# youmi-zym/GO-SLAM

Measured on AMD Instinct MI355X. Metric: BA keyframes/s (6 x FactorGraph.update: reproject + corr lookup + GRU + 2 GN BA iters) on synthetic 640x480 RGB-D, higher is better.
Workload: dtype f32 (BA/geometry; fp64 solve), f16 (corr volume, GRU convs); 1 GPU; configs[1]-shaped frontend window: 60x80 maps (480x640 RGB-D), P=25 keyframes, E=75 edges, 6 updates/keyframe, iters=2, RGB-D depth prior, upsample on; parallelism=replicas x1 (tracking does not shard)

## Files before the change

go_slam_amd/_lib.py:

```python
import ctypes
import os
import subprocess

_HERE = os.path.dirname(os.path.abspath(__file__))
CSRC = os.path.join(_HERE, "csrc")
LIB_PATH = os.environ.get("GOSLAM_HIP_LIB") or os.path.join(CSRC, "libgoslam_hip.so")

_lib = None

c_int, c_float, c_void_p, c_size_t = ctypes.c_int, ctypes.c_float, ctypes.c_void_p, ctypes.c_size_t

_P = c_void_p
SIGNATURES = {
    "gs_version": (ctypes.c_char_p, []),
    "gs_last_error": (ctypes.c_char_p, []),
    "gs_enc_conv_wpack_elems": (c_size_t, [c_int, c_int, c_int]),
    "gs_enc_conv_stat_chunks": (c_int, [c_int, c_int, c_int]),
    "gs_enc_conv": (c_int, [_P, c_int, c_int, _P, _P, _P, c_int, c_int, c_int, c_int, c_int, c_int, c_int, _P, _P, _P]),
    "gs_norm_act_workspace_bytes_chunks": (c_size_t, [c_int, c_int, c_int]),
    "gs_timing_begin": (c_int, [_P]),
    "gs_timing_end": (c_int, []),
    "gs_timing_read": (c_int, [ctypes.c_char_p, ctypes.POINTER(ctypes.c_double), ctypes.POINTER(c_int)]),
    "gs_timing_names": (c_int, [ctypes.c_char_p, c_int]),
    "gs_corr_index_forward": (c_int, [_P, _P, _P] + [c_int] * 7 + [_P]),
    "gs_corr_index_backward": (c_int, [_P, _P, _P] + [c_int] * 7 + [_P]),
    "gs_corr_lookup_pyramid": (c_int, [_P] * 6 + [c_int] * 9 + [_P]),
    "gs_corr_lookup_enc": (c_int, [_P] * 8 + [c_int] * 7 + [_P]),
    "gs_corr_lookup_enc_slots": (c_int, [_P] * 9 + [c_int] * 7 + [_P]),
    "gs_corr_lookup_pyramid_slots": (c_int, [_P] * 7 + [c_int] * 9 + [_P]),
    "gs_corr_volume_pyramid_slots": (c_int, [_P] * 7 + [c_int] * 5 + [_P, c_size_t, _P]),
    "gs_corr_volume_workspace_bytes": (c_size_t, [c_int] * 4),
    "gs_corr_volume_pyramid": (c_int, [_P] * 6 + [c_int] * 5 + [_P, c_size_t, _P]),
    "gs_corr_level_elems": (c_size_t, [c_int] * 4),
    "gs_altcorr_backward": (c_int, [_P] * 6 + [c_int] * 8 + [_P]),
    "gs_altcorr_forward": (c_int, [_P] * 4 + [c_int] * 9 + [_P]),
    "gs_altcorr_pyramid": (c_int, [_P] * 8 + [c_int] * 5 + [_P]),
    "gs_reproject": (c_int, [_P] * 7 + [c_int] * 3 + [_P]),
    "gs_projmap": (c_int, [_P] * 7 + [c_int] * 3 + [_P]),
    "gs_frame_distance": (c_int, [_P] * 6 + [c_int] * 3 + [c_float, _P]),
    "gs_iproj": (c_int, [_P] * 4 + [c_int] * 3 + [_P]),
    "gs_depth_filter": (c_int, [_P] * 6 + [c_int] * 4 + [_P]),
    "gs_pointcloud_workspace_bytes": (c_size_t, [c_int] * 3),
    "gs_pointcloud_count": (c_int, [_P] * 5 + [c_float, c_float] + [c_int] * 4 + [_P, c_size_t, _P]),
    "gs_pointcloud_mask": (c_int, [_P, _P] + [c_int] * 4 + [_P, c_size_t, _P]),
    "gs_pointcloud_scan": (c_int, [c_int] * 3 + [_P, c_size_t, _P, _P]),
    "gs_pointcloud_emit": (c_int, [_P] * 5 + [c_int] * 4 + [_P, c_size_t, ctypes.c_longlong, _P, _P, _P]),
    "gs_frame_prep_color": (c_int, [_P, c_int, c_int, c_int, c_int, c_int, _P]),
    "gs_frame_prep_depth": (c_int, [_P, c_int, c_float, c_int, c_int, c_int, c_int, _P]),
    "gs_cvx_upsample":(c_int, [_P] * 4 + [c_int] * 4 + [_P]),
    "gs_upmask_upsample": (c_int, [_P, c_int, _P, _P, _P, _P, _P, c_int, c_int, c_int, _P]),
    "gs_bias_act": (c_int, [_P, _P, _P, c_int, c_int, c_int, c_int, c_int, _P]),
    "gs_motion_features": (c_int, [_P, _P, _P, c_int, c_int, c_int, _P]),
    "gs_ba_inputs": (c_int, [_P] * 6 + [c_int, c_int, c_int, _P]),
    "gs_lowmem_gather": (c_int, [_P] * 7 + [c_int, c_int, c_int, _P]),
    "gs_lowmem_scatter": (c_int, [_P] * 8 + [c_int, c_int, c_int, _P]),
    "gs_damping_rows": (c_int, [_P] * 5 + [c_int, c_int, c_float, c_float, _P]),
    "gs_conv1x1": (c_int, [_P, c_int, c_int, _P, _P, c_int, _P, c_int, c_int, ctypes.c_longlong, _P]),
    "gs_conv7x7_c4": (c_int, [_P, _P, _P, _P, c_int, c_int, c_int, c_int, c_int, c_int, _P]),
    "gs_conv3x3_wpack_elems": (c_size_t, [c_int, c_int]),
    "gs_conv3x3_pp": (c_int, [_P, c_int, c_int, _P, c_int, _P, c_int, c_int, c_int, c_int, c_int, c_int, _P]),
    "gs_conv3x3_bias_relu": (c_int, [_P, c_int, c_int, _P, _P, _P, c_int, c_int, c_int, c_int, c_int, _P]),
    "gs_conv3x3_gru_zr": (c_int, [_P, c_int, c_int, _P, _P, _P, _P, _P, _P, c_int, c_int, c_int, _P]),
    "gs_conv3x3_gru_zr2": (c_int, [_P, _P, c_int, c_int, _P, _P, _P, _P, _P, _P, c_int, c_int, c_int, _P]),
    "gs_conv3x3_gru_q": (c_int, [_P, _P, c_int, c_int, _P, _P, _P, _P, _P, _P, _P, c_int, c_int, c_int, _P]),
    "gs_conv3x3_head": (c_int, [_P, c_int, _P, c_int, _P, _P, c_int, c_int, c_float, _P, c_int, c_int, c_int, _P]),
    "gs_segment_mean": (c_int, [_P, c_int, _P, c_int, _P, _P, _P, c_int, c_int, c_int, _P]),
    "gs_norm_act_workspace_bytes": (c_size_t, [c_int, c_int, c_int]),
    "gs_norm_act": (c_int, [_P, _P, _P, _P] + [c_int] * 6 + [c_float, _P, c_size_t, c_int, _P]),
    "gs_gru_glo_workspace_bytes": (c_size_t, [c_int]),
    "gs_gru_glo": (c_int, [_P] * 11 + [c_int, c_int, _P, c_size_t, _P]),
    "gs_gru_glo_fused_workspace_bytes": (c_size_t, [c_int, c_int]),
    "gs_gru_glo_fused": (c_int, [_P, c_int] + [_P] * 10 + [c_int, c_int, _P, c_size_t, _P]),
    "gs_gru_gate_zr": (c_int, [_P] * 6 + [c_int] * 3 + [_P]),
    "gs_gru_gate_q": (c_int, [_P] * 7 + [c_int] * 2 + [_P]),
    "gs_edge_prep": (c_int, [_P] * 4 + [c_int, _P, _P] + [c_int] * 6 + [c_float, c_int, c_int, _P]),
    "gs_edge_greedy": (c_int, [_P] * 5 + [c_int] * 5 + [c_float, c_int, c_int, _P]),
    "gs_ba_workspace_bytes": (c_size_t, [c_int] * 5),
    "gs_ba": (c_int, [_P] * 9 + [c_int] * 3 + [c_float, c_float] + [c_int] * 6 + [_P, _P, _P, _P, c_size_t, _P]),
    "gs_ba_ex": (c_int, [_P] * 9 + [c_int] * 3 + [c_float, c_float] + [c_int] * 6 + [_P, _P, _P, _P, c_size_t, c_int, _P]),
    "gs_chol_solve": (c_int, [_P, _P, c_int, c_float, c_float, c_int, _P, _P, _P]),
    "gs_traj_eval_workspace_bytes": (c_size_t, [c_int]),
    "gs_traj_world": (c_int, [_P, _P, c_int, _P, _P, _P]),
    "gs_ape_moments": (c_int, [_P, _P, _P, c_int, _P, _P, c_size_t, _P]),
    "gs_ape_stats": (c_int, [_P, _P, _P, _P, c_int, _P, _P, _P, c_size_t, _P]),
    "gs_grid_meta_default": (c_int, [_P]),
    "gs_neus_level_major_min_points": (c_int, [c_int]),
    "gs_render_sample": (c_int, [_P] * 7 + [c_float, _P, _P, _P] + [c_int] * 3 + [_P]),
    "gs_grid_encode": (c_int, [_P] * 4 + [c_int, _P]),
    "gs_grid_backward": (c_int, [_P, _P, _P, c_int, c_float, _P, _P, c_int, c_float, _P, _P, c_int, _P]),
    "gs_mlp_workspace_bytes": (c_size_t, [c_int, c_int]),
    "gs_mlp_forward": (c_int, [_P] * 3 + [c_int] * 3 + [_P, c_size_t, _P]),
    "gs_neus_forward_workspace_bytes": (c_size_t, [c_int, c_int]),
    "gs_neus_forward": (c_int, [_P] * 9 + [c_float] + [_P] * 18 + [c_float, _P, c_float, c_int, c_int, _P, c_size_t, _P]),
    "gs_neus_forward_pieces": (c_int, [c_int] * 3),
    "gs_neus_forward_segmented": (c_int, [_P] * 9 + [c_float] + [_P] * 18 + [c_float, c_int, _P, _P, c_float]
                                  + [c_int] * 4 + [_P, c_size_t, _P]),
    "gs_render_img_sample": (c_int, [_P, c_int, c_int] + [c_float] * 4 + [_P] * 5 + [c_int] + [_P] * 5
                             + [c_int, c_int, _P]),
    "gs_render_img_metrics_workspace_bytes": (c_size_t, []),
    "gs_render_img_metrics": (c_int, [_P] * 7 + [c_int, c_int] + [_P] * 5 + [c_size_t, _P]),
    "gs_neus_backward_rays": (c_int, [_P] * 13 + [c_int, c_int, _P]),
    "gs_mapping_loss": (c_int, [_P] * 8 + [c_float] * 4 + [c_int] + [_P] * 4 + [c_int, c_int, _P]),
    "gs_map_grad_sqnorm": (c_int, [_P, c_size_t, c_float, _P, c_size_t, _P, _P]),
    "gs_map_adamw": (c_int, [_P, _P, _P, _P, _P, c_size_t, c_float, _P, c_size_t] + [c_float] * 6 + [c_int, _P, c_float, _P]),
    "gs_map_gram_blocks": (c_int, [c_int]),
    "gs_map_gram": (c_int, [_P, c_int, _P, _P]),
    "gs_map_step_prep": (c_int, [_P, c_int, _P, c_float, c_float, c_int] + [_P] * 13),
    "gs_map_step_post": (c_int, [_P, c_int, c_float, _P, c_int, _P, _P, _P, c_float, _P, _P, c_int, c_float, c_int, _P, _P, _P]),
    "gs_map_adamw_seg": (c_int, [_P, _P, _P, _P, _P, c_size_t, c_float, _P, _P, _P, _P, _P, c_size_t] + [c_float] * 6
                         + [c_int, _P, _P, c_float, _P]),
    "gs_mlp_backward_blocks": (c_int, [c_int]),
    "gs_mlp_backward": (c_int, [_P, _P, _P, _P, c_float, _P, _P, c_int, _P]),
    "gs_neus_backward_points": (c_int, [_P] * 7 + [c_float] + [_P] * 9 + [c_int, c_float, _P, _P, c_int, c_float] + [_P] * 5 + [c_int, c_float, c_int, _P, c_int, c_int, _P, _P]),
    "gs_neus_backward_points_binned": (c_int, [_P] * 7 + [c_float] + [_P] * 9 + [c_int, c_float, _P, _P, c_float] + [_P] * 5
                                       + [c_int, c_float, c_int, _P, c_int, c_int, _P, c_size_t, _P, _P, _P]),
    "gs_neus_bin_workspace_bytes": (c_size_t, [c_int]),
    "gs_neus_backward_raygrad": (c_int, [_P] * 7 + [c_float] + [_P] * 9 + [c_int, c_float] + [_P] * 3
                                 + [c_int, c_int, _P]),
    "gs_pose_grad_reduce": (c_int, [_P, _P, _P, c_int, _P, _P]),
    "gs_ray_draw": (c_int, [_P] * 7 + [c_int] * 4 + [c_float] * 4 + [_P] * 5),
    "gs_sdf_lattice": (c_int, [_P] * 3 + [c_int] * 3 + [_P] * 6 + [_P]),
    "gs_mcubes_workspace_bytes": (c_size_t, [c_int] * 3),
    "gs_mcubes_count": (c_int, [_P, c_int, c_int, c_int, c_float, _P, c_size_t, _P]),
    "gs_mcubes_scan": (c_int, [c_int, c_int, c_int, _P, c_size_t, _P, _P]),
    "gs_mcubes_emit": (c_int, [_P, c_int, c_int, c_int, c_float, _P, c_size_t, ctypes.c_longlong, ctypes.c_longlong,
                               _P, _P, _P]),
    "gs_mesh_depth_workspace_bytes": (c_size_t, []),
    "gs_mesh_depth": (c_int, [_P, c_int, _P, c_int, _P, c_int] + [c_float] * 4 + [c_int, c_int, c_float, c_float, _P, _P,
                                                                                   c_size_t, _P]),
    "gs_mesh_visibility": (c_int, [_P, c_int, _P, _P, c_int] + [c_float] * 4 + [c_int, c_int, c_float, _P, _P, _P]),
    "gs_face_components_workspace_bytes": (c_size_t, [c_int]),
    "gs_face_components": (c_int, [_P, c_int, _P, _P, c_size_t, _P]),
    "gs_face_component_areas": (c_int, [_P, _P, c_int, _P, _P, _P, _P, _P, c_size_t, _P]),
    "gs_hull_extremes_workspace_bytes": (c_size_t, [c_int]),
    "gs_hull_extremes": (c_int, [_P, c_int, _P, _P, c_size_t, _P]),
    "gs_hull_prefilter": (c_int, [_P, c_int, _P, c_int, ctypes.c_double, _P, _P]),
    "gs_mesh_visbuf_workspace_bytes": (c_size_t, []),
    "gs_mesh_visbuf": (c_int, [_P, c_int, _P, c_int, _P, c_int] + [c_float] * 4 + [c_int, c_int, c_float, c_float, _P, _P,
                                                                                    c_size_t, _P]),
    "gs_line_visbuf": (c_int, [_P, c_int, ctypes.c_uint, _P, c_int] + [c_float] * 4 + [c_int, c_int, c_float, c_float, _P,
                                                                                        _P]),
    "gs_vertex_normals": (c_int, [_P, c_int, _P, c_int, ctypes.c_double, _P, _P, _P]),
    "gs_visbuf_resolve": (c_int, [_P, c_int, c_int, c_int, _P, c_int, _P, c_int, _P] + [c_float] * 4
                          + [_P, _P, c_int, _P, c_int, c_float, c_float, ctypes.c_uint, _P, _P]),
    "gs_nn_cell_keys":(c_int, [_P, c_int, _P, _P, _P, _P]),
    "gs_nn_grid_build": (c_int, [_P, c_int, _P, _P, _P, _P, _P, _P, _P]),
    "gs_nn_query_workspace_bytes": (c_size_t, [c_int]),
    "gs_nn_query": (c_int, [_P, _P, _P, _P, c_int, _P, _P, _P, c_int, _P, ctypes.c_double, _P, _P, _P, c_size_t, _P]),
    "gs_icp_moments_workspace_bytes": (c_size_t, [c_int]),
    "gs_icp_moments": (c_int, [_P, c_int, _P, _P, _P, _P, _P, _P, c_size_t, _P]),
}


class ColorView(ctypes.Structure):
    _fields_ = [("src", c_void_p), ("map_x", c_void_p), ("map_y", c_void_p), ("tmp", c_void_p), ("dst", c_void_p),
                ("h", c_int), ("w", c_int), ("c", c_int), ("mh", c_int), ("mw", c_int)]


class DepthView(ctypes.Structure):
    _fields_ = [("src", c_void_p), ("dst", c_void_p), ("h", c_int), ("w", c_int)]


FRAME_PREP_MAX_VIEWS = 32


class GridMeta(ctypes.Structure):
    _fields_ = [("scale", c_float * 16), ("resolution", ctypes.c_uint32 * 16), ("size", ctypes.c_uint32 * 16),
                ("offset", ctypes.c_uint32 * 16), ("hashed", ctypes.c_uint32 * 16), ("total", ctypes.c_uint32)]


def grid_meta():
    m = GridMeta()
    check(lib().gs_grid_meta_default(ctypes.byref(m)), "gs_grid_meta_default")
    return m


def build(verbose=False):
    cmd = ["make", "-C", CSRC, "-j8"]
    res = subprocess.run(cmd, stdout=subprocess.PIPE, stderr=subprocess.STDOUT, text=True)
    if verbose or res.returncode != 0:
        print(res.stdout)
    if res.returncode != 0:
        raise RuntimeError("building libgoslam_hip.so failed:\n" + res.stdout[-4000:])
    return LIB_PATH


def lib():
    global _lib
    if _lib is None:
        if not os.path.exists(LIB_PATH):
            raise RuntimeError(
                f"{LIB_PATH} not found: build it with `python -c 'import __graft_entry__ as g; g.build()'` "
                "(go_slam_amd has no CPU fallback)")
        handle = ctypes.CDLL(LIB_PATH)
        for name, (res, args) in SIGNATURES.items():
            fn = getattr(handle, name)
            fn.restype = res
            fn.argtypes = args
        _lib = handle
    return _lib


def check(rc, what):
    if rc != 0:
        msg = lib().gs_last_error().decode("utf-8", "replace")
        raise RuntimeError(f"{what} failed (status {rc}): {msg}")


class kernel_timer:

    def __init__(self, device=None):
        self.device = device

    def __enter__(self):
        check(lib().gs_timing_begin(stream_ptr(self.device)), "gs_timing_begin")
        return self

    def __exit__(self, *exc):
        lib().gs_timing_end()
        return False

    def read(self):
        L = lib()
        buf = ctypes.create_string_buffer(1 << 16)
        check(L.gs_timing_names(buf, len(buf)), "gs_timing_names")
        out = {}
        for name in [n for n in buf.value.decode().split(",") if n]:
            ms, cnt = ctypes.c_double(0.0), c_int(0)
            check(L.gs_timing_read(name.encode(), ctypes.byref(ms), ctypes.byref(cnt)), "gs_timing_read")
            out[name] = (ms.value, cnt.value)
        return out


def stream_ptr(device=None):
    import torch
    return ctypes.c_void_p(torch.cuda.current_stream(device).cuda_stream)


_EMPTY_SENTINEL = {}


def ptr(t):
    if t is None:
        return ctypes.c_void_p(0)
    p = t.data_ptr()
    if p == 0 and t.numel() == 0 and t.is_cuda:
        s = _EMPTY_SENTINEL.get(t.device)
        if s is None:
            import torch
            s = _EMPTY_SENTINEL[t.device] = torch.zeros(64, dtype=torch.uint8, device=t.device)
        p = s.data_ptr()
    return ctypes.c_void_p(p)
```

go_slam_amd/csrc/ba.hip:

```cpp
#include "common.h"

int gs_chol_solve_launch(double* H, double* b, int n, float lm, float ep, float* dx_out, int32_t* fail_flag,
                         int32_t* fail_count, hipStream_t st);

namespace {

constexpr float kMinDepth = 0.25f;
constexpr float kAlpha = 0.05f;
constexpr int kPrepThreads = 1024;
constexpr int kAccSplit = 4;
constexpr int kMaxBuf = 4096;

struct BaWs {
  int32_t* hdr;
  int32_t* kinv;
  int32_t* kx;
  int32_t* edge_m;
  int32_t* row_ptr;
  int32_t* csr_edge;
  int32_t* ent_ptr;
  int32_t* ent_src;
  int32_t* ent_pose;
  int32_t* pair_ptr;
  float* Q;
// ... 312 lines not shown
          if (j_in) gs_atomic_add_f64(&w.b[6 * pj_ + (tid - 84)], s);
        }
      }
      __syncthreads();
    }
  }

  if (!motion_only && active) {
    if (nsplit > 1) {
      float* po = w.part + (((size_t)split * gridDim.y + m) * 8) * hw + p;
      po[0] = Csum;
      po[(size_t)hw] = wsum;
#pragma unroll
      for (int n = 0; n < 6; ++n) po[(size_t)(2 + n) * hw] = Ei[n];
      return;
    }
    const size_t o = (size_t)m * hw + p;
    const float sens = disps_sens[(size_t)k * hw + p];
    const float mk = (sens > 0.0f) ? 1.0f : 0.0f;
    const float C = Csum + mk * kAlpha + (1.0f - mk) * eta[o];
    const float ww = wsum - mk * kAlpha * (disp - sens);
    w.Q[o] = 1.0f / C;
    w.W[o] = ww;
    if (i_in) {
      float* eo = w.Ei + ((size_t)m * 6) * hw + p;
#pragma unroll
      for (int n = 0; n < 6; ++n) eo[(size_t)n * hw] = Ei[n];
    }
  }
}

__global__ __launch_bounds__(256) void ba_accum_finish_kernel(const float* __restrict__ disps,
                                                              const float* __restrict__ disps_sens,
                                                              const float* __restrict__ eta, int t0, int t1, int hw, int nsp,
                                                              BaWs w) {
  const int m = blockIdx.y;
  if (m >= w.hdr[0]) return;
  const int nsplit = min(nsp, max(w.row_ptr[m + 1] - w.row_ptr[m], 1));
  if (nsplit <= 1) return;
  const int p = blockIdx.x * 256 + threadIdx.x;
  if (p >= hw) return;
  float acc[8];
#pragma unroll
  for (int n = 0; n < 8; ++n) acc[n] = 0.0f;
  for (int s2 = 0; s2 < nsplit; ++s2) {
    const float* pi_ = w.part + (((size_t)s2 * gridDim.y + m) * 8) * hw + p;
#pragma unroll
    for (int n = 0; n < 8; ++n) acc[n] += pi_[(size_t)n * hw];
  }
  const int k = w.kx[m];
  const size_t o = (size_t)m * hw + p;
  const float disp = disps[(size_t)k * hw + p];
  const float sens = disps_sens[(size_t)k * hw + p];
  const float mk = (sens > 0.0f) ? 1.0f : 0.0f;
  const float C = acc[0] + mk * kAlpha + (1.0f - mk) * eta[o];
  const float ww = acc[1] - mk * kAlpha * (disp - sens);
  w.Q[o] = 1.0f / C;
  w.W[o] = ww;
  const int pi = k - t0;
  if (pi >= 0 && pi < t1 - t0) {
    float* eo = w.Ei + ((size_t)m * 6) * hw + p;
#pragma unroll
    for (int n = 0; n < 6; ++n) eo[(size_t)n * hw] = acc[2 + n];
  }
}

__global__ __launch_bounds__(256) void ba_schur_kernel(int M, int hw, int P, BaWs w) {
  __shared__ float red[4][44];
  const int tid = threadIdx.x;
  const int wave = tid >> 6, lane = tid & 63;
  typedef const __attribute__((address_space(4))) int* cip;
  cip pair_ptr = (cip)w.pair_ptr, ent_ptr = (cip)w.ent_ptr, ent_pose = (cip)w.ent_pose, ent_src = (cip)w.ent_src;
  const int n_pairs = pair_ptr[M];
  const int n6 = 6 * P;
  for (int pidx = blockIdx.x; pidx < n_pairs; pidx += gridDim.x) {
    int lo = 0, hi = M;
    while (hi - lo > 1) {
      const int mid = (lo + hi) >> 1;
      if (pair_ptr[mid] <= pidx) lo = mid; else hi = mid;
    }
    const int m = lo;
    const int eb = ent_ptr[m];
    const int nm = ent_ptr[m + 1] - eb;
    const int r = pidx - pair_ptr[m];
    const int a = r / nm, b = r - a * nm;
    const int pa = ent_pose[eb + a], pb = ent_pose[eb + b];
    if (pa < pb) continue;
    const int sa = ent_src[eb + a], sb = ent_src[eb + b];
    const float* Ea = (sa < M) ? w.Ei + (size_t)sa * 6 * hw : w.Eij + (size_t)(sa - M) * 6 * hw;
    const float* Eb = (sb < M) ? w.Ei + (size_t)sb * 6 * hw : w.Eij + (size_t)(sb - M) * 6 * hw;
    const float* Qm = w.Q + (size_t)m * hw;
    const float* Wm = w.W + (size_t)m * hw;
    const bool diag = (a == b);
    float S[36];
#pragma unroll
    for (int i = 0; i < 36; ++i) S[i] = 0.f;
    float vv[6] = {0.f, 0.f, 0.f, 0.f, 0.f, 0.f};
    constexpr int UP = 4;
    for (int p0 = tid; p0 < hw; p0 += UP * 256) {
      float q[UP], ea[UP][6], eb_[UP][6], ww[UP];
#pragma unroll
      for (int u = 0; u < UP; ++u) {
        const int p = p0 + 256 * u;
        const bool ok = p < hw;
        const int pc = ok ? p : tid;
        q[u] = Qm[pc];
#pragma unroll
        for (int n = 0; n < 6; ++n) {
          ea[u][n] = Ea[(size_t)n * hw + pc];
          eb_[u][n] = Eb[(size_t)n * hw + pc];
        }
        ww[u] = diag ? Wm[pc] : 0.0f;
      }
#pragma unroll
      for (int u = 0; u < UP; ++u) {
        if (p0 + 256 * u < hw) {
#pragma unroll
          for (int n = 0; n < 6; ++n) ea[u][n] = ea[u][n] * q[u];
#pragma unroll
          for (int n = 0; n < 6; ++n)
#pragma unroll
            for (int c = 0; c < 6; ++c) S[n * 6 + c] = fmaf(ea[u][n], eb_[u][c], S[n * 6 + c]);
          if (diag) {
#pragma unroll
            for (int n = 0; n < 6; ++n) vv[n] = fmaf(ea[u][n], ww[u], vv[n]);
          }
        }
      }
    }
    {
      float rs[42];
#pragma unroll
      for (int i = 0; i < 36; ++i) rs[i] = S[i];
#pragma unroll
      for (int n = 0; n < 6; ++n) rs[36 + n] = vv[n];
      gs_wave_reduce_scatter<42>(rs, lane);
      const int ix = gs_bitrev6(lane);
      if (ix < 42) red[wave][ix] = rs[0];
    }
    __syncthreads();
    if (tid < 36) {
      const int rr = tid / 6, cc = tid - rr * 6;
      const double s = (double)((red[0][tid] + red[1][tid]) + (red[2][tid] + red[3][tid]));
      if (pa > pb || rr >= cc)
        gs_atomic_add_f64(&w.H[(size_t)(6 * pa + rr) * n6 + (6 * pb + cc)], -s);
    } else if (diag && tid < 42) {
      const double s = (double)((red[0][tid] + red[1][tid]) + (red[2][tid] + red[3][tid]));
      gs_atomic_add_f64(&w.b[6 * pa + (tid - 36)], -s);
    }
    __syncthreads();
  }
}

__global__ __launch_bounds__(256) void ba_update_kernel(
    float* __restrict__ poses, float* __restrict__ disps, const float* __restrict__ dx,
    float* __restrict__ dz, int M, int t0, int t1, int hw, BaWs w) {
  const int tid = threadIdx.x;
  const int P = t1 - t0;
  if ((int)blockIdx.y == M) {
    if (blockIdx.x != 0) return;
    for (int kk = t0 + tid; kk < t1; kk += 256) {
      float* pp = poses + (size_t)kk * 7;
      float t[3] = {pp[0], pp[1], pp[2]};
      float q[4] = {pp[3], pp[4], pp[5], pp[6]};
      float xi[6], tn[3], qn[4];
#pragma unroll
      for (int n = 0; n < 6; ++n) xi[n] = dx[(size_t)(kk - t0) * 6 + n];
      gs_retr_se3(xi, t, q, tn, qn);
      pp[0] = tn[0]; pp[1] = tn[1]; pp[2] = tn[2];
      pp[3] = qn[0]; pp[4] = qn[1]; pp[5] = qn[2]; pp[6] = qn[3];
    }
    return;
  }
  const int m = blockIdx.y;
  const int p = blockIdx.x * 256 + tid;
  if (p >= hw) return;
  if (m >= w.hdr[0]) {
    dz[(size_t)m * hw + p] = 0.0f;
    return;
  }
  const int eb = w.ent_ptr[m], ee = w.ent_ptr[m + 1];
  float dw = 0.f;
  for (int idx = eb; idx < ee; ++idx) {
    const int pn = w.ent_pose[idx];
    if (pn <= 0 || pn >= P) continue;
    const int s = w.ent_src[idx];
    const float* En = (s < M) ? w.Ei + (size_t)s * 6 * hw : w.Eij + (size_t)(s - M) * 6 * hw;
    float acc = 0.f;
#pragma unroll
    for (int n = 0; n < 6; ++n) acc += En[(size_t)n * hw + p] * dx[(size_t)pn * 6 + n];
    dw += acc;
  }
  const size_t o = (size_t)m * hw + p;
  const float z = w.Q[o] * (w.W[o] - dw);
  dz[o] = z;
  const size_t dk = (size_t)w.kx[m] * hw + p;
  disps[dk] = disps[dk] + z;
}

__global__ void ba_status_kernel(int32_t* status_out, BaWs w) {
  if (threadIdx.x < 4) status_out[threadIdx.x] = (threadIdx.x == 2) ? w.hdr[3] : (threadIdx.x == 3 ? w.hdr[4] : w.hdr[threadIdx.x]);
}

}

extern "C" size_t gs_ba_workspace_bytes(int n_edges, int n_poses, int n_depth, int nbuf, int hw) {
  if (n_edges < 0 || n_poses < 0 || n_depth < 0 || nbuf < 0 || hw < 0) return 0;
  return carve(nullptr, n_edges, n_poses, n_depth, nbuf, hw).total + 256;
}

extern "C" int gs_ba_ex(float* poses, float* disps, const float* intrinsics, const float* disps_sens,
                        const float* targets, const float* weights, const float* eta, const int64_t* ii,
                        const int64_t* jj, int t0, int t1, int iterations, float lm, float ep, int motion_only,
                        int n_edges, int n_depth, int nbuf, int h, int w, float* dx, float* dz,
                        int32_t* status_out, void* workspace, size_t workspace_bytes, int flags, gs_stream_t stream) {
  GS_REQUIRE(poses && disps && intrinsics && disps_sens && targets && weights && ii && jj && dx && workspace,
             "ba: null pointer");
  GS_REQUIRE(motion_only || (eta && dz), "ba: eta/dz required unless motion_only");
  GS_REQUIRE(h > 0 && w > 0 && n_edges >= 0 && iterations >= 0, "ba: bad shape");
  GS_REQUIRE(t0 >= 0 && t1 > t0 && t1 <= nbuf, "ba: window [%d,%d) outside buffer of %d frames", t0, t1, nbuf);
  GS_REQUIRE(nbuf <= kMaxBuf, "ba: buffer of %d frames exceeds the supported %d", nbuf, kMaxBuf);
  GS_REQUIRE(n_depth > 0 && n_depth <= nbuf && n_depth <= 65534, "ba: n_depth=%d out of range", n_depth);
  const int hw = h * w, P = t1 - t0, M = n_depth;
  const size_t need = gs_ba_workspace_bytes(n_edges, P, M, nbuf, hw);
  if (workspace_bytes < need) {
    gs_set_error("ba: workspace too small (%zu < %zu bytes)", workspace_bytes, need);
    return GS_ERR_WORKSPACE;
  }
  void* base = (void*)gs_align((size_t)workspace);
  BaWs ws = carve(base, n_edges, P, M, nbuf, hw);
  hipStream_t st = (hipStream_t)stream;
  const int n6 = 6 * P;

  const bool reuse = (flags & 1) != 0;
  if (!reuse) {
    ba_prep_kernel<<<1, kPrepThreads, 0, st>>>(ii, jj, n_edges, nbuf, t0, t1, M, ws);
    GS_CHECK_LAUNCH("ba_prep");
  }
  const int chunks = gs_cdiv(hw, 256);
  for (int it = 0; it < iterations; ++it) {
    if (hipMemsetAsync(ws.H, 0, ((size_t)n6 * n6 + n6) * sizeof(double), st) != hipSuccess) {
      gs_set_error("ba: memset failed");
      return GS_ERR_LAUNCH;
    }
    const int nsp = (!motion_only && n_edges >= 6 * M) ? kAccSplit : 1;
    ba_accum_kernel<<<dim3(chunks, M, nsp), 256, 0, st>>>(poses, disps, intrinsics, disps_sens, targets, weights,
                                                          eta, jj, t0, t1, hw, w, motion_only,
                                                          (reuse && it == 0) ? 1 : 0, ws);
    GS_CHECK_LAUNCH("ba_accum");
    if (!motion_only) {
      if (nsp > 1) {
        ba_accum_finish_kernel<<<dim3(chunks, M), 256, 0, st>>>(disps, disps_sens, eta, t0, t1, hw, nsp, ws);
        GS_CHECK_LAUNCH("ba_accum_finish");
      }
      ba_schur_kernel<<<2048, 256, 0, st>>>(M, hw, P, ws);
      GS_CHECK_LAUNCH("ba_schur");
    }
    int rc = gs_chol_solve_launch(ws.H, ws.b, n6, lm, ep, dx, &ws.hdr[2], &ws.hdr[3], st);
    if (rc != GS_OK) return rc;
    if (motion_only)
      ba_update_kernel<<<dim3(1, 1), 256, 0, st>>>(poses, disps, dx, dz, 0, t0, t1, hw, ws);
    else
      ba_update_kernel<<<dim3(chunks, M + 1), 256, 0, st>>>(poses, disps, dx, dz, M, t0, t1, hw, ws);
    GS_CHECK_LAUNCH("ba_update");
  }
  if (status_out) {
    ba_status_kernel<<<1, 64, 0, st>>>(status_out, ws);
    GS_CHECK_LAUNCH("ba_status");
  }
  return GS_OK;
}

extern "C" int gs_ba(float* poses, float* disps, const float* intrinsics, const float* disps_sens,
                     const float* targets, const float* weights, const float* eta, const int64_t* ii,
                     const int64_t* jj, int t0, int t1, int iterations, float lm, float ep, int motion_only,
                     int n_edges, int n_depth, int nbuf, int h, int w, float* dx, float* dz,
                     int32_t* status_out, void* workspace, size_t workspace_bytes, gs_stream_t stream) {
  return gs_ba_ex(poses, disps, intrinsics, disps_sens, targets, weights, eta, ii, jj, t0, t1, iterations, lm, ep,
                  motion_only, n_edges, n_depth, nbuf, h, w, dx, dz, status_out, workspace, workspace_bytes, 0, stream);
}
```

go_slam_amd/csrc/conv3x3_pp.hip:

```cpp
#include "common.h"
#include "conv3x3_common.h"

namespace {

constexpr int PP_KG = 4;
constexpr int PP_PSTR = 5;
constexpr int pp_zpad(int tw) { return (((2 * (tw + 2) + 2) * PP_PSTR + 3 + 15) / 16) * 16; }
constexpr int pp_patch_slots(int tw) {
  return (((512 / tw + 2) * (tw + 2) * PP_PSTR + 511) / 512) * 512 + pp_zpad(tw);
}

__device__ __attribute__((aligned(16))) const uint32_t pp_zero_page[4] = {0u, 0u, 0u, 0u};

__device__ __forceinline__ void pp_glds16(const void* src, void* lds_wave_base) {
  __builtin_amdgcn_global_load_lds((const __attribute__((address_space(1))) void*)src,
                                   (__attribute__((address_space(3))) void*)lds_wave_base, 16, 0, 0);
}

#define PP_BAR()                              \
  do {                                        \
    asm volatile("" ::: "memory");            \
    __builtin_amdgcn_s_barrier();             \
    asm volatile("" ::: "memory");            \
    __builtin_amdgcn_sched_barrier(0);        \
  } while (0)

#define PP_LGKM0()                                        \
  do {                                                    \
    asm volatile("s_waitcnt lgkmcnt(0)" ::: "memory");    \
    __builtin_amdgcn_sched_barrier(0);                    \
  } while (0)

struct PpEpi {
  const float* bias;
  const float* glo;
  const _Float16* inp_pre;
  const _Float16* aux0;
  const _Float16* aux1;
  _Float16* out0;
  _Float16* out1;
  const _Float16* xb;
  int xsb, split;
  long long* dbg;
  int variant;
};

template <bool PROBE>
__device__ __forceinline__ void pp_stamp(long long* dbg, int slot) {
  if constexpr (PROBE) {
    if (dbg && threadIdx.x == 0) dbg[(size_t)blockIdx.x * 4 + slot] = (long long)__builtin_amdgcn_s_memtime();
  }
}

__device__ __forceinline__ float pp_sigm(float v) { return gs_sigmoid(v); }

template <int TW, int EPI, int BN = 128, bool PROBE = false>
__global__ __launch_bounds__(512, 1) void conv3x3_pp_kernel(const _Float16* __restrict__ x, int xs, int C,
                                                            const half8* __restrict__ wpack, _Float16* __restrict__ y,
                                                            int ys, int H, int W, int rows, int tiles_x, int NB,
                                                            int xcd, PpEpi ep) {
  static_assert(BN == 128 || (BN == 64 && (EPI == 0 || EPI == 3)), "64-channel workgroups: plain / bias + ReLU only");
  constexpr int PP_BN = BN;
  constexpr int PP_WTAP = PP_KG * PP_BN;
  constexpr int NJ = BN / 64;
  constexpr int PP_TS = NJ == 2 ? 72 : 40;
  constexpr int TH_ = 512 / TW, PW_ = TW + 2, NPX = (TH_ + 2) * PW_;
  constexpr int PSTR = PP_PSTR;
  constexpr int ZPAD = pp_zpad(TW);
  constexpr int NROUND = (NPX * PSTR + 511) / 512;
  constexpr int PSLOTS = NROUND * 512 + ZPAD;
  constexpr int ZSLOT = NROUND * 512;
  static_assert(PSLOTS == pp_patch_slots(TW), "launch_pp sizes the LDS with the same formula");
  static_assert(NROUND <= 9, "one DMA round per tap");
  extern __shared__ half8 smem[];
  half8* const pbuf = smem;
  half8* const wbuf = smem + 2 * PSLOTS;
  half8* const wjunk = wbuf + 4 * PP_WTAP;
  const int tid = threadIdx.x, lane = tid & 63;
  const int wv = __builtin_amdgcn_readfirstlane(tid >> 6);
  const int grp2 = wv >> 2;
  const int wm = (wv & 1) + 2 * grp2;
  const int wn = (wv >> 1) & 1;
  const int r = lane & 31, kgl = lane >> 5;
  int tix, nb;
  decode_block(blockIdx.x, gridDim.x / NB, NB, xcd, tix, nb);
  const int tx0 = (tix % tiles_x) * TW;
  const int g0 = (tix / tiles_x) * TH_;
  const int nchunk = C / 32;
  const int T = nchunk * 9;
  const half8* wsrc = wpack + (size_t)nb * T * PP_WTAP;

  int pb[4];
  bool top[4], bot[4];
#pragma unroll
  for (int i = 0; i < 4; ++i) {
    int ty, tx;
    tile_pixel<TW, true>(wm, i, r, ty, tx);
    pb[i] = ty * PW_ + tx;
    const int yy = (g0 + ty) % H;
    top[i] = yy == 0;
    bot[i] = yy == H - 1;
  }
  int poff[NROUND];
#pragma unroll
  for (int q = 0; q < NROUND; ++q) {
    const int s = q * 512 + tid, p = s / PSTR, kg = s - PSTR * p;
    int off = -1;
    if (p < NPX && kg < 4) {
      const int pr = p / PW_, pc = p - pr * PW_;
      const int gv = g0 + pr - 1, gx = tx0 + pc - 1;
      if (gv >= 0 && gv < rows && gx >= 0 && gx < W) off = (gv * W + gx) * 4 + kg;
    }
    poff[q] = off;
  }

  int vb[4], vt[4], vo[4];
#pragma unroll
  for (int i = 0; i < 4; ++i) {
    vb[i] = pb[i] * PSTR + kgl;
    vt[i] = top[i] ? ZSLOT : vb[i];
    vo[i] = bot[i] ? ZSLOT : vb[i];
  }
  {
    const half8 z8 = {0, 0, 0, 0, 0, 0, 0, 0};
    if (tid < ZPAD) pbuf[ZSLOT + tid] = z8;
    else if (tid < 2 * ZPAD) pbuf[PSLOTS + ZSLOT + tid - ZPAD] = z8;
    static_assert(2 * ZPAD <= 512, "one store per thread");
  }

  float16v acc[NJ][4];
#pragma unroll
  for (int j = 0; j < NJ; ++j)
#pragma unroll
    for (int i = 0; i < 4; ++i)
#pragma unroll
      for (int e = 0; e < 16; ++e) acc[j][i][e] = 0.0f;
  half8 a[2][NJ], b[2][4];

  auto issue_patch = [&](int src_chunk, int buf, int q, int off) {
    const void* src = (const void*)pp_zero_page;
    if (off >= 0) {
      const size_t pix = (size_t)(off >> 2);
      const int c0 = src_chunk * 32 + (off & 3) * 8;
      if constexpr (EPI == 1 || EPI == 2)
        src = c0 < ep.split ? (const void*)(x + pix * xs + c0) : (const void*)(ep.xb + pix * ep.xsb + (c0 - ep.split));
      else
        src = (const void*)(x + pix * xs + c0);
    }
    pp_glds16(src, pbuf + buf * PSLOTS + q * 512 + wv * 64);
  };
  auto issue_w = [&](int src_tap, int buf) {
    if constexpr (BN == 128) {
      pp_glds16(wsrc + (size_t)src_tap * PP_WTAP + tid, wbuf + buf * PP_WTAP + wv * 64);
    } else {
      if (wv < 4) pp_glds16(wsrc + (size_t)src_tap * PP_WTAP + tid, wbuf + buf * PP_WTAP + wv * 64);
      else pp_glds16((const void*)pp_zero_page, wjunk + (wv - 4) * 64);
    }
  };
  auto read_frags = [&](int pbuf_ix, int wbuf_ix, int tap) {
    const half8* wb = wbuf + wbuf_ix * PP_WTAP;
    const half8* pp = pbuf + pbuf_ix * PSLOTS;
    const int dy = tap / 3, toff = dy * PW_ + (tap % 3);
#pragma unroll
    for (int s = 0; s < 2; ++s) {
      const int kg = 2 * s + kgl;
#pragma unroll
      for (int j = 0; j < NJ; ++j) a[s][j] = wb[kg * PP_BN + wn * (PP_BN / 2) + 32 * j + r];
    }
#pragma unroll
    for (int i = 0; i < 4; ++i) {
      int base = dy == 0 ? vt[i] : dy == 2 ? vo[i] : vb[i];
      if constexpr (PROBE) {
        if (ep.variant & 2) base = vb[i];
      }
      asm volatile("" : "+v"(base));
      const half8* q = pp + base;
      b[0][i] = q[toff * PSTR];
      b[1][i] = q[toff * PSTR + 2];
    }
  };
  bool prio = true;
  if constexpr (PROBE) prio = !(ep.variant & 1);
  auto math = [&](auto&& between) {
    if (prio) __builtin_amdgcn_s_setprio(1);
#pragma unroll
    for (int i = 0; i < 2; ++i)
#pragma unroll
      for (int j = 0; j < NJ; ++j)
        acc[j][i] = __builtin_amdgcn_mfma_f32_32x32x16_f16(a[0][j], b[0][i], acc[j][i], 0, 0, 0);
    __builtin_amdgcn_sched_barrier(0);
    between();
    __builtin_amdgcn_sched_barrier(0);
#pragma unroll
    for (int i = 2; i < 4; ++i)
#pragma unroll
      for (int j = 0; j < NJ; ++j)
        acc[j][i] = __builtin_amdgcn_mfma_f32_32x32x16_f16(a[0][j], b[0][i], acc[j][i], 0, 0, 0);
#pragma unroll
    for (int i = 0; i < 4; ++i)
#pragma unroll
      for (int j = 0; j < NJ; ++j)
        acc[j][i] = __builtin_amdgcn_mfma_f32_32x32x16_f16(a[1][j], b[1][i], acc[j][i], 0, 0, 0);
    if (prio) __builtin_amdgcn_s_setprio(0);
  };

  pp_stamp<PROBE>(ep.dbg, 0);
#pragma unroll
  for (int q = 0; q < NROUND; ++q) issue_patch(0, 0, q, poff[q]);
  issue_w(0, 0);
  issue_w(1, 1);
  issue_w(2, 2);
  asm volatile("s_waitcnt vmcnt(0) lgkmcnt(0)" ::: "memory");
  PP_BAR();
  pp_stamp<PROBE>(ep.dbg, 1);
  if (grp2 == 1) PP_BAR();
  read_frags(0, 0, 0);
  PP_LGKM0();
  PP_BAR();

  for (int ck = 0; ck < nchunk; ++ck) {
#pragma unroll
    for (int tap = 0; tap < 9; ++tap) {
      const int tg = ck * 9 + tap;
      __builtin_amdgcn_sched_barrier(0);
      math([&]() {
        if constexpr (PROBE) {
          if (ep.variant & 4) return;
        }
        const int tw = tg + 3 < T ? tg + 3 : T - 1;
        issue_w(tw, (tg + 3) & 3);
        if (tap < NROUND) issue_patch(ck + 1 < nchunk ? ck + 1 : nchunk - 1, (ck + 1) & 1, tap, poff[tap]);
      });
      __builtin_amdgcn_sched_barrier(0);
      if (tap < NROUND) asm volatile("s_waitcnt vmcnt(2)" ::: "memory");
      else asm volatile("s_waitcnt vmcnt(1)" ::: "memory");
      PP_BAR();
      bool reads = true;
      if constexpr (PROBE) reads = !(ep.variant & 8);
      if (reads) {
        if (tap < 8) read_frags(ck & 1, (tg + 1) & 3, tap + 1);
        else if (ck + 1 < nchunk) read_frags((ck + 1) & 1, (tg + 1) & 3, 0);
      }
      PP_LGKM0();
      PP_BAR();
    }
  }
  pp_stamp<PROBE>(ep.dbg, 2);
  if (grp2 == 0) PP_BAR();
  asm volatile("s_waitcnt vmcnt(0)" ::: "memory");
  PP_BAR();

  _Float16* tile = reinterpret_cast<_Float16*>(smem) + wv * 32 * PP_TS;
  _Float16* yb = y + nb * PP_BN + wn * (PP_BN / 2);
  constexpr int PIECES = NJ * 4;
  constexpr int PXIT = 64 / PIECES;
  constexpr int NIT = 32 / PXIT;
#pragma unroll
  for (int i = 0; i < 4; ++i) {
    size_t pix4[NIT];
    bool ok4[NIT];
    half8 pi4[NIT], u4[NIT], v4[NIT];
    const int piece = lane & (PIECES - 1);
    const int c8 = wn * (PP_BN / 2) + piece * 8;
#pragma unroll
    for (int it = 0; it < NIT; ++it) {
      const int pxr = it * PXIT + lane / PIECES;
      int ty, tx;
      tile_pixel<TW, true>(wm, i, pxr, ty, tx);
      const int gv = g0 + ty, gx = tx0 + tx;
      ok4[it] = gv < rows && gx < W;
      pix4[it] = (size_t)gv * W + gx;
      if constexpr (EPI == 1 || EPI == 2) {
        const half8 z8 = {0, 0, 0, 0, 0, 0, 0, 0};
        pi4[it] = z8; u4[it] = z8; v4[it] = z8;
        if (ok4[it]) {
          if constexpr (EPI == 1) {
            if (ep.inp_pre) pi4[it] = *reinterpret_cast<const half8*>(ep.inp_pre + pix4[it] * 384 + nb * 128 + c8);
            if (nb == 1) u4[it] = *reinterpret_cast<const half8*>(x + pix4[it] * xs + c8);
          } else {
            if (ep.inp_pre) pi4[it] = *reinterpret_cast<const half8*>(ep.inp_pre + pix4[it] * 384 + 256 + c8);
            u4[it] = *reinterpret_cast<const half8*>(ep.aux0 + pix4[it] * 128 + c8);
            v4[it] = *reinterpret_cast<const half8*>(ep.aux1 + pix4[it] * 128 + c8);
          }
        }
      }
    }
#pragma unroll
    for (int j = 0; j < NJ; ++j)
#pragma unroll
      for (int g = 0; g < 4; ++g) {
        half4 o;
#pragma unroll
        for (int e = 0; e < 4; ++e) o[e] = (_Float16)acc[j][i][4 * g + e];
        *reinterpret_cast<half4*>(tile + r * PP_TS + j * 32 + 8 * g + 4 * kgl) = o;
      }
    __builtin_amdgcn_fence(__ATOMIC_RELEASE, "wavefront");
    __builtin_amdgcn_wave_barrier();
    __builtin_amdgcn_fence(__ATOMIC_ACQUIRE, "wavefront");
#pragma unroll
    for (int it = 0; it < NIT; ++it) {
      const int pxr = it * PXIT + lane / PIECES;
      if (ok4[it]) {
        const half8 v = *reinterpret_cast<const half8*>(tile + pxr * PP_TS + piece * 8);
        const size_t pix = pix4[it];
        if constexpr (EPI == 0) {
          *reinterpret_cast<half8*>(yb + pix * ys + piece * 8) = v;
        } else if constexpr (EPI == 3) {
          const float* bb = ep.bias + nb * PP_BN + c8;
          half8 o;
#pragma unroll
          for (int k = 0; k < 8; ++k) o[k] = (_Float16)fmaxf((float)v[k] + bb[k], 0.0f);
          *reinterpret_cast<half8*>(yb + pix * ys + piece * 8) = o;
        } else if constexpr (EPI == 1) {
          const int img = (int)(pix / ((size_t)H * W));
          const half8 pi = pi4[it];
          const float* bb = ep.bias + nb * 128 + c8;
          const float* gg = ep.glo + (size_t)img * 256 + nb * 128 + c8;
          half8 o;
          if (nb == 0) {
#pragma unroll
            for (int k = 0; k < 8; ++k) o[k] = (_Float16)pp_sigm((float)v[k] + (float)pi[k] + bb[k] + gg[k]);
            *reinterpret_cast<half8*>(ep.out0 + pix * 128 + c8) = o;
          } else {
            const half8 net = u4[it];
#pragma unroll
            for (int k = 0; k < 8; ++k)
              o[k] = (_Float16)(pp_sigm((float)v[k] + (float)pi[k] + bb[k] + gg[k]) * (float)net[k]);
            *reinterpret_cast<half8*>(ep.out1 + pix * 128 + c8) = o;
          }
        } else {
          const int img = (int)(pix / ((size_t)H * W));
          const half8 pi = pi4[it], zz = u4[it], nn = v4[it];
          const float* bb = ep.bias + c8;
          const float* gg = ep.glo + (size_t)img * 128 + c8;
          half8 o;
#pragma unroll
          for (int k = 0; k < 8; ++k) {
            const float a_ = (float)v[k] + (float)pi[k] + bb[k] + gg[k];
            const float q = gs_tanh(a_);
            const float zf = (float)zz[k];
            o[k] = (_Float16)((1.0f - zf) * (float)nn[k] + zf * q);
          }
          *reinterpret_cast<half8*>(ep.out0 + pix * 128 + c8) = o;
        }
      }
    }
    __builtin_amdgcn_fence(__ATOMIC_RELEASE, "wavefront");
    __builtin_amdgcn_wave_barrier();
  }
  pp_stamp<PROBE>(ep.dbg, 3);
}

template <int TW, int EPI, int BN = 128, bool PROBE = false>
int launch_pp(const void* x, int x_stride, int c_in, const void* wpack, void* y, int y_stride, int n_out, int n, int h,
              int w, int xcd, hipStream_t st, PpEpi ep = PpEpi()) {
  constexpr int PP_BN = BN, PP_WTAP = PP_KG * BN;
  constexpr size_t lds = (size_t)(2 * pp_patch_slots(TW) + 4 * PP_WTAP + (BN == 64 ? 256 : 0)) * sizeof(half8);
  static_assert(lds <= 160 * 1024, "conv3x3_pp: more LDS than a CU has");
  static GsLdsLimit limit;
  if (int rc = limit.raise((const void*)conv3x3_pp_kernel<TW, EPI, BN, PROBE>, lds, "conv3x3_pp")) return rc;
  const long long rows = (long long)n * h;
  GS_REQUIRE(rows * w < (1ll << 29), "conv3x3_pp: too many pixels");
  const int tiles_x = gs_cdiv(w, TW), tiles_y = gs_cdiv((int)rows, 512 / TW);
  const int NB = n_out / PP_BN;
  const long long blocks = (long long)tiles_x * tiles_y * NB;
  GS_REQUIRE(blocks < (1ll << 31), "conv3x3_pp: too many workgroups");
  conv3x3_pp_kernel<TW, EPI, BN, PROBE><<<dim3((unsigned)blocks), 512, lds, st>>>(
      (const _Float16*)x, x_stride, c_in, (const half8*)wpack, (_Float16*)y, y_stride, h, w, (int)rows, tiles_x, NB, xcd,
      ep);
  GS_CHECK_LAUNCH("conv3x3_pp");
  return GS_OK;
}

template <int EPI, int BN = 128>
int dispatch_pp(const void* x, int x_stride, int c_in, const void* wpack, int tw, void* y, int y_stride, int n_out, int n,
                int h, int w, int xcd, hipStream_t st, PpEpi ep = PpEpi()) {
  if (tw == 8) return launch_pp<8, EPI, BN>(x, x_stride, c_in, wpack, y, y_stride, n_out, n, h, w, xcd, st, ep);
  return launch_pp<16, EPI, BN>(x, x_stride, c_in, wpack, y, y_stride, n_out, n, h, w, xcd, st, ep);
}

int pp_block_channels(int n_out) { return n_out % 128 == 0 ? 128 : 64; }

int pp_tile_width(int w) { return gs_cdiv(w, 8) * 8 < gs_cdiv(w, 16) * 16 ? 8 : 16; }

}

extern "C" int gs_conv3x3_pp(const void* x, int x_stride, int c_in, const void* wpack, int tw, void* y, int y_stride,
                             int n_out, int n, int h, int w, int xcd_order, gs_stream_t stream) {
  GS_REQUIRE(x && wpack && y, "conv3x3_pp: null pointer");
  GS_REQUIRE(tw == 8 || tw == 16, "conv3x3_pp: tile width must be 8 or 16");
  GS_REQUIRE(c_in > 0 && c_in % 32 == 0, "conv3x3_pp: c_in must be a multiple of 32 (weights packed with kc = 32)");
  GS_REQUIRE(n_out > 0 && n_out % 64 == 0, "conv3x3_pp: n_out must be a multiple of 64");
  GS_REQUIRE(x_stride >= c_in && x_stride % 8 == 0, "conv3x3_pp: x_stride must be >= c_in and a multiple of 8");
  GS_REQUIRE(y_stride >= n_out && y_stride % 8 == 0, "conv3x3_pp: y_stride must be >= n_out and a multiple of 8");
  GS_REQUIRE(n >= 0 && h > 0 && w > 0, "conv3x3_pp: bad shape");
  if (n == 0) return GS_OK;
  if (pp_block_channels(n_out) == 64)
    return dispatch_pp<0, 64>(x, x_stride, c_in, wpack, tw, y, y_stride, n_out, n, h, w, xcd_order ? 1 : 0,
                              (hipStream_t)stream);
  return dispatch_pp<0>(x, x_stride, c_in, wpack, tw, y, y_stride, n_out, n, h, w, xcd_order ? 1 : 0,
                        (hipStream_t)stream);
}

extern "C" int gs_conv3x3_gru_zr(const void* hx, int hx_stride, int c_in, const void* wpack, const float* bias_zr,
                                 const float* glo_zr, const void* inp_pre, void* z_out, void* rnet_out, int n, int h,
                                 int w, gs_stream_t stream) {
  GS_REQUIRE(hx && wpack && bias_zr && glo_zr && z_out && rnet_out, "conv3x3_gru_zr: null pointer");
  GS_REQUIRE(c_in >= 128 && c_in % 32 == 0, "conv3x3_gru_zr: c_in must be >= 128 and a multiple of 32");
  GS_REQUIRE(hx_stride >= c_in && hx_stride % 8 == 0, "conv3x3_gru_zr: bad hx_stride");
  GS_REQUIRE(n >= 0 && h > 0 && w > 0, "conv3x3_gru_zr: bad shape");
  if (n == 0) return GS_OK;
  PpEpi ep = PpEpi();
  ep.bias = bias_zr;
  ep.glo = glo_zr;
  ep.inp_pre = (const _Float16*)inp_pre;
  ep.out0 = (_Float16*)z_out;
  ep.out1 = (_Float16*)rnet_out;
  ep.xb = (const _Float16*)hx;
  ep.xsb = hx_stride;
  ep.split = 1 << 30;
  return dispatch_pp<1>(hx, hx_stride, c_in, wpack, pp_tile_width(w), nullptr, 0, 256, n, h, w, 1, (hipStream_t)stream, ep);
}

extern "C" int gs_conv3x3_gru_zr2(const void* net, const void* x_rest, int x_rest_stride, int c_rest, const void* wpack,
                                  const float* bias_zr, const float* glo_zr, const void* inp_pre, void* z_out,
                                  void* rnet_out, int n, int h, int w, gs_stream_t stream) {
  GS_REQUIRE(net && x_rest && wpack && bias_zr && glo_zr && z_out && rnet_out, "conv3x3_gru_zr2: null pointer");
  GS_REQUIRE(c_rest > 0 && c_rest % 32 == 0, "conv3x3_gru_zr2: c_rest must be a multiple of 32");
  GS_REQUIRE(x_rest_stride >= c_rest && x_rest_stride % 8 == 0, "conv3x3_gru_zr2: bad x_rest_stride");
  GS_REQUIRE(n >= 0 && h > 0 && w > 0, "conv3x3_gru_zr2: bad shape");
  if (n == 0) return GS_OK;
  PpEpi ep = PpEpi();
  ep.bias = bias_zr;
  ep.glo = glo_zr;
  ep.inp_pre = (const _Float16*)inp_pre;
  ep.out0 = (_Float16*)z_out;
  ep.out1 = (_Float16*)rnet_out;
  ep.xb = (const _Float16*)x_rest;
  ep.xsb = x_rest_stride;
  ep.split = 128;
  return dispatch_pp<1>(net, 128, 128 + c_rest, wpack, pp_tile_width(w), nullptr, 0, 256, n, h, w, 1,
                        (hipStream_t)stream, ep);
}

extern "C" int gs_conv3x3_gru_q(const void* rnet, const void* x_rest, int x_rest_stride, int c_rest, const void* wpack,
                                const float* bias_q, const float* glo_q, const void* inp_pre, const void* z,
                                const void* net, void* net_out, int n, int h, int w, gs_stream_t stream) {
  GS_REQUIRE(rnet && x_rest && wpack && bias_q && glo_q && z && net && net_out, "conv3x3_gru_q: null pointer");
  GS_REQUIRE(c_rest > 0 && c_rest % 32 == 0, "conv3x3_gru_q: c_rest must be a multiple of 32");
  GS_REQUIRE(x_rest_stride >= c_rest && x_rest_stride % 8 == 0, "conv3x3_gru_q: bad x_rest_stride");
  GS_REQUIRE(n >= 0 && h > 0 && w > 0, "conv3x3_gru_q: bad shape");
  if (n == 0) return GS_OK;
  PpEpi ep = PpEpi();
  ep.bias = bias_q;
  ep.glo = glo_q;
  ep.inp_pre = (const _Float16*)inp_pre;
  ep.aux0 = (const _Float16*)z;
  ep.aux1 = (const _Float16*)net;
  ep.out0 = (_Float16*)net_out;
  ep.xb = (const _Float16*)x_rest;
  ep.xsb = x_rest_stride;
  ep.split = 128;
  return dispatch_pp<2>(rnet, 128, 128 + c_rest, wpack, pp_tile_width(w), nullptr, 0, 128, n, h, w, 1,
                        (hipStream_t)stream, ep);
}

extern "C" int gs_conv3x3_bias_relu(const void* x, int x_stride, int c_in, const void* wpack, const float* bias, void* y,
                                    int y_stride, int n_out, int n, int h, int w, gs_stream_t stream) {
  GS_REQUIRE(x && wpack && bias && y, "conv3x3_bias_relu: null pointer");
  GS_REQUIRE(c_in > 0 && c_in % 32 == 0, "conv3x3_bias_relu: c_in must be a multiple of 32");
  GS_REQUIRE(n_out > 0 && n_out % 64 == 0, "conv3x3_bias_relu: n_out must be a multiple of 64");
  GS_REQUIRE(x_stride >= c_in && x_stride % 8 == 0, "conv3x3_bias_relu: bad x_stride");
  GS_REQUIRE(y_stride >= n_out && y_stride % 8 == 0, "conv3x3_bias_relu: bad y_stride");
  GS_REQUIRE(n >= 0 && h > 0 && w > 0, "conv3x3_bias_relu: bad shape");
  if (n == 0) return GS_OK;
  PpEpi ep = PpEpi();
  ep.bias = bias;
  if (pp_block_channels(n_out) == 64)
    return dispatch_pp<3, 64>(x, x_stride, c_in, wpack, pp_tile_width(w), y, y_stride, n_out, n, h, w, 1,
                              (hipStream_t)stream, ep);
  return dispatch_pp<3>(x, x_stride, c_in, wpack, pp_tile_width(w), y, y_stride, n_out, n, h, w, 1, (hipStream_t)stream,
                        ep);
}

extern "C" size_t gs_conv3x3_wpack_elems(int c_in, int n_out) { return (size_t)9 * c_in * n_out; }

#ifdef GS_BUILD_PROBES
extern "C" int gs_conv3x3_pp_probe(const void* x, int x_stride, int c_in, const void* wpack, int tw, void* y, int y_stride,
                                   int n_out, int n, int h, int w, int variant, long long* dbg, gs_stream_t stream) {
  GS_REQUIRE(x && wpack && y, "conv3x3_pp_probe: null pointer");
  GS_REQUIRE(tw == 16 && c_in > 0 && c_in % 32 == 0 && n_out > 0 && n_out % 128 == 0 && n > 0,
             "conv3x3_pp_probe: bad arguments (tw must be 16)");
  PpEpi ep = PpEpi();
  ep.dbg = dbg;
  ep.variant = variant;
  return launch_pp<16, 0, 128, true>(x, x_stride, c_in, wpack, y, y_stride, n_out, n, h, w, 1, (hipStream_t)stream, ep);
}
#endif
```

go_slam_amd/csrc/geom.hip:

```cpp
#include "geom_common.h"

namespace {

constexpr float kMinDepthKernel = 0.25f;
constexpr float kMinDepthPy = 0.2f;

__global__ __launch_bounds__(256) void reproject_kernel(
    const float* __restrict__ poses, const float* __restrict__ disps, const float* __restrict__ intr,
    const int64_t* __restrict__ ii, const int64_t* __restrict__ jj, float* __restrict__ coords,
    float* __restrict__ valid, int hw, int wd) {
  const int p = blockIdx.x * 256 + threadIdx.x;
  const int e = blockIdx.y;
  if (p >= hw) return;
  const int ix = (int)ii[e], jx = (int)jj[e];
  float tij[3], qij[4];
  if (ix == jx) {
    tij[0] = -0.1f; tij[1] = 0.f; tij[2] = 0.f;
    qij[0] = 0.f; qij[1] = 0.f; qij[2] = 0.f; qij[3] = 1.f;
  } else {
    float ti[3], qi[4], tj[3], qj[4];
    gs_load_pose(poses, ix, ti, qi);
    gs_load_pose(poses, jx, tj, qj);
    float qinv[4] = {-qi[0], -qi[1], -qi[2], qi[3]};
    float r[3], tinv[3];
    gs_act_so3(qinv, ti, r);
    tinv[0] = -r[0]; tinv[1] = -r[1]; tinv[2] = -r[2];
    gs_act_so3(qj, tinv, r);
    tij[0] = tj[0] + r[0]; tij[1] = tj[1] + r[1]; tij[2] = tj[2] + r[2];
    gs_quat_mul(qj, qinv, qij);
  }
  const float fxi = intr[ix * 4 + 0], fyi = intr[ix * 4 + 1], cxi = intr[ix * 4 + 2], cyi = intr[ix * 4 + 3];
  const float fxj = intr[jx * 4 + 0], fyj = intr[jx * 4 + 1], cxj = intr[jx * 4 + 2], cyj = intr[jx * 4 + 3];
  const float u = (float)(p % wd), v = (float)(p / wd);
  float X0[4] = {(u - cxi) / fxi, (v - cyi) / fyi, 1.0f, disps[(size_t)ix * hw + p]};
  float X1[4];
  gs_act_se3(tij, qij, X0, X1);
  const float Z = (X1[2] < 0.5f * kMinDepthPy) ? 1.0f : X1[2];
  const size_t o = (size_t)e * hw + p;
  reinterpret_cast<float2*>(coords)[o] = make_float2(fxj * (X1[0] / Z) + cxj, fyj * (X1[1] / Z) + cyj);
  valid[o] = ((X1[2] > kMinDepthPy) && (X0[2] > kMinDepthPy)) ? 1.0f : 0.0f;
}

__global__ __launch_bounds__(256) void projmap_kernel(
    const float* __restrict__ poses, const float* __restrict__ disps, const float* __restrict__ intr,
    const int64_t* __restrict__ ii, const int64_t* __restrict__ jj, float* __restrict__ coords,
    float* __restrict__ valid, int hw, int wd) {
  const int p = blockIdx.x * 256 + threadIdx.x;
  const int e = blockIdx.y;
  if (p >= hw) return;
  const int ix = (int)ii[e], jx = (int)jj[e];
  float ti[3], qi[4], tj[3], qj[4], tij[3], qij[4];
  gs_load_pose(poses, ix, ti, qi);
  gs_load_pose(poses, jx, tj, qj);
  gs_rel_se3(ti, qi, tj, qj, tij, qij);
  const float fx = intr[0], fy = intr[1], cx = intr[2], cy = intr[3];
  const float u = (float)(p % wd), v = (float)(p / wd);
  float Xi[4] = {(u - cx) / fx, (v - cy) / fy, 1.0f, disps[(size_t)ix * hw + p]};
  float Xj[4];
  gs_act_se3(tij, qij, Xi, Xj);
  float cu = u, cv = v;
  if (Xj[2] > 0.01f) {
    cu = fx * (Xj[0] / Xj[2]) + cx;
    cv = fy * (Xj[1] / Xj[2]) + cy;
  }
  const size_t o = (size_t)e * hw + p;
  coords[o * 3 + 0] = cu;
  coords[o * 3 + 1] = cv;
  coords[o * 3 + 2] = 0.0f;
  valid[o] = (Xj[2] > kMinDepthKernel) ? 1.0f : 0.0f;
}

__global__ __launch_bounds__(256) void frame_distance_kernel(
    const float* __restrict__ poses, const float* __restrict__ disps, const float* __restrict__ intr,
    const int64_t* __restrict__ ii, const int64_t* __restrict__ jj, float* __restrict__ dist,
    int hw, int wd, float beta) {
  const int e = blockIdx.x;
  const int ix = (int)ii[e], jx = (int)jj[e];
  float ti[3], qi[4], tj[3], qj[4], tij[3], qij[4];
  gs_load_pose(poses, ix, ti, qi);
  gs_load_pose(poses, jx, tj, qj);
  gs_rel_se3(ti, qi, tj, qj, tij, qij);
  const float fx = intr[0], fy = intr[1], cx = intr[2], cy = intr[3];
  float accum = 0.f, valid = 0.f;
  const float* dsp = disps + (size_t)ix * hw;
  for (int p = threadIdx.x; p < hw; p += 256) {
    const float u = (float)(p % wd), v = (float)(p / wd);
    float Xi[4] = {(u - cx) / fx, (v - cy) / fy, 1.0f, dsp[p]};
    float Xj[4];
    gs_act_se3(tij, qij, Xi, Xj);
    float du = fx * (Xj[0] / Xj[2]) + cx - u;
    float dv = fy * (Xj[1] / Xj[2]) + cy - v;
    float d = sqrtf(du * du + dv * dv);
    if (Xj[2] > kMinDepthKernel) { accum += beta * d; valid += beta; }
    float Yx = Xi[0] + Xi[3] * tij[0];
    float Yy = Xi[1] + Xi[3] * tij[1];
    float Yz = Xi[2] + Xi[3] * tij[2];
    du = fx * (Yx / Yz) + cx - u;
    dv = fy * (Yy / Yz) + cy - v;
    d = sqrtf(du * du + dv * dv);
    if (Yz > kMinDepthKernel) { accum += (1.0f - beta) * d; valid += (1.0f - beta); }
  }
  __shared__ float red[2][4];
  accum = gs_wave_sum(accum);
  valid = gs_wave_sum(valid);
  const int wave = threadIdx.x >> 6;
  if ((threadIdx.x & 63) == 0) { red[0][wave] = accum; red[1][wave] = valid; }
  __syncthreads();
  if (threadIdx.x == 0) {
    const float a = (red[0][0] + red[0][1]) + (red[0][2] + red[0][3]);
    const float vl = (red[1][0] + red[1][1]) + (red[1][2] + red[1][3]);
    const float total = (float)hw * (beta + (1.0f - beta));
    dist[e] = (vl / (total + 1e-8f) < 0.75f) ? 1000.0f : a / vl;
  }
}

__global__ __launch_bounds__(256) void iproj_kernel(
    const float* __restrict__ poses, const float* __restrict__ disps, const float* __restrict__ intr,
    float* __restrict__ points, int hw, int wd) {
  const int p = blockIdx.x * 256 + threadIdx.x;
  const int n = blockIdx.y;
  if (p >= hw) return;
  float t[3], q[4];
  gs_load_pose(poses, n, t, q);
  const float u = (float)(p % wd), v = (float)(p / wd);
  gs_iproj_point(t, q, intr[0], intr[1], intr[2], intr[3], u, v, disps[(size_t)n * hw + p],
                 points + ((size_t)n * hw + p) * 3);
}

__global__ __launch_bounds__(256) void depth_filter_kernel(
    const float* __restrict__ poses, const float* __restrict__ disps, const float* __restrict__ intr,
    const int64_t* __restrict__ inds, const float* __restrict__ thresh, float* __restrict__ counter,
    int num, int hw, int ht, int wd) {
  const int p = blockIdx.x * 256 + threadIdx.x;
  const int b = blockIdx.y;
  if (p >= hw) return;
  counter[(size_t)b * hw + p] = gs_depth_filter_count(poses, disps, (int)inds[b], p, intr[0], intr[1], intr[2],
                                                      intr[3], thresh[b], num, hw, ht, wd);
}

}

#define GS_GEOM_COMMON(name)                                                              \
  GS_REQUIRE(n >= 0 && h > 0 && w > 0, name ": bad shape");                               \
  if (n == 0) return GS_OK;                                                               \
  hipStream_t st = (hipStream_t)stream;                                                   \
  const int hw = h * w;

extern "C" int gs_reproject(const float* poses, const float* disps, const float* intrinsics,
                            const int64_t* ii, const int64_t* jj, float* coords, float* valid, int n, int h,
                            int w, gs_stream_t stream) {
  GS_REQUIRE(poses && disps && intrinsics && ii && jj && coords && valid, "reproject: null pointer");
  GS_GEOM_COMMON("reproject");
  GS_REQUIRE(n <= 65535, "reproject: n=%d exceeds grid.y limit", n);
  reproject_kernel<<<dim3(gs_cdiv(hw, 256), n), 256, 0, st>>>(poses, disps, intrinsics, ii, jj, coords, valid, hw, w);
  GS_CHECK_LAUNCH("reproject");
  return GS_OK;
}

extern "C" int gs_projmap(const float* poses, const float* disps, const float* intrinsics, const int64_t* ii,
                          const int64_t* jj, float* coords, float* valid, int n, int h, int w,
                          gs_stream_t stream) {
  GS_REQUIRE(poses && disps && intrinsics && ii && jj && coords && valid, "projmap: null pointer");
  GS_GEOM_COMMON("projmap");
  GS_REQUIRE(n <= 65535, "projmap: n=%d exceeds grid.y limit", n);
  projmap_kernel<<<dim3(gs_cdiv(hw, 256), n), 256, 0, st>>>(poses, disps, intrinsics, ii, jj, coords, valid, hw, w);
  GS_CHECK_LAUNCH("projmap");
  return GS_OK;
}

extern "C" int gs_frame_distance(const float* poses, const float* disps, const float* intrinsics,
                                 const int64_t* ii, const int64_t* jj, float* dist, int n, int h, int w,
                                 float beta, gs_stream_t stream) {
  GS_REQUIRE(poses && disps && intrinsics && ii && jj && dist, "frame_distance: null pointer");
  GS_GEOM_COMMON("frame_distance");
  frame_distance_kernel<<<n, 256, 0, st>>>(poses, disps, intrinsics, ii, jj, dist, hw, w, beta);
  GS_CHECK_LAUNCH("frame_distance");
  return GS_OK;
}

extern "C" int gs_iproj(const float* poses, const float* disps, const float* intrinsics, float* points, int n,
                        int h, int w, gs_stream_t stream) {
  GS_REQUIRE(poses && disps && intrinsics && points, "iproj: null pointer");
  GS_GEOM_COMMON("iproj");
  GS_REQUIRE(n <= 65535, "iproj: n=%d exceeds grid.y limit", n);
  iproj_kernel<<<dim3(gs_cdiv(hw, 256), n), 256, 0, st>>>(poses, disps, intrinsics, points, hw, w);
  GS_CHECK_LAUNCH("iproj");
  return GS_OK;
}

extern "C" int gs_depth_filter(const float* poses, const float* disps, const float* intrinsics,
                               const int64_t* ix, const float* thresh, float* counter, int n, int num, int h,
                               int w, gs_stream_t stream) {
  GS_REQUIRE(poses && disps && intrinsics && ix && thresh && counter, "depth_filter: null pointer");
  GS_GEOM_COMMON("depth_filter");
  GS_REQUIRE(n <= 65535 && num > 0, "depth_filter: bad n/num");
  depth_filter_kernel<<<dim3(gs_cdiv(hw, 256), n), 256, 0, st>>>(poses, disps, intrinsics, ix, thresh, counter, num, hw, h, w);
  GS_CHECK_LAUNCH("depth_filter");
  return GS_OK;
}
```

go_slam_amd/csrc/gru_gates.hip:

```cpp
#include "common.h"

namespace {

typedef _Float16 half8 __attribute__((ext_vector_type(8)));

__device__ __forceinline__ float sigm(float x) { return gs_sigmoid(x); }

__global__ __launch_bounds__(256) void gru_gate_zr_kernel(const _Float16* __restrict__ zr_pre,
                                                          const float* __restrict__ bias,
                                                          const float* __restrict__ glo,
                                                          const _Float16* __restrict__ inp_pre,
                                                          _Float16* __restrict__ hx,
                                                          _Float16* __restrict__ z_out, int hw, int ldx,
                                                          size_t total ) {
  const size_t t = (size_t)blockIdx.x * 256 + threadIdx.x;
  if (t >= total) return;
  const int c8 = (int)(t & 15);
  const size_t pix = t >> 4;
  const int n = (int)(pix / hw);
  const half8 zp = *reinterpret_cast<const half8*>(zr_pre + pix * 256 + c8 * 8);
  const half8 rp = *reinterpret_cast<const half8*>(zr_pre + pix * 256 + 128 + c8 * 8);
  half8* hp = reinterpret_cast<half8*>(hx + pix * ldx + c8 * 8);
  const half8 net = *hp;
  half8 zi = {0, 0, 0, 0, 0, 0, 0, 0}, ri = zi;
// ... 254 lines not shown
      __builtin_amdgcn_fence(__ATOMIC_RELEASE, "wavefront");
      __builtin_amdgcn_wave_barrier();
    }
  }
}

__global__ __launch_bounds__(384) void glo_heads_kernel(const float* __restrict__ partial, int nchunk, float inv_hw,
                                                        const _Float16* __restrict__ wz, const _Float16* __restrict__ wr,
                                                        const _Float16* __restrict__ wq, const float* __restrict__ bz,
                                                        const float* __restrict__ br, const float* __restrict__ bq,
                                                        float* __restrict__ gzr, float* __restrict__ gq) {
  const int n = blockIdx.x, t = threadIdx.x;
  __shared__ float g[128];
  __shared__ float part3[3][128];
  {
    const int third = t >> 7, ch = t & 127;
    float s = 0.0f;
    for (int c0 = third; c0 < nchunk; c0 += 30) {
      float v[10];
#pragma unroll
      for (int u = 0; u < 10; ++u) {
        const int c = c0 + 3 * u;
        v[u] = c < nchunk ? partial[((size_t)n * nchunk + c) * 128 + ch] : 0.0f;
      }
#pragma unroll
      for (int u = 0; u < 10; ++u)
        if (c0 + 3 * u < nchunk) s += v[u];
    }
    part3[third][ch] = s;
  }
  __syncthreads();
  if (t < 128) g[t] = (float)(_Float16)(((part3[0][t] + part3[1][t]) + part3[2][t]) * inv_hw);
  __syncthreads();
  const int head = t >> 7, o = t & 127;
  const _Float16* w = (head == 0 ? wz : head == 1 ? wr : wq) + (size_t)o * 128;
  float s = (head == 0 ? bz : head == 1 ? br : bq)[o];
#pragma unroll 4
  for (int k8 = 0; k8 < 16; ++k8) {
    const half8 v = *reinterpret_cast<const half8*>(w + k8 * 8);
#pragma unroll
    for (int k = 0; k < 8; ++k) s = fmaf((float)v[k], g[k8 * 8 + k], s);
  }
  s = (float)(_Float16)s;
  if (head < 2) gzr[(size_t)n * 256 + head * 128 + o] = s;
  else gq[(size_t)n * 128 + o] = s;
}
}

extern "C" int gs_bias_act(const void* x, const float* bias, void* y, int rows, int channels, int x_stride,
                           int y_stride, int act, gs_stream_t stream) {
  GS_REQUIRE(x && y, "bias_act: null pointer");
  GS_REQUIRE(rows >= 0 && channels > 0 && channels % 8 == 0, "bias_act: channels must be a multiple of 8");
  GS_REQUIRE(x_stride >= channels && x_stride % 8 == 0, "bias_act: x_stride must be >= channels and a multiple of 8");
  GS_REQUIRE(y_stride >= channels && y_stride % 8 == 0, "bias_act: y_stride must be >= channels and a multiple of 8");
  GS_REQUIRE(act >= 0 && act <= 2, "bias_act: act in {0 none, 1 relu, 2 sigmoid}");
  if (rows == 0) return GS_OK;
  const size_t total = (size_t)rows * (channels / 8);
  const unsigned grid = (unsigned)((total + 255) / 256);
  hipStream_t st = (hipStream_t)stream;
  const _Float16* xi = (const _Float16*)x;
  _Float16* yo = (_Float16*)y;
  const int c8n = channels / 8;
#define GS_BA(A, B) bias_act_kernel<A, B><<<grid, 256, 0, st>>>(xi, bias, yo, c8n, x_stride, y_stride, total)
  if (bias) { if (act == 0) GS_BA(0, true); else if (act == 1) GS_BA(1, true); else GS_BA(2, true); }
  else      { if (act == 0) GS_BA(0, false); else if (act == 1) GS_BA(1, false); else GS_BA(2, false); }
#undef GS_BA
  GS_CHECK_LAUNCH("bias_act");
  return GS_OK;
}

extern "C" int gs_segment_mean(const void* x, int x_stride, const float* in_bias, int in_relu, const int* seg_offsets,
                               const int* seg_edges, void* out, int n_seg, int hw, int channels, gs_stream_t stream) {
  GS_REQUIRE(x && seg_offsets && seg_edges && out, "segment_mean: null pointer");
  GS_REQUIRE(n_seg >= 0 && hw > 0 && channels > 0 && channels % 8 == 0, "segment_mean: channels must be a multiple of 8");
  GS_REQUIRE(x_stride >= channels && x_stride % 8 == 0, "segment_mean: x_stride must be >= channels, multiple of 8");
  if (n_seg == 0) return GS_OK;
  const size_t total = (size_t)n_seg * hw * (channels / 8);
  segment_mean_kernel<<<(unsigned)((total + 255) / 256), 256, 0, (hipStream_t)stream>>>(
      (const _Float16*)x, x_stride, in_bias, in_relu, seg_offsets, seg_edges, (_Float16*)out, hw, channels / 8, total);
  GS_CHECK_LAUNCH("segment_mean");
  return GS_OK;
}

constexpr int GLO_CHUNKS = 32;
extern "C" size_t gs_gru_glo_workspace_bytes(int n) { return (size_t)(n > 0 ? n : 0) * GLO_CHUNKS * 128 * sizeof(float); }

extern "C" int gs_gru_glo(const void* w_pre, const float* w_bias, const void* net, const void* wz, const void* wr,
                          const void* wq, const float* bz, const float* br, const float* bq, float* gzr, float* gq,
                          int n, int hw, void* workspace, size_t workspace_bytes, gs_stream_t stream) {
  GS_REQUIRE(w_pre && w_bias && net && wz && wr && wq && bz && br && bq && gzr && gq, "gru_glo: null pointer");
  GS_REQUIRE(n >= 0 && hw > 0, "gru_glo: bad shape");
  if (n == 0) return GS_OK;
  GS_REQUIRE(workspace && workspace_bytes >= gs_gru_glo_workspace_bytes(n), "gru_glo: workspace too small");
  hipStream_t st = (hipStream_t)stream;
  const int nchunk = GLO_CHUNKS;
  glo_pool_kernel<<<dim3(nchunk, n), 256, 0, st>>>((const _Float16*)w_pre, w_bias, (const _Float16*)net,
                                                   (float*)workspace, hw, nchunk);
  GS_CHECK_LAUNCH("gru_glo pool");
  glo_heads_kernel<<<n, 384, 0, st>>>((const float*)workspace, nchunk, 1.0f / (float)hw, (const _Float16*)wz,
                                      (const _Float16*)wr, (const _Float16*)wq, bz, br, bq, gzr, gq);
  GS_CHECK_LAUNCH("gru_glo heads");
  return GS_OK;
}

extern "C" size_t gs_gru_glo_fused_workspace_bytes(int n, int hw) {
  if (n <= 0 || hw <= 0) return 0;
  return (size_t)n * ((hw + 31) / 32) * 128 * sizeof(float);
}

extern "C" int gs_gru_glo_fused(const void* net, int net_stride, const void* w_pack, const float* w_bias, const void* wz,
                                const void* wr, const void* wq, const float* bz, const float* br, const float* bq,
                                float* gzr, float* gq, int n, int hw, void* workspace, size_t workspace_bytes,
                                gs_stream_t stream) {
  GS_REQUIRE(net && w_pack && w_bias && wz && wr && wq && bz && br && bq && gzr && gq, "gru_glo_fused: null pointer");
  GS_REQUIRE(n >= 0 && hw > 0 && net_stride >= 128 && net_stride % 8 == 0, "gru_glo_fused: bad shape");
  GS_REQUIRE((((size_t)net | (size_t)w_pack) & 15) == 0, "gru_glo_fused: net / w_pack must be 16-byte aligned");
  if (n == 0) return GS_OK;
  GS_REQUIRE(workspace && workspace_bytes >= gs_gru_glo_fused_workspace_bytes(n, hw), "gru_glo_fused: workspace too small");
  hipStream_t st = (hipStream_t)stream;
  const int bpi = (hw + 31) / 32;
  const size_t nblk = (size_t)n * bpi;
  const size_t lds = (size_t)(4 * 8 * 512 + 4 * 32 * 72) * sizeof(_Float16) + 128 * sizeof(float);
  static GsLdsLimit limit;
  if (int rc = limit.raise((const void*)glo_conv_pool_kernel, lds, "gru_glo_fused")) return rc;
  size_t grid = 256 * 3;
  if (grid > (nblk + 3) / 4) grid = (nblk + 3) / 4;
  glo_conv_pool_kernel<<<(unsigned)grid, 256, lds, st>>>((const _Float16*)net, net_stride, (const _Float16*)w_pack, w_bias,
                                                         (float*)workspace, hw, bpi, nblk);
  GS_CHECK_LAUNCH("gru_glo_fused pool");
  glo_heads_kernel<<<n, 384, 0, st>>>((const float*)workspace, bpi, 1.0f / (float)hw, (const _Float16*)wz,
                                      (const _Float16*)wr, (const _Float16*)wq, bz, br, bq, gzr, gq);
  GS_CHECK_LAUNCH("gru_glo_fused heads");
  return GS_OK;
}

namespace {
__global__ __launch_bounds__(256) void motion_features_kernel(const float2* __restrict__ coords1,
                                                              const float2* __restrict__ target,
                                                              _Float16* __restrict__ out, int hw, int w, size_t total) {
  const size_t t = (size_t)blockIdx.x * 256 + threadIdx.x;
  if (t >= total) return;
  const int p = (int)(t % hw);
  const float gx = (float)(p % w), gy = (float)(p / w);
  const float2 c = coords1[t], tg = target[t];
  typedef _Float16 half4m __attribute__((ext_vector_type(4)));
  half4m o;
  o[0] = (_Float16)fminf(fmaxf(c.x - gx, -64.0f), 64.0f);
  o[1] = (_Float16)fminf(fmaxf(c.y - gy, -64.0f), 64.0f);
  o[2] = (_Float16)fminf(fmaxf(tg.x - c.x, -64.0f), 64.0f);
  o[3] = (_Float16)fminf(fmaxf(tg.y - c.y, -64.0f), 64.0f);
  reinterpret_cast<half4m*>(out)[t] = o;
}

__global__ __launch_bounds__(256) void damping_rows_kernel(const float* __restrict__ eta, const int* __restrict__ inv,
                                                           const int64_t* __restrict__ index,
                                                           float* __restrict__ damping_buf, float* __restrict__ out,
                                                           int hw, float scale, float eps, size_t total) {
  const size_t t = (size_t)blockIdx.x * 256 + threadIdx.x;
  if (t >= total) return;
  const int k = (int)(t / hw), p = (int)(t - (size_t)k * hw);
  const int m = inv[k];
  float* slot = damping_buf + (size_t)index[k] * hw + p;
  float v;
  if (m >= 0) { v = eta[(size_t)m * hw + p]; *slot = v; }
  else v = *slot;
  out[t] = scale * v + eps;
}

__global__ __launch_bounds__(256) void ba_inputs_kernel(const float2* __restrict__ coords1, const float2* __restrict__ delta,
                                                        const float2* __restrict__ weight, float2* __restrict__ target,
                                                        float* __restrict__ ba_target, float* __restrict__ ba_weight,
                                                        int hw, size_t total) {
  const size_t t = (size_t)blockIdx.x * 256 + threadIdx.x;
  if (t >= total) return;
  const size_t e = t / hw;
  const int p = (int)(t - e * hw);
  const float2 c = coords1[t], d = delta[t], wt = weight[t];
  const float2 tg = make_float2(c.x + d.x, c.y + d.y);
  target[t] = tg;
  float* bt = ba_target + e * 2 * hw + p;
  bt[0] = tg.x; bt[hw] = tg.y;
  float* bw = ba_weight + e * 2 * hw + p;
  bw[0] = wt.x; bw[hw] = wt.y;
}
}

extern "C" int gs_motion_features(const float* coords1, const float* target, void* out, int n, int h, int w,
                                  gs_stream_t stream) {
  GS_REQUIRE(coords1 && target && out, "motion_features: null pointer");
  GS_REQUIRE(n >= 0 && h > 0 && w > 0, "motion_features: bad shape");
  if (n == 0) return GS_OK;
  const size_t total = (size_t)n * h * w;
  motion_features_kernel<<<(unsigned)((total + 255) / 256), 256, 0, (hipStream_t)stream>>>(
      (const float2*)coords1, (const float2*)target, (_Float16*)out, h * w, w, total);
  GS_CHECK_LAUNCH("motion_features");
  return GS_OK;
}

extern "C" int gs_ba_inputs(const float* coords1, const float* delta, const float* weight, float* target,
                            float* ba_target, float* ba_weight, int n, int h, int w, gs_stream_t stream) {
  GS_REQUIRE(coords1 && delta && weight && target && ba_target && ba_weight, "ba_inputs: null pointer");
  GS_REQUIRE(n >= 0 && h > 0 && w > 0, "ba_inputs: bad shape");
  if (n == 0) return GS_OK;
  const size_t total = (size_t)n * h * w;
  ba_inputs_kernel<<<(unsigned)((total + 255) / 256), 256, 0, (hipStream_t)stream>>>(
      (const float2*)coords1, (const float2*)delta, (const float2*)weight, (float2*)target, ba_target, ba_weight,
      h * w, total);
  GS_CHECK_LAUNCH("ba_inputs");
  return GS_OK;
}

extern "C" int gs_damping_rows(const float* eta, const int* inv, const int64_t* index, float* damping_buf, float* out,
                               int n_rows, int hw, float scale, float eps, gs_stream_t stream) {
  GS_REQUIRE(inv && index && damping_buf && out, "damping_rows: null pointer");
  GS_REQUIRE(n_rows >= 0 && hw > 0, "damping_rows: bad shape");
  if (n_rows == 0) return GS_OK;
  const size_t total = (size_t)n_rows * hw;
  damping_rows_kernel<<<(unsigned)((total + 255) / 256), 256, 0, (hipStream_t)stream>>>(eta, inv, index, damping_buf, out,
                                                                                       hw, scale, eps, total);
  GS_CHECK_LAUNCH("damping_rows");
  return GS_OK;
}
```

go_slam_amd/depth_video.py:

```python
import torch
import torch.multiprocessing as _mp

from . import droid_backends
from .droid_net import cvx_upsample


class DepthVideo:
    def __init__(self, cfg_or_ht, args_or_wd, buffer=512, device="cuda:0", stereo=False, full_res=False):
        if isinstance(cfg_or_ht, int):
            self.cfg, self.args = None, None
            mh, mw = int(cfg_or_ht), int(args_or_wd)
            shared = False
        else:
            cfg, args = cfg_or_ht, args_or_wd
            self.cfg, self.args = cfg, args
            mh, mw = cfg["cam"]["H_out"] // 8, cfg["cam"]["W_out"] // 8
            buffer, device = cfg["tracking"]["buffer"], args.device
            stereo = (cfg["mode"] == "stereo")
            full_res, shared = True, True
        self.device = torch.device(device)
        self.scale_factor = 8
        self.map_ht, self.map_wd = mh, mw
        self.ht, self.wd = (cfg["cam"]["H_out"], cfg["cam"]["W_out"]) if self.cfg is not None else (8 * mh, 8 * mw)
        self.stereo = stereo
# ... 56 lines not shown
    def _count(self):
        return int(self._counter.value)

    def _set_count(self, n):
        self._counter.value = int(n)

    def __setitem__(self, index, item):
        n = self._count()
        if isinstance(index, int) and index >= n:
            self._set_count(index + 1)
        elif torch.is_tensor(index) and int(index.max()) > n:
            self._set_count(int(index.max()) + 1)
        self.timestamp[index] = item[0]
        if hasattr(self, "images"):
            self.images[index] = item[1]
        pose, disp, depth = item[2], item[3], item[4]
        if pose is not None:
            self.poses[index] = pose
        if disp is not None:
            self.disps[index] = disp
        if depth is not None:
            if hasattr(self, "depths_gt"):
                self.depths_gt[index] = depth
            sub = depth[..., 3::8, 3::8].to(self.device)
            self.disps_sens[index] = torch.where(sub > 0, 1.0 / sub, sub)
            self.disps[index] = self.disps_sens[index].clone()
        for slot, name in ((5, "intrinsics"), (6, "fmaps"), (7, "nets"), (8, "inps")):
            if len(item) > slot and (slot > 5 or item[slot] is not None):
                getattr(self, name)[index] = item[slot]
        if len(item) > 6:
            self._run_write_hooks(index)
        if len(item) > 9 and item[9] is not None and hasattr(self, "poses_gt"):
            self.poses_gt[index] = item[9].to(self.poses_gt.device)

    def add_write_hook(self, fn):
        import weakref
        hooks = self.__dict__.setdefault("_write_hooks", [])
        hooks.append(weakref.WeakMethod(fn) if hasattr(fn, "__self__") else (lambda f=fn: f))

    def __getstate__(self):
        state = dict(self.__dict__)
        state.pop("_write_hooks", None)
        return state

    def _run_write_hooks(self, index):
        hooks = self.__dict__.get("_write_hooks")
        if hooks:
            live = []
            for h in hooks:
                fn = h()
                if fn is not None:
                    fn(index)
                    live.append(h)
            self._write_hooks = live

    def __getitem__(self, index):
        if isinstance(index, int) and index > 0:
            index = self._count() + index
        return (self.poses[index], self.disps[index], self.intrinsics[index], self.fmaps[index], self.nets[index],
                self.inps[index])

    def append(self, *item):
        self[self._count()] = item

    def get_bound(self):
        with self.mapping.get_lock():
            return self.bound[0]

    def get_mapping_item(self, index, device="cuda:0", decay=0.1):
        from .lietorch_shim import SE3
        with self.mapping.get_lock():
            image = self.images[index].permute(1, 2, 0).contiguous().to(device)
            mask = self.mask_filtered[index].clone().to(device)
            depth = 1.0 / (self.disps_filtered[index].to(device) + 1e-7)
            w2c = SE3(self.poses_filtered[index].clone()).to(device)
            c2w = (SE3(self.pose_compensate[0].clone()).to(device) * w2c.inv()).matrix()
            gt_c2w = self.poses_gt[index].clone().to(device)
            self.update_priority[index] *= decay
            self._finish_locked_section()
        return image, depth, c2w, gt_c2w, mask

    def get_mapping_items(self, indices, device="cuda:0", decay=0.1):
        from .lietorch_shim import SE3
        order = list(indices)
        uniq = list(dict.fromkeys(order))
        if not uniq:
            return {}
        t = torch.as_tensor(uniq, dtype=torch.long, device=self.images.device)
        count = {}
        for i in order:
            count[i] = count.get(i, 0) + 1
        with self.mapping.get_lock():
            images = self.images[t].permute(0, 2, 3, 1).contiguous().to(device)
            masks = self.mask_filtered[t].clone().to(device)
            depths = 1.0 / (self.disps_filtered[t].to(device) + 1e-7)
            w2c = SE3(self.poses_filtered[t].clone()).to(device)
            c2w = (SE3(self.pose_compensate[0:1].clone()).to(device) * w2c.inv()).matrix()
            gt = self.poses_gt[t].clone().to(device)
            for k in range(max(count.values())):
                sel = [i for i in uniq if count[i] > k]
                self.update_priority[torch.as_tensor(sel, dtype=torch.long, device=self.update_priority.device)] *= decay
            self._finish_locked_section()
        return {i: (images[j], depths[j], c2w[j], gt[j], masks[j]) for j, i in enumerate(uniq)}

    def normalize(self):
        with self.get_lock():
            n = self._count()
            s = self.disps[:n].mean()
            self.disps[:n] /= s
            self.poses[:n, :3] *= s
            self.dirty[:n] = True
            self._finish_locked_section()

    def _finish_locked_section(self):
        if self._shared and self.device.type == "cuda":
            torch.cuda.current_stream(self.device).synchronize()

    @staticmethod
    def format_indices(ii, jj, device="cuda"):
        if not isinstance(ii, torch.Tensor):
            ii = torch.as_tensor(ii)
        if not isinstance(jj, torch.Tensor):
            jj = torch.as_tensor(jj)
        return (ii.to(device=device, dtype=torch.long).reshape(-1).contiguous(),
                jj.to(device=device, dtype=torch.long).reshape(-1).contiguous())

    def upsample(self, ix, mask):
        if hasattr(mask, "upsample_into"):
            ix = ix.to(device=self.device, dtype=torch.long).contiguous()
            if self.disps.is_cuda and self.disps.is_contiguous() and self.disps_up.is_contiguous():
                mask.upsample_into(self.disps, ix, self.disps_up)
                return
            mask = mask.materialize()
        m = mask.reshape(-1, 576, self.map_ht, self.map_wd)
        if m.dtype == torch.float16 and m.is_cuda:
            cl = m.is_contiguous(memory_format=torch.channels_last)
            if not cl:
                m = m.contiguous()
            ix = ix.to(device=self.device, dtype=torch.long).contiguous()
            from . import _lib
            with torch.cuda.device(self.device):
                rc = _lib.lib().gs_cvx_upsample(_lib.ptr(self.disps), _lib.ptr(m), _lib.ptr(ix),
                                                _lib.ptr(self.disps_up), ix.numel(), self.map_ht, self.map_wd, int(cl),
                                                _lib.stream_ptr(self.device))
            _lib.check(rc, "DepthVideo.upsample")
            return
        up = cvx_upsample(self.disps[ix].unsqueeze(-1), mask)
        self.disps_up[ix] = up.squeeze(-1).float()

    def reproject(self, ii, jj):
        ii, jj = DepthVideo.format_indices(ii, jj, self.device)
        return droid_backends.reproject(self.poses, self.disps, self.intrinsics, ii, jj)

    def distance(self, ii=None, jj=None, beta=0.3, bidirectional=True):
        return_matrix = False
        N = self._count()
        if ii is None:
            return_matrix = True
            ii, jj = torch.meshgrid(torch.arange(N), torch.arange(N), indexing="ij")
        ii, jj = DepthVideo.format_indices(ii, jj, self.device)
        intr = self.intrinsics[0].contiguous()
        if bidirectional:
            poses = self.poses[:N].clone()
            d1 = droid_backends.frame_distance(poses, self.disps, intr, ii, jj, beta)
            d2 = droid_backends.frame_distance(poses, self.disps, intr, jj, ii, beta)
            d = 0.5 * (d1 + d2)
        else:
            d = droid_backends.frame_distance(self.poses, self.disps, intr, ii, jj, beta)
        return d.reshape(N, N) if return_matrix else d

    ba_accepts_tables = True

    def ba(self, target, weight, eta, ii, jj, t0=1, t1=None, iters=2, lm=1e-4, ep=0.1,
           motion_only=False, ba_type=None, tables=None):
        lock = self.get_lock() if ba_type is None else self.get_ba_lock(ba_type)
        with lock:
            if t1 is None:
                t1 = max(int(ii.max()), int(jj.max())) + 1
            out = droid_backends.ba(self.poses, self.disps, self.intrinsics[0].contiguous(), self.disps_sens,
                                    target, weight, eta, ii, jj, t0, t1, iters, lm, ep, motion_only, tables=tables)
            self.disps.clamp_(min=0.001)
            self._finish_locked_section()
        return out
```

go_slam_amd/droid_backends.py:

```python
import os

import torch

from . import _lib

_DT = {torch.float16: 0, torch.float32: 1, torch.float64: 2}

_ws_cache = {}
_ba_status = {}
BA_CHECK = os.environ.get("GOSLAM_BA_CHECK", "0") == "1"


def _chk(name, t, dtype=None):
    if not isinstance(t, torch.Tensor):
        raise RuntimeError(f"{name} must be a tensor")
    if not t.is_cuda:
        raise RuntimeError(f"{name} must be a GPU tensor (go_slam_amd has no CPU path)")
    if not t.is_contiguous():
        raise RuntimeError(f"{name} must be contiguous")
    if dtype is not None and t.dtype != dtype:
        raise RuntimeError(f"{name} must have dtype {dtype}, got {t.dtype}")
    return t


def _workspace(device, nbytes):
    key = (device.index, torch.cuda.current_stream(device).cuda_stream)
    buf = _ws_cache.get(key)
    if buf is None or buf.numel() < nbytes:
        buf = torch.empty(int(nbytes * 1.25) + 1024, dtype=torch.uint8, device=device)
        _ws_cache[key] = buf
    return buf


def ba(poses, disps, intrinsics, disps_sens, targets, weights, eta, ii, jj,
       t0, t1, iterations, lm, ep, motion_only, tables=None):
    _chk("targets", targets, torch.float32)
    _chk("weights", weights, torch.float32)
    _chk("poses", poses, torch.float32)
    _chk("disps", disps, torch.float32)
    _chk("intrinsics", intrinsics, torch.float32)
    _chk("disps_sens", disps_sens, torch.float32)
    _chk("ii", ii, torch.int64)
    _chk("jj", jj, torch.int64)
    if not eta.is_contiguous():
        eta = eta.contiguous()
    dev = poses.device
    nbuf, ht, wd = disps.shape
    E = ii.shape[0]
    P = int(t1) - int(t0)
    hw = ht * wd
    M = eta.reshape(-1, hw).shape[0]
    L = _lib.lib()
    need = L.gs_ba_workspace_bytes(E, P, M, nbuf, hw)
    flags = 0
    new_key = None
    if tables is None:
        ws = _workspace(dev, need + 256)
    else:
        key = (ii.data_ptr(), ii._version, jj.data_ptr(), jj._version, E, int(t0), int(t1), M, nbuf, ht, wd, dev)
        ws = tables.get("workspace")
        if ws is not None and tables.get("key") == key and ws.numel() >= need + 256:
            flags = 1
        else:
            ws = tables["workspace"] = torch.empty(need + 256, dtype=torch.uint8, device=dev)
            tables.pop("key", None)
            new_key = key
    dx = torch.empty(P, 6, dtype=torch.float32, device=dev)
    dz = None if motion_only else (torch.empty if int(iterations) > 0 else torch.zeros)(M, hw, dtype=torch.float32,
                                                                                      device=dev)
    status = _ba_status.get(dev.index)
    if status is None:
        status = _ba_status[dev.index] = torch.zeros(4, dtype=torch.int32, device=dev)
    with torch.cuda.device(dev):
        rc = L.gs_ba_ex(_lib.ptr(poses), _lib.ptr(disps), _lib.ptr(intrinsics), _lib.ptr(disps_sens),
                        _lib.ptr(targets), _lib.ptr(weights), _lib.ptr(eta), _lib.ptr(ii), _lib.ptr(jj),
                        int(t0), int(t1), int(iterations), float(lm), float(ep), int(bool(motion_only)),
                        E, M, nbuf, ht, wd, _lib.ptr(dx), _lib.ptr(dz), _lib.ptr(status),
                        _lib.ptr(ws), ws.numel(), flags, _lib.stream_ptr(dev))
    _lib.check(rc, "droid_backends.ba")
    if new_key is not None:
        tables["key"] = new_key
        tables["ii"], tables["jj"] = ii, jj
    if BA_CHECK:
        st = ba_status(dev)
        if st["depth_rows_mismatch"]:
            raise RuntimeError(f"droid_backends.ba: eta has {M} rows but the graph has {st['depth_keyframes']} depth "
                               "keyframes (unique(arange(t0, t1) U ii))")
    return [dx, dz]


def ba_status(device=None):
    dev = torch.device("cuda", torch.cuda.current_device()) if device is None else torch.device(device)
    status = _ba_status.get(dev.index if dev.index is not None else torch.cuda.current_device())
    if status is None:
        return None
    s = status.tolist()
    return {"depth_keyframes": s[0], "depth_rows_mismatch": bool(s[1]), "cholesky_failures": s[2]}


def frame_distance(poses, disps, intrinsics, ii, jj, beta):
    _chk("poses", poses, torch.float32)
    _chk("disps", disps, torch.float32)
    _chk("intrinsics", intrinsics, torch.float32)
    _chk("ii", ii, torch.int64)
    _chk("jj", jj, torch.int64)
    n = ii.shape[0]
    _, ht, wd = disps.shape
    dist = torch.empty(n, dtype=torch.float32, device=poses.device)
    with torch.cuda.device(poses.device):
        rc = _lib.lib().gs_frame_distance(_lib.ptr(poses), _lib.ptr(disps), _lib.ptr(intrinsics), _lib.ptr(ii),
                                          _lib.ptr(jj), _lib.ptr(dist), n, ht, wd, float(beta),
                                          _lib.stream_ptr(poses.device))
    _lib.check(rc, "droid_backends.frame_distance")
    return dist


def projmap(poses, disps, intrinsics, ii, jj):
    _chk("poses", poses, torch.float32)
    _chk("disps", disps, torch.float32)
    _chk("intrinsics", intrinsics, torch.float32)
    _chk("ii", ii, torch.int64)
    _chk("jj", jj, torch.int64)
    n = ii.shape[0]
    _, ht, wd = disps.shape
    coords = torch.empty(n, ht, wd, 3, dtype=torch.float32, device=poses.device)
    valid = torch.empty(n, ht, wd, 1, dtype=torch.float32, device=poses.device)
    with torch.cuda.device(poses.device):
        rc = _lib.lib().gs_projmap(_lib.ptr(poses), _lib.ptr(disps), _lib.ptr(intrinsics), _lib.ptr(ii),
                                   _lib.ptr(jj), _lib.ptr(coords), _lib.ptr(valid), n, ht, wd,
                                   _lib.stream_ptr(poses.device))
    _lib.check(rc, "droid_backends.projmap")
    return [coords, valid]


def depth_filter(poses, disps, intrinsics, ix, thresh):
    _chk("poses", poses, torch.float32)
    _chk("disps", disps, torch.float32)
    _chk("intrinsics", intrinsics, torch.float32)
    _chk("ix", ix, torch.int64)
    _chk("thresh", thresh, torch.float32)
    num, ht, wd = disps.shape
    n = ix.shape[0]
    counter = torch.empty(n, ht, wd, dtype=torch.float32, device=disps.device)
    with torch.cuda.device(disps.device):
        rc = _lib.lib().gs_depth_filter(_lib.ptr(poses), _lib.ptr(disps), _lib.ptr(intrinsics), _lib.ptr(ix),
                                        _lib.ptr(thresh), _lib.ptr(counter), n, num, ht, wd,
                                        _lib.stream_ptr(disps.device))
    _lib.check(rc, "droid_backends.depth_filter")
    return counter


def iproj(poses, disps, intrinsics):
    _chk("poses", poses, torch.float32)
    _chk("disps", disps, torch.float32)
    _chk("intrinsics", intrinsics, torch.float32)
    n, ht, wd = disps.shape
    points = torch.empty(n, ht, wd, 3, dtype=torch.float32, device=disps.device)
    with torch.cuda.device(disps.device):
        rc = _lib.lib().gs_iproj(_lib.ptr(poses), _lib.ptr(disps), _lib.ptr(intrinsics), _lib.ptr(points),
                                 n, ht, wd, _lib.stream_ptr(disps.device))
    _lib.check(rc, "droid_backends.iproj")
    return points


def corr_index_forward(volume, coords, radius):
    _chk("volume", volume)
    _chk("coords", coords, torch.float32)
    if volume.dtype not in _DT:
        raise RuntimeError(f"corr_index_forward: unsupported dtype {volume.dtype}")
    n, h1, w1, h2, w2 = volume.shape
    rd = 2 * radius + 1
    corr = torch.empty(n, rd, rd, h1, w1, dtype=volume.dtype, device=volume.device)
    with torch.cuda.device(volume.device):
        rc = _lib.lib().gs_corr_index_forward(_lib.ptr(volume), _lib.ptr(coords), _lib.ptr(corr), n, h1, w1, h2,
                                              w2, int(radius), _DT[volume.dtype],
                                              _lib.stream_ptr(volume.device))
    _lib.check(rc, "droid_backends.corr_index_forward")
    return [corr]


def corr_index_backward(volume, coords, corr_grad, radius):
    _chk("volume", volume)
    _chk("coords", coords, torch.float32)
    _chk("corr_grad", corr_grad, volume.dtype)
    n, h1, w1, h2, w2 = volume.shape
    grad = torch.zeros_like(volume)
    with torch.cuda.device(volume.device):
        rc = _lib.lib().gs_corr_index_backward(_lib.ptr(coords), _lib.ptr(corr_grad), _lib.ptr(grad), n, h1, w1,
                                               h2, w2, int(radius), _DT[volume.dtype],
                                               _lib.stream_ptr(volume.device))
    _lib.check(rc, "droid_backends.corr_index_backward")
    return [grad]


CORR_ROWMAJOR, CORR_TILE8 = 0, 1


def corr_lookup_pyramid(pyramid, coords, radius=3, channels_last=False, layout=CORR_ROWMAJOR, map_size=None):
    assert len(pyramid) == 4
    for i, v in enumerate(pyramid):
        _chk(f"pyramid[{i}]", v, pyramid[0].dtype)
    _chk("coords", coords, torch.float32)
    if layout == CORR_TILE8:
        n, h1, w1 = pyramid[0].shape[:3]
        h2, w2 = map_size
        for l in range(4):
            want = (n, h1, w1, _lib.lib().gs_corr_level_elems(h2, w2, l, layout)) if l < 2 else (n, h1, w1, h2 >> l, w2 >> l)
            if tuple(pyramid[l].shape) != want:
                raise RuntimeError(f"tile8 pyramid level {l} has shape {tuple(pyramid[l].shape)}, expected {want}")
    else:
        n, h1, w1, h2, w2 = pyramid[0].shape
        for l in range(4):
            if tuple(pyramid[l].shape) != (n, h1, w1, h2 >> l, w2 >> l):
                raise RuntimeError(f"pyramid level {l} has shape {tuple(pyramid[l].shape)}")
    rd = 2 * radius + 1
    corr = torch.empty((n, 4 * rd * rd, h1, w1), dtype=pyramid[0].dtype, device=coords.device,
                       memory_format=torch.channels_last if channels_last else torch.contiguous_format)
    with torch.cuda.device(coords.device):
        rc = _lib.lib().gs_corr_lookup_pyramid(_lib.ptr(pyramid[0]), _lib.ptr(pyramid[1]), _lib.ptr(pyramid[2]),
                                               _lib.ptr(pyramid[3]), _lib.ptr(coords), _lib.ptr(corr), n, h1, w1,
                                               h2, w2, int(radius), _DT[pyramid[0].dtype], int(bool(channels_last)),
                                               int(layout), _lib.stream_ptr(coords.device))
    _lib.check(rc, "corr_lookup_pyramid")
    return corr


def reproject(poses, disps, intrinsics, ii, jj):
    _chk("poses", poses, torch.float32)
    _chk("disps", disps, torch.float32)
    _chk("intrinsics", intrinsics, torch.float32)
    _chk("ii", ii, torch.int64)
    _chk("jj", jj, torch.int64)
    n = ii.shape[0]
    _, ht, wd = disps.shape
    coords = torch.empty(1, n, ht, wd, 2, dtype=torch.float32, device=poses.device)
    valid = torch.empty(1, n, ht, wd, 1, dtype=torch.float32, device=poses.device)
    with torch.cuda.device(poses.device):
        rc = _lib.lib().gs_reproject(_lib.ptr(poses), _lib.ptr(disps), _lib.ptr(intrinsics), _lib.ptr(ii),
                                     _lib.ptr(jj), _lib.ptr(coords), _lib.ptr(valid), n, ht, wd,
                                     _lib.stream_ptr(poses.device))
    _lib.check(rc, "reproject")
    return coords, valid


def altcorr_forward(fmap1, fmap2, coords, radius):
    _chk("fmap1", fmap1)
    _chk("fmap2", fmap2, fmap1.dtype)
    _chk("coords", coords, torch.float32)
    if fmap1.dtype not in (torch.float16, torch.float32):
        raise RuntimeError(f"altcorr_forward: unsupported dtype {fmap1.dtype}")
    B, H1, W1, C = fmap1.shape
    _, H2, W2, _ = fmap2.shape
    S = coords.shape[1]
    rd = 2 * radius + 1
    corr = torch.empty(B, S, rd * rd, H1, W1, dtype=fmap1.dtype, device=fmap1.device)
    with torch.cuda.device(fmap1.device):
        rc = _lib.lib().gs_altcorr_forward(_lib.ptr(fmap1), _lib.ptr(fmap2), _lib.ptr(coords), _lib.ptr(corr), B, S,
                                           H1, W1, H2, W2, C, int(radius), _DT[fmap1.dtype],
                                           _lib.stream_ptr(fmap1.device))
    _lib.check(rc, "droid_backends.altcorr_forward")
    return [corr]


def altcorr_backward(fmap1, fmap2, coords, corr_grad, radius):
    for name, t in (("fmap1", fmap1), ("fmap2", fmap2), ("coords", coords), ("corr_grad", corr_grad)):
        _chk(name, t, torch.float32)
    B, H1, W1, C = fmap1.shape
    _, H2, W2, _ = fmap2.shape
    S = coords.shape[1]
    g1 = torch.empty_like(fmap1)
    g2 = torch.zeros_like(fmap2)
    gc = torch.zeros_like(coords)
    with torch.cuda.device(fmap1.device):
        rc = _lib.lib().gs_altcorr_backward(_lib.ptr(fmap1), _lib.ptr(fmap2), _lib.ptr(coords), _lib.ptr(corr_grad),
                                            _lib.ptr(g1), _lib.ptr(g2), B, S, H1, W1, H2, W2, C, int(radius),
                                            _lib.stream_ptr(fmap1.device))
    _lib.check(rc, "droid_backends.altcorr_backward")
    return [g1, g2, gc]


CORR_VOLUME_MAX_W = 96


def corr_volume_supported(fmap1):
    n, dim, h, w = fmap1.shape
    return fmap1.dtype == torch.float16 and dim == 128 and h >= 8 and w % 4 == 0 and 8 <= w <= CORR_VOLUME_MAX_W


def corr_tile8_supported(fmap):
    return corr_volume_supported(fmap) and fmap.shape[-1] % 16 == 0


def corr_untile8(vol, hl, wl):
    n, h, w, plane = vol.shape
    nty, ntx = (hl + 7) // 8, (wl + 7) // 8
    t = vol.view(n, h, w, nty, ntx, 8, 8).permute(0, 1, 2, 3, 5, 4, 6).reshape(n, h, w, nty * 8, ntx * 8)
    return t[..., :hl, :wl].contiguous()


def corr_volume_pyramid(fmap1, fmap2, layout=CORR_ROWMAJOR):
    _chk("fmap1", fmap1, torch.float16)
    _chk("fmap2", fmap2, torch.float16)
    if fmap1.shape != fmap2.shape or not corr_volume_supported(fmap1):
        raise RuntimeError(f"corr_volume_pyramid: unsupported shape {tuple(fmap1.shape)} / {tuple(fmap2.shape)}")
    n, dim, h, w = fmap1.shape
    dev = fmap1.device
    L = _lib.lib()
    if layout == CORR_TILE8:
        if not corr_tile8_supported(fmap1):
            raise RuntimeError(f"corr_volume_pyramid: tile8 layout needs w % 16 == 0, got {tuple(fmap1.shape)}")
        vols = [torch.empty(n, h, w, L.gs_corr_level_elems(h, w, l, layout), dtype=torch.float16, device=dev)
                for l in range(2)]
        vols += [torch.empty(n, h, w, h >> l, w >> l, dtype=torch.float16, device=dev) for l in (2, 3)]
    else:
        vols = [torch.empty(n, h, w, h >> l, w >> l, dtype=torch.float16, device=dev) for l in range(4)]
    need = L.gs_corr_volume_workspace_bytes(n, dim, h, w)
    ws = _workspace(dev, need + 256)
    with torch.cuda.device(dev):
        rc = L.gs_corr_volume_pyramid(_lib.ptr(fmap1), _lib.ptr(fmap2), *[_lib.ptr(v) for v in vols], n, dim, h, w,
                                      int(layout), _lib.ptr(ws), ws.numel(), _lib.stream_ptr(dev))
    _lib.check(rc, "corr_volume_pyramid")
    return vols
```

go_slam_amd/droid_net.py:

```python
import os

import torch
import torch.nn as nn
import torch.nn.functional as F

from .weight_packs import WeightPacks, conv_pack, tensors_key


class GradientClip(nn.Module):

    def forward(self, x):
        return x


def segment_mean(x, index, num_segments):
    n = x.shape[0]
    onehot = torch.zeros(num_segments, n, dtype=x.dtype, device=x.device)
    onehot[index, torch.arange(n, device=x.device)] = 1
    cnt = onehot.sum(dim=1, keepdim=True).clamp(min=1)
    avg = (onehot / cnt)
    if x.is_contiguous(memory_format=torch.channels_last):
        flat = x.permute(0, 2, 3, 1).reshape(n, -1)
        out = (avg @ flat).view(num_segments, x.shape[2], x.shape[3], x.shape[1])
        return out.permute(0, 3, 1, 2)
# ... 183 lines not shown
        return conv3x3_hip(x, w)
    with torch.autocast("cuda", enabled=False):
        y = F.conv2d(x, w, None, stride=stride, padding=padding)
    if not y.is_contiguous(memory_format=torch.channels_last):
        y = y.contiguous(memory_format=torch.channels_last)
    return y


def conv_bias_act(cache, conv, x, act, out=None, out_channel=0):
    w, b = conv_pack(cache, conv, "nhwc", lambda t: t.detach().half().contiguous(memory_format=torch.channels_last))
    if GRU_FUSED_EPILOGUE and act == "relu" and _use_own_conv3x3(x, w, conv.stride, conv.padding):
        from . import _lib
        n, c, h, wd = x.shape
        O = w.shape[0]
        if out is None:
            out, out_channel = torch.empty((n, O, h, wd), dtype=torch.float16, device=x.device,
                                           memory_format=torch.channels_last), 0
        with torch.cuda.device(x.device):
            rc = _lib.lib().gs_conv3x3_bias_relu(_lib.ptr(x), c, c, _lib.ptr(conv3x3_weight_image(w, 32)), _lib.ptr(b),
                                                 out.data_ptr() + 2 * out_channel, out.shape[1], O, n, h, wd,
                                                 _lib.stream_ptr(x.device))
        _lib.check(rc, "conv3x3_bias_relu")
        return out
    y = conv_nobias(x, w, conv.stride, conv.padding)
    return bias_act(y, b, act, out, out_channel)


def copy_channels(x, out, out_channel):
    bias_act(x, None, "none", out, out_channel)


class LazyUpmask:

    def __init__(self, module, x, shape):
        self.module, self.x, self.shape_ = module, x, shape
        self._value = None

    def __getitem__(self, index):
        if index == 0 and self.shape_[0] == 1:
            return self
        return self.materialize()[index]

    def materialize(self):
        if self._value is None:
            m = self.module
            self._value = conv1x1_bias_act(m._packs, m.agg.upmask[0], self.x, "none").view(*self.shape_)
        return self._value

    def upsample_into(self, disps, ix, disps_up):
        from . import _lib
        wplain, bias = conv_pack(self.module._packs, self.module.agg.upmask[0], "plain",
                                 lambda w: w.detach().reshape(576, 128).half().contiguous())
        x = self.x
        m, c, h, w = x.shape
        assert c == 128 and x.is_contiguous(memory_format=torch.channels_last) and ix.numel() == m
        with torch.cuda.device(x.device):
            rc = _lib.lib().gs_upmask_upsample(_lib.ptr(x), 128, _lib.ptr(wplain), _lib.ptr(bias), _lib.ptr(disps),
                                               _lib.ptr(ix), _lib.ptr(disps_up), m, h, w, _lib.stream_ptr(x.device))
        _lib.check(rc, "upmask_upsample")

    def __getattr__(self, name):
        return getattr(self.materialize(), name)


class ConvGRU(nn.Module):

    def __init__(self, h_planes=128, i_planes=128):
        super().__init__()
        self.do_checkpoint = False
        self.fuse_gates = True
        c = h_planes + i_planes
        self.convz = nn.Conv2d(c, h_planes, 3, padding=1)
        self.convr = nn.Conv2d(c, h_planes, 3, padding=1)
        self.convq = nn.Conv2d(c, h_planes, 3, padding=1)
        self.w = nn.Conv2d(h_planes, h_planes, 1)
        self.convz_glo = nn.Conv2d(h_planes, h_planes, 1)
        self.convr_glo = nn.Conv2d(h_planes, h_planes, 1)
        self.convq_glo = nn.Conv2d(h_planes, h_planes, 1)
        self._packs = WeightPacks()

    def _fusable(self, net, inputs):
        cl = torch.channels_last
        return (net.is_cuda and not torch.is_grad_enabled() and net.dtype == torch.float16 and net.shape[1] == 128
                and net.is_contiguous(memory_format=cl) and all(t.dtype == torch.float16 for t in inputs))

    def _weight_tensors(self):
        mods = (self.convz, self.convr, self.convq, self.w, self.convz_glo, self.convr_glo, self.convq_glo)
        return [m.weight for m in mods] + [m.bias for m in mods]

    def _weights_key(self):
        return tensors_key(self._weight_tensors())

    def _all_packs(self):
        def build():
            cl = torch.channels_last
            wzr = torch.cat([self.convz.weight, self.convr.weight], 0).detach().half().contiguous(memory_format=cl)
            wq = self.convq.weight.detach().half().contiguous(memory_format=cl)
            bzr = torch.cat([self.convz.bias, self.convr.bias]).detach().float().contiguous()
            bq = self.convq.bias.detach().float().contiguous()
            ww = self.w.weight.detach().half().contiguous(memory_format=cl)
            bw = self.w.bias.detach().float().contiguous()
            glo = [m.weight.detach().half().reshape(128, 128).contiguous()
                   for m in (self.convz_glo, self.convr_glo, self.convq_glo)]
            glo += [m.bias.detach().float().contiguous() for m in (self.convz_glo, self.convr_glo, self.convq_glo)]
            keep = list(range(0, 128)) + list(range(256, self.convz.weight.shape[1]))
            w_all = torch.cat([self.convz.weight, self.convr.weight, self.convq.weight], 0).detach()
            hoist = (w_all[:, 128:256].half().contiguous(memory_format=cl),
                     w_all[:256][:, keep].half().contiguous(memory_format=cl),
                     w_all[256:][:, keep].half().contiguous(memory_format=cl))
            return (wzr, wq, bzr, bq, ww, bw, glo), hoist, pack_1x1_weight(self.w.weight)
        return self._packs.get("gru", self._weight_tensors(), build)

    def _half_weights(self):
        return self._all_packs()[0]

    _hw_hoist = property(lambda self: self._all_packs()[1])
    _ww_pack = property(lambda self: self._all_packs()[2])

    def _forward_fused(self, net, inputs):
        hx = torch.cat([net, *inputs], dim=1)
        if not hx.is_contiguous(memory_format=torch.channels_last):
            hx = hx.contiguous(memory_format=torch.channels_last)
        return self.forward_hx(net, hx)

    def inp_gates(self, inp):
        return conv_nobias(inp, self._hw_hoist[0], padding=1)

    def global_context(self, net):
        from . import _lib
        b, c, h, w = net.shape
        hw = h * w
        (wzr, wq, bzr, bq, ww, bw, gw), _, ww_pack = self._all_packs()
        L = _lib.lib()
        st = _lib.stream_ptr(net.device)
        dev = net.device
        gzr = torch.empty(b, 256, dtype=torch.float32, device=dev)
        gq = torch.empty(b, 128, dtype=torch.float32, device=dev)
        if GRU_GLO_FUSED:
            ws = torch.empty(L.gs_gru_glo_fused_workspace_bytes(b, hw), dtype=torch.uint8, device=dev)
            _lib.check(L.gs_gru_glo_fused(_lib.ptr(net), 128, _lib.ptr(ww_pack), _lib.ptr(bw), _lib.ptr(gw[0]),
                                          _lib.ptr(gw[1]), _lib.ptr(gw[2]), _lib.ptr(gw[3]), _lib.ptr(gw[4]),
                                          _lib.ptr(gw[5]), _lib.ptr(gzr), _lib.ptr(gq), b, hw, _lib.ptr(ws),
                                          ws.numel(), st), "gru_glo_fused")
        else:
            w_pre = torch.empty_like(net)
            _lib.check(L.gs_conv1x1(_lib.ptr(net), 128, 128, _lib.ptr(ww_pack), None, 0, _lib.ptr(w_pre), 128,
                                    128, b * hw, st), "conv1x1(gru.w)")
            ws = torch.empty(L.gs_gru_glo_workspace_bytes(b), dtype=torch.uint8, device=dev)
            _lib.check(L.gs_gru_glo(_lib.ptr(w_pre), _lib.ptr(bw), _lib.ptr(net), _lib.ptr(gw[0]), _lib.ptr(gw[1]),
                                    _lib.ptr(gw[2]), _lib.ptr(gw[3]), _lib.ptr(gw[4]), _lib.ptr(gw[5]),
                                    _lib.ptr(gzr), _lib.ptr(gq), b, hw, _lib.ptr(ws), ws.numel(), st), "gru_glo")
        return gzr, gq

    def forward_hx(self, net, hx, inp_pre=None, glo=None):
        from . import _lib
        b, c, h, w = net.shape
        hw = h * w
        (wzr, wq, bzr, bq, ww, bw, gw), hoist, _ = self._all_packs()
        if inp_pre is not None:
            wzr, wq = hoist[1], hoist[2]
        L = _lib.lib()
        st = _lib.stream_ptr(net.device)
        dev = net.device
        with torch.autocast("cuda", enabled=False):
            gzr, gq = glo if glo is not None else self.global_context(net)
            cin = hx.shape[1]
            if GRU_FUSED_EPILOGUE and _use_own_conv3x3(hx, wzr, 1, 1) and h * w > 0:
                z = torch.empty_like(net)
                rnet = torch.empty_like(net)
                out = torch.empty_like(net)
                _lib.check(L.gs_conv3x3_gru_zr2(_lib.ptr(net), hx.data_ptr() + 2 * 128, cin, cin - 128,
                                                _lib.ptr(conv3x3_weight_image(wzr, 32)), _lib.ptr(bzr), _lib.ptr(gzr),
                                                _lib.ptr(inp_pre), _lib.ptr(z), _lib.ptr(rnet), b, h, w, st),
                           "conv3x3_gru_zr2")
                _lib.check(L.gs_conv3x3_gru_q(_lib.ptr(rnet), hx.data_ptr() + 2 * 128, cin, cin - 128,
                                              _lib.ptr(conv3x3_weight_image(wq, 32)), _lib.ptr(bq), _lib.ptr(gq),
                                              _lib.ptr(inp_pre), _lib.ptr(z), _lib.ptr(net), _lib.ptr(out), b, h, w,
                                              st), "conv3x3_gru_q")
                return out
            copy_channels(net, hx, 0)
            zr_pre = conv_nobias(hx, wzr, padding=1)
            z = torch.empty_like(net)
            _lib.check(L.gs_gru_gate_zr(_lib.ptr(zr_pre), _lib.ptr(bzr), _lib.ptr(gzr), _lib.ptr(inp_pre), _lib.ptr(hx),
                                        _lib.ptr(z), b, hw, hx.shape[1], st), "gru_gate_zr")
            q_pre = conv_nobias(hx, wq, padding=1)
            out = torch.empty_like(net)
            _lib.check(L.gs_gru_gate_q(_lib.ptr(q_pre), _lib.ptr(bq), _lib.ptr(gq), _lib.ptr(inp_pre), _lib.ptr(z),
                                       _lib.ptr(net), _lib.ptr(out), b, hw, st), "gru_gate_q")
        return out

    def forward(self, net, *inputs):
        if self.fuse_gates and self._fusable(net, inputs):
            return self._forward_fused(net, inputs)
        inp = torch.cat(inputs, dim=1)
        hx = torch.cat([net, inp], dim=1)
        b, c, h, w = net.shape
        glo = (torch.sigmoid(self.w(net)) * net).view(b, c, h * w).mean(-1).view(b, c, 1, 1)
        z = torch.sigmoid(self.convz(hx) + self.convz_glo(glo))
        r = torch.sigmoid(self.convr(hx) + self.convr_glo(glo))
        q = torch.tanh(self.convq(torch.cat([r * net, inp], dim=1)) + self.convq_glo(glo))
        return (1 - z) * net + z * q


class GraphAgg(nn.Module):

    def __init__(self):
        super().__init__()
        self.conv1 = nn.Conv2d(128, 128, 3, padding=1)
        self.conv2 = nn.Conv2d(128, 128, 3, padding=1)
        self.relu = nn.ReLU(inplace=True)
        self.eta = nn.Sequential(nn.Conv2d(128, 1, 3, padding=1), GradientClip(), nn.Softplus())
        self.upmask = nn.Sequential(nn.Conv2d(128, 8 * 8 * 9, 1, padding=0))

    def forward(self, net, ii):
        batch, num, ch, ht, wd = net.shape
        x = self.relu(self.conv1(net.view(batch * num, ch, ht, wd)))
        uniq, ix = torch.unique(ii, sorted=True, return_inverse=True)
        assert batch == 1
        x = segment_mean(x, ix, uniq.numel())
        x = self.relu(self.conv2(x))
        eta = self.eta(x).view(batch, -1, ht, wd)
        upmask = self.upmask(x).view(batch, -1, 8 * 8 * 9, ht, wd)
        return 0.01 * eta, upmask


class UpdateModule(nn.Module):

    def __init__(self):
        super().__init__()
        cor_planes = 4 * (2 * 3 + 1) ** 2
        self.corr_encoder = nn.Sequential(
            nn.Conv2d(cor_planes, 128, 1), nn.ReLU(inplace=True),
            nn.Conv2d(128, 128, 3, padding=1), nn.ReLU(inplace=True))
        self.flow_encoder = nn.Sequential(
            nn.Conv2d(4, 128, 7, padding=3), nn.ReLU(inplace=True),
            nn.Conv2d(128, 64, 3, padding=1), nn.ReLU(inplace=True))
        self.weight = nn.Sequential(
            nn.Conv2d(128, 128, 3, padding=1), nn.ReLU(inplace=True),
            nn.Conv2d(128, 2, 3, padding=1), GradientClip(), nn.Sigmoid())
        self.delta = nn.Sequential(
            nn.Conv2d(128, 128, 3, padding=1), nn.ReLU(inplace=True),
            nn.Conv2d(128, 2, 3, padding=1), GradientClip())
        self.gru = ConvGRU(128, 128 + 128 + 64)
        self.agg = GraphAgg()
        self.fuse_epilogues = True
        self._packs = WeightPacks()

    def drop_edge_caches(self):
        self._inp_pre_cache = None

    invalidate_context = drop_edge_caches

    INP_CACHE_BYTES = 16 << 30
    INP_CACHE_ENTRIES = 64
    cache_check = os.environ.get("GOSLAM_CACHE_CHECK", "0") == "1"

    @staticmethod
    def _checksum(inp):
        flat = inp.detach().reshape(-1)
        if flat.dtype in (torch.float16, torch.bfloat16):
            flat = flat.view(torch.int16)
        elif flat.dtype == torch.float32:
            flat = flat.view(torch.int32)
        w = (torch.arange(flat.numel(), device=flat.device, dtype=torch.int64) % 8191) + 1
        return int((flat.to(torch.int64) * w).sum())

    _device_caps = {}

    def _cache_cap(self, device):
        cap = self.INP_CACHE_BYTES
        if device.type == "cuda":
            idx = device.index if device.index is not None else torch.cuda.current_device()
            dev_cap = UpdateModule._device_caps.get(idx)
            if dev_cap is None:
                try:
                    dev_cap = torch.cuda.mem_get_info(device)[1] // 8
                except RuntimeError:
                    dev_cap = cap
                UpdateModule._device_caps[idx] = dev_cap
            cap = min(cap, dev_cap)
        return cap

    def _edge_state(self, inp, n, ht, wd):
        import collections
        import weakref
        hx = getattr(self, "_hx", None)
        if hx is None or hx.shape[0] != n or hx.shape[2:] != (ht, wd) or hx.device != inp.device:
            hx = torch.empty((n, 320, ht, wd), dtype=torch.float16, device=inp.device,
                             memory_format=torch.channels_last)
            self._hx = hx
        cache = getattr(self, "_inp_pre_cache", None)
        if cache is None:
            cache = self._inp_pre_cache = collections.OrderedDict()
        wkey = self.gru._weights_key()
        owner = inp._base if inp._base is not None else inp
        key = (inp.data_ptr(), tuple(inp.shape), tuple(inp.stride()), inp.dtype)
        ent = cache.get(key)
        if ent is not None and ent[0]() is owner and ent[1] == inp._version and ent[2] == wkey:
            if self.cache_check and ent[4] != self._checksum(inp):
                raise RuntimeError("UpdateModule: the context features `inp` were modified behind the version counter "
                                   "(raw-pointer write?) while their hoisted convolution was cached; call "
                                   "update.invalidate_context() after such writes")
            cache.move_to_end(key)
            return hx, ent[3]
        inp4 = inp.view(n, -1, ht, wd)
        if inp4.dtype != torch.float16 or not inp4.is_contiguous(memory_format=torch.channels_last):
            inp4 = inp4.half().contiguous(memory_format=torch.channels_last)
        try:
            inp_pre = self.gru.inp_gates(inp4)
        except torch.OutOfMemoryError:
            cache.clear()
            torch.cuda.empty_cache()
            inp_pre = self.gru.inp_gates(inp4)
        for k in [k for k, e in cache.items() if e[2] != wkey or e[0]() is None]:
            del cache[k]

        def _gone(_ref, key=key, cache_ref=weakref.ref(cache)):
            c = cache_ref()
            if c is not None:
                e = c.get(key)
                if e is not None and e[0] is _ref:
                    del c[key]
        cache[key] = (weakref.ref(owner, _gone), inp._version, wkey, inp_pre,
                      self._checksum(inp) if self.cache_check else None)
        nbytes = lambda e: sum(x.numel() * x.element_size()
                               for x in (e[3] if isinstance(e[3], (tuple, list)) else (e[3],)) if torch.is_tensor(x))
        total = sum(nbytes(e) for e in cache.values())
        cap = self._cache_cap(inp.device)
        while (total > cap or len(cache) > self.INP_CACHE_ENTRIES) and len(cache) > 1:
            _, e = cache.popitem(last=False)
            total -= nbytes(e)
        return hx, inp_pre

    def _head_weights(self):
        mods = (self.delta[0], self.weight[0], self.agg.conv1)

        def build():
            w = torch.cat([m.weight for m in mods], 0).detach().half().contiguous(memory_format=torch.channels_last)
            return w, [m.bias.detach().float().contiguous() for m in mods]
        return self._packs.get("heads", [m.weight for m in mods] + [m.bias for m in mods], build)

    def _corr_independent_part(self, net4, inp, f4, n, ht, wd):
        hx, inp_pre = self._edge_state(inp, n, ht, wd)
        if CONV7X7_OWN and conv7x7_c4_supported(self.flow_encoder[0], f4):
            f4 = conv7x7_c4_bias_act(self._packs, self.flow_encoder[0], f4, "relu")
        else:
            f4 = conv_bias_act(self._packs, self.flow_encoder[0], f4, "relu")
        conv_bias_act(self._packs, self.flow_encoder[2], f4, "relu", out=hx, out_channel=256)
        with torch.autocast("cuda", enabled=False):
            glo = self.gru.global_context(net4)
        return hx, inp_pre, glo

    def _forward_fast(self, net, inp, corr, flow, ii, jj, seg=None):
        batch, num, ch, ht, wd = net.shape
        cl = torch.channels_last
        packs = self._packs
        out_dim = (batch, num, -1, ht, wd)
        n = batch * num
        net4 = net.view(n, -1, ht, wd)
        from .corr import LazyLookup
        lazy = corr if isinstance(corr, LazyLookup) and FUSE_LOOKUP_ENCODER and corr.block.fused_encoder_supported() \
            else None
        if lazy is None:
            if isinstance(corr, LazyLookup):
                corr = corr.materialize()
            c4 = corr.view(n, -1, ht, wd).half().contiguous(memory_format=cl)
        if flow is None:
            flow = torch.zeros(batch, num, 4, ht, wd, device=net.device)
        f4 = flow.view(n, -1, ht, wd).half().contiguous(memory_format=cl)
        hx, inp_pre, glo = self._corr_independent_part(net4, inp, f4, n, ht, wd)
        if lazy is not None:
            c4 = lazy.encoded(*self._corr_enc0_padded())
        else:
            c4 = conv1x1_bias_act(packs, self.corr_encoder[0], c4, "relu")
        conv_bias_act(packs, self.corr_encoder[2], c4, "relu", out=hx, out_channel=128)
        net4 = self.gru.forward_hx(net4, hx, inp_pre, glo=glo)
        net = net4.view(*out_dim)
        hw_, hb = self._head_weights()
        heads = conv_nobias(net4, hw_ if ii is not None else hw_[:256], padding=1)
        delta = conv3x3_head(heads, self.delta[2], packs, "none", in_channel=0, in_bias=hb[0], in_relu=True)
        weight = conv3x3_head(heads, self.weight[2], packs, "sigmoid", in_channel=128, in_bias=hb[1], in_relu=True)
        delta, weight = delta.view(batch, num, ht, wd, 2), weight.view(batch, num, ht, wd, 2)
        if ii is None:
            return net, delta, weight
        agg = self.agg
        if seg is None:
            seg = build_segments(ii.to(net.device))
        x = segment_mean_hip(heads, seg, in_channel=256, channels=128, in_bias=hb[2], in_relu=True)
        x = conv_bias_act(packs, agg.conv2, x, "relu")
        eta = conv3x3_head(x, agg.eta[0], packs, "softplus", out_scale=0.01).view(batch, -1, ht, wd)
        if FUSE_UPMASK_UPSAMPLE:
            upmask = LazyUpmask(self, x, (batch, -1, 8 * 8 * 9, ht, wd))
        else:
            upmask = conv1x1_bias_act(packs, agg.upmask[0], x, "none").view(batch, -1, 8 * 8 * 9, ht, wd)
        return net, delta, weight, eta, upmask

    def _corr_enc0_padded(self):
        def pad(weight):
            w = torch.zeros(128, 208, dtype=torch.float16, device=weight.device)
            w[:, :196] = weight.detach().reshape(128, 196).half()
            return w
        return conv_pack(self._packs, self.corr_encoder[0], "pad208", pad)

    def _fast_ok(self, net, inp, corr):
        cl = torch.channels_last
        n4 = net.view(-1, *net.shape[2:])
        return (self.fuse_epilogues and net.is_cuda and not torch.is_grad_enabled() and net.dtype == torch.float16
                and net.shape[2] == 128 and n4.is_contiguous(memory_format=cl) and torch.is_autocast_enabled())

    def forward(self, net, inp, corr, flow=None, ii=None, jj=None, seg=None):
        batch, num, ch, ht, wd = net.shape
        if self._fast_ok(net, inp, corr):
            return self._forward_fast(net, inp, corr, flow, ii, jj, seg)
        if hasattr(corr, "materialize"):
            corr = corr.materialize()
        if flow is None:
            flow = torch.zeros(batch, num, 4, ht, wd, device=net.device)
        out_dim = (batch, num, -1, ht, wd)
        net = net.view(batch * num, -1, ht, wd)
        inp = inp.view(batch * num, -1, ht, wd)
        corr = self.corr_encoder(corr.view(batch * num, -1, ht, wd))
        flow = self.flow_encoder(flow.view(batch * num, -1, ht, wd))
        net = self.gru(net, inp, corr, flow)
        delta = self.delta(net).view(*out_dim).permute(0, 1, 3, 4, 2)[..., :2].contiguous()
        weight = self.weight(net).view(*out_dim).permute(0, 1, 3, 4, 2)[..., :2].contiguous()
        net = net.view(*out_dim)
        if ii is not None:
            eta, upmask = self.agg(net, ii.to(net.device))
            return net, delta, weight, eta, upmask
        return net, delta, weight


class DroidNet(nn.Module):

    def __init__(self):
        super().__init__()
        from .extractor import BasicEncoder
        self.fnet = BasicEncoder(out_dim=128, norm_fn="instance")
        self.cnet = BasicEncoder(out_dim=256, norm_fn="none")
        self.update = UpdateModule()


def load_pretrained(net, state_dict):
    sd = {k.replace("module.", ""): v for k, v in state_dict.items()}
    for head in ("weight", "delta"):
        for p in ("weight", "bias"):
            k = f"update.{head}.2.{p}"
            sd[k] = sd[k][:2]
    net.load_state_dict(sd)
    return net
```

go_slam_amd/factor_graph.py:

```python
import numpy as np
import torch

from .corr import AltCorrBlock, CorrBlock, CorrPool

def coords_grid(ht, wd, device):
    y, x = torch.meshgrid(torch.arange(ht, device=device).float(), torch.arange(wd, device=device).float(),
                          indexing="ij")
    return torch.stack([x, y], dim=-1)


def _segments_np(index):
    uniq, ix = np.unique(index, return_inverse=True)
    ix = ix.reshape(-1).astype(np.int64)
    order = np.argsort(ix, kind="stable").astype(np.int32)
    offsets = np.zeros(uniq.size + 1, dtype=np.int32)
    offsets[1:] = np.cumsum(np.bincount(ix, minlength=uniq.size))
    return {"uniq": uniq.astype(np.int64), "ix": ix, "offsets": offsets, "order": order, "n": int(uniq.size)}


def _as_tensors(d):
    return {k: (torch.from_numpy(np.ascontiguousarray(v)) if isinstance(v, np.ndarray) else v) for k, v in d.items()}


def upload_tables(host, device):
# ... 193 lines not shown
        if ii.numel() == 0 or self.ii.numel() + self.ii_inac.numel() == 0:
            return ii, jj
        if ii.is_cuda:
            have = torch.cat([self.ii, self.ii_inac]) * (1 << 20) + torch.cat([self.jj, self.jj_inac])
            keep = torch.nonzero(~torch.isin(ii * (1 << 20) + jj, have)).reshape(-1)
            if keep.numel() == ii.numel():
                return ii, jj
            return ii.index_select(0, keep), jj.index_select(0, keep)
        have = set(self._edges_on_host((self.ii, self.jj), (self.ii_inac, self.jj_inac)))
        keep = torch.tensor([e not in have for e in zip(ii.cpu().tolist(), jj.cpu().tolist())],
                            dtype=torch.bool, device=ii.device)
        return ii[keep], jj[keep]

    @torch.no_grad()
    def filter_edges(self):
        conf = self.weight.mean(dim=(0, 2, 3, 4))
        mask = ((self.ii - self.jj).abs() > 2) & (conf < 1e-3)
        self.ii_bad = torch.cat([self.ii_bad, self.ii[mask]])
        self.jj_bad = torch.cat([self.jj_bad, self.jj[mask]])
        self.rm_factors(mask, store=False)

    @torch.no_grad()
    def clear_edges(self):
        if self.ii.numel():
            if self.corr_impl == "volume" and self.corr is not None:
                self.corr = self.corr[torch.zeros(0, dtype=torch.long, device=self.ii.device)]
            self.ii, self.jj, self.age = (x.new_empty((0,)) for x in (self.ii, self.jj, self.age))
            self.target, self.weight = (x.new_empty((x.shape[0], 0) + tuple(x.shape[2:])) for x in (self.target, self.weight))
        self.net = None
        self.inp = None

    _KEYFRAME_BUFFERS = ("timestamp", "images", "dirty", "red", "poses", "poses_gt", "disps", "disps_sens",
                         "disps_up", "depths_gt", "intrinsics", "poses_filtered", "disps_filtered",
                         "mask_filtered", "update_priority", "nets", "inps", "fmaps")

    @torch.no_grad()
    def rm_keyframe(self, ix):
        v = self.video
        for name in self._KEYFRAME_BUFFERS:
            buf = getattr(v, name, None)
            if torch.is_tensor(buf):
                buf[ix] = buf[ix + 1]
        m = (self.ii_inac == ix) | (self.jj_inac == ix)
        self.ii_inac = self.ii_inac - (self.ii_inac >= ix).long()
        self.jj_inac = self.jj_inac - (self.jj_inac >= ix).long()
        if bool(m.any()):
            keep = ~m
            self.ii_inac, self.jj_inac = self.ii_inac[keep], self.jj_inac[keep]
            self.target_inac, self.weight_inac = self.target_inac[:, keep], self.weight_inac[:, keep]
        m = (self.ii == ix) | (self.jj == ix)
        self.ii = self.ii - (self.ii >= ix).long()
        self.jj = self.jj - (self.jj >= ix).long()
        self.rm_factors(m, store=False)

    def add_neighborhood_factors(self, t0, t1, r=3):
        ii, jj = torch.meshgrid(torch.arange(t0, t1), torch.arange(t0, t1), indexing="ij")
        ii, jj = ii.reshape(-1), jj.reshape(-1)
        c = 1 if getattr(self.video, "stereo", False) else 0
        keep = ((ii - jj).abs() > c) & ((ii - jj).abs() <= r)
        self.add_factors(ii[keep].to(self.device), jj[keep].to(self.device))

    @staticmethod
    def propose_proximity_edges(d, existing, t0, t1, t, rad, nms, thresh, max_factors, stereo):
        import numpy as np
        ilen, jlen = t - t0, t - t1

        def suppress(di, dj):
            d[max(0, di - nms):min(ilen, di + nms + 1), max(0, dj - nms):min(jlen, dj + nms + 1)] = np.inf

        for i, j in existing:
            if t0 <= i < t and t1 <= j < t:
                d[i - t0, j - t1] = np.inf
                suppress(i - t0, j - t1)
        es = []
        for i in range(t0, t):
            if stereo:
                es.append((i, i))
                d[i - t0, i - t1] = np.inf
            for j in range(max(i - rad, 0), i):
                es += [(i, j), (j, i)]
                d[i - t0, j - t1] = np.inf
                suppress(i - t0, j - t1)
        flat = d.reshape(-1)
        order = np.argsort(flat, kind="stable")
        order = order[flat[order] <= thresh]
        for k in order.tolist():
            di, dj = k // jlen, k % jlen
            if d[di, dj] > thresh:
                continue
            if len(es) > max_factors:
                break
            i, j = t0 + di, t1 + dj
            es += [(i, j), (j, i)]
            suppress(di, dj)
        return es

    @staticmethod
    def propose_edges_on_device(raw, existing, i0, j0, t, rad, nms, cut, thresh, max_factors, stereo, jmin, loop):
        from . import _lib
        dev = raw.device
        n_local = sum((1 if stereo else 0) + 2 * max(i - max(i - rad, jmin), 0) for i in range(i0, t))
        cap = n_local + max(int(max_factors), 0) + 16
        raw = raw.detach().float().contiguous()
        d_work = torch.empty_like(raw)
        es = torch.zeros(cap, 2, dtype=torch.long, device=dev)
        count = torch.zeros(1, dtype=torch.int32, device=dev)
        ex_i, ex_j = (None, None) if existing is None else (existing[0].long().contiguous(), existing[1].long().contiguous())
        n_ex = 0 if existing is None else int(ex_i.numel())
        L, st = _lib.lib(), _lib.stream_ptr(dev)
        with torch.cuda.device(dev):
            _lib.check(L.gs_edge_prep(_lib.ptr(raw), _lib.ptr(d_work), _lib.ptr(ex_i), _lib.ptr(ex_j), n_ex, _lib.ptr(es),
                                      _lib.ptr(count), cap, i0, j0, t, rad, nms, float(cut), int(bool(stereo)), jmin, st),
                       "edge_prep")
            vals, order = torch.sort(d_work, stable=True)
            _lib.check(L.gs_edge_greedy(_lib.ptr(raw), _lib.ptr(vals), _lib.ptr(order), _lib.ptr(es), _lib.ptr(count), cap,
                                        i0, j0, t, nms, float(thresh), int(max_factors), int(bool(loop)), st),
                       "edge_greedy")
        return es[:int(count)]

    @torch.no_grad()
    def add_proximity_factors(self, t0=0, t1=0, rad=2, nms=2, beta=0.25, thresh=16.0, remove=False, max_t=None):
        cnt = self.video.counter
        t = max_t if max_t is not None else int(getattr(cnt, "value", cnt))
        if t <= t0 or t <= t1:
            return
        vdev = torch.device(self.device)
        ii, jj = torch.meshgrid(torch.arange(t0, t, device=vdev), torch.arange(t1, t, device=vdev), indexing="ij")
        ii, jj = ii.reshape(-1), jj.reshape(-1)
        d_dev = self.video.distance(ii, jj, beta=beta)
        if d_dev.is_cuda and (t - t0) * (t - t1) <= 512 * 512:
            existing = (torch.cat([self.ii, self.ii_bad, self.ii_inac]), torch.cat([self.jj, self.jj_bad, self.jj_inac]))
            e = FactorGraph.propose_edges_on_device(d_dev, existing, t0, t1, t, rad, nms, 100.0, thresh, self.max_factors,
                                                    bool(getattr(self.video, "stereo", False)), 0, False)
            if e.shape[0]:
                self.add_factors(e[:, 0].contiguous(), e[:, 1].contiguous(), remove)
            return
        d = d_dev.detach().float().cpu()
        ii, jj = ii.cpu(), jj.cpu()
        d[ii - rad < jj] = float("inf")
        d[d > 100] = float("inf")
        d = d.reshape(t - t0, t - t1).numpy().copy()
        existing = self._edges_on_host((self.ii, self.jj), (self.ii_bad, self.jj_bad), (self.ii_inac, self.jj_inac))
        es = FactorGraph.propose_proximity_edges(d, existing, t0, t1, t, rad, nms, thresh, self.max_factors,
                                                 bool(getattr(self.video, "stereo", False)))
        if not es:
            return
        e = torch.tensor(es, dtype=torch.long, device=self.device)
        self.add_factors(e[:, 0], e[:, 1], remove)

    @torch.no_grad()
    def update(self, t0=None, t1=None, iters=2, use_inactive=False, EPS=1e-7, motion_only=False):
        idx = self._edge_index(t0, t1, use_inactive)
        t0, t1, seg = idx["t0"], idx["t1"], idx["seg"]
        coords1, mask = self.video.reproject(self.ii, self.jj)
        fused = self._glue_fusable(coords1)
        ht, wd = self.ht, self.wd
        E = self.ii.numel()
        if fused:
            from . import _lib
            L, st = _lib.lib(), _lib.stream_ptr(self.device)
            m4 = torch.empty(E, ht, wd, 4, dtype=torch.float16, device=self.device)
            _lib.check(L.gs_motion_features(_lib.ptr(coords1), _lib.ptr(self.target), _lib.ptr(m4), E, ht, wd, st),
                       "motion_features")
            motion = m4.permute(0, 3, 1, 2).unsqueeze(0)
        else:
            motion = torch.cat([coords1 - self.coords0, self.target - coords1], dim=-1)
            motion = motion.permute(0, 1, 4, 2, 3).clamp(-64.0, 64.0)

        corr = self.corr.lazy(coords1) if hasattr(self.corr, "lazy") else self.corr(coords1)
        with torch.autocast("cuda", dtype=torch.float16):
            self.net, delta, weight, damping, upmask = self.update_op(
                self.net, self.inp, corr, motion, self.ii, self.jj, seg=seg)

        fuse_damping = fused and damping.dtype == torch.float32 and damping.is_contiguous() and \
            self.damping.is_contiguous() and damping.shape[1] == idx["uniq_host"].numel()
        if not fuse_damping:
            self.damping[seg["uniq"]] = damping.float()
        eta_rows = damping
        if fused and delta.dtype == torch.float32 and weight.dtype == torch.float32:
            bt, bw, n_in = self._ba_buffers(idx, use_inactive)
            target_new = torch.empty_like(coords1)
            _lib.check(L.gs_ba_inputs(_lib.ptr(coords1), _lib.ptr(delta.contiguous()), _lib.ptr(weight.contiguous()),
                                      _lib.ptr(target_new), bt[n_in:].data_ptr(), bw[n_in:].data_ptr(), E, ht, wd, st),
                       "ba_inputs")
            self.target, self.weight = target_new, weight
            target, weight = bt, bw
        else:
            self.target = coords1 + delta.float()
            self.weight = weight.float()
            if use_inactive:
                sel = idx["sel"]
                target = torch.cat([self.target_inac[:, sel], self.target], 1)
                weight = torch.cat([self.weight_inac[:, sel], self.weight], 1)
            else:
                target, weight = self.target, self.weight
            target = target.view(-1, ht, wd, 2).permute(0, 3, 1, 2).contiguous()
            weight = weight.view(-1, ht, wd, 2).permute(0, 3, 1, 2).contiguous()

        if fuse_damping:
            damping = torch.empty(idx["damping_index"].numel(), ht, wd, device=self.device)
            _lib.check(L.gs_damping_rows(_lib.ptr(eta_rows), _lib.ptr(idx["damping_inv"]), _lib.ptr(idx["damping_index"]),
                                         _lib.ptr(self.damping), _lib.ptr(damping), damping.shape[0], ht * wd, 0.2,
                                         float(EPS), st), "damping_rows")
        else:
            damping = 0.2 * self.damping[idx["damping_index"]].contiguous() + EPS

        tables = idx.setdefault("ba_tables", {}) if getattr(self.video, "ba_accepts_tables", False) else None
        if tables is None:
            self.video.ba(target, weight, damping, idx["ii"], idx["jj"], t0=t0, t1=t1, iters=iters,
                          lm=1e-4, ep=0.1, motion_only=motion_only)
        else:
            self.video.ba(target, weight, damping, idx["ii"], idx["jj"], t0=t0, t1=t1, iters=iters,
                          lm=1e-4, ep=0.1, motion_only=motion_only, tables=tables)
        if self.upsample:
            self.video.upsample(seg["uniq"], upmask[0])
        self.age += 1

    def _select_edges(self, x5, sel):
        x4 = x5[0]
        if self.channels_last and x4.is_contiguous(memory_format=torch.channels_last):
            return x4.permute(0, 2, 3, 1).index_select(0, sel).permute(0, 3, 1, 2).unsqueeze(0)
        return x4.index_select(0, sel).unsqueeze(0)

    def _lowmem_index(self, t0, t1, rig):
        tens = (self.ii, self.jj)
        key = tuple(x._version for x in tens) + (t0, t1, rig, getattr(getattr(self.video, "inps", None), "_version", 0))
        c = getattr(self, "_lidx", None)
        if c is not None and c["key"] == key and all(a is b for a, b in zip(c["tens"], tens)):
            return c
        dev = self.device
        host = torch.stack([self.ii, self.jj]).cpu().numpy()
        ii_c, jj_c = host[0], host[1]
        a0 = max(1, int(ii_c.min()) + 1) if t0 is None else t0
        a0 = max(1, a0)
        a1 = (max(int(ii_c.max()), int(jj_c.max())) + 1) if t1 is None else t1
        chunks, up, segs = [], {}, []
        s = 13
        for i in range(int(ii_c.min()), int(ii_c.max()) + 1, s):
            sel = np.nonzero((ii_c >= i) & (ii_c < i + s))[0].astype(np.int64)
            if sel.size < 1:
                continue
            iis, jjs = ii_c[sel], jj_c[sel]
            n = len(segs)
            up.update({f"{n}.sel": sel, f"{n}.ii": iis, f"{n}.jj": jjs, f"{n}.corr_ii": rig * iis,
                       f"{n}.corr_jj": rig * jjs + (iis == jjs).astype(np.int64), f"{n}.uniq": np.unique(iis)})
            segs.append(_segments_np(iis))
            up.update({f"{n}.seg.{k}": v for k, v in segs[-1].items() if isinstance(v, np.ndarray)})
        up["damping_index"] = np.unique(np.concatenate([np.arange(a0, a1, dtype=np.int64), ii_c]))
        up = _as_tensors(up)
        up = upload_tables(up, dev)
        for n, seg_h in enumerate(segs):
            ck = {k: up[f"{n}.{k}"] for k in ("sel", "ii", "jj", "corr_ii", "corr_jj", "uniq")}
            seg = {k: (up[f"{n}.seg.{k}"] if isinstance(v, np.ndarray) else v) for k, v in seg_h.items()}
            ck["seg_kw"] = {"seg": seg} if getattr(self.update_op, "_forward_fast", None) is not None else {}
            def _inp(ix=ck["ii"], box=ck):
                v = box.get("inp_cached")
                if v is None:
                    v = box["inp_cached"] = self._fmt(self.video.inps[ix]).unsqueeze(0)
                return v
            ck["inp"] = _inp
            chunks.append(ck)
        c = {"key": key, "tens": tens, "t0": a0, "t1": a1, "chunks": chunks, "ii": self.ii.contiguous(),
             "jj": self.jj.contiguous(), "damping_index": up["damping_index"]}
        self._lidx = c
        return c

    @torch.no_grad()
    def update_lowmem(self, t0=None, t1=None, iters=2, use_inactive=False, EPS=1e-7, steps=8, max_t=None,
                      ba_type="dense", motion_only=False):
        cur_t = self.video.counter
        cur_t = int(getattr(cur_t, "value", cur_t))
        t = max_t if max_t is not None else cur_t
        fm = self.video.fmaps[:cur_t + 2]
        num, rig, ch, ht, wd = fm.shape
        corr_op = AltCorrBlock(fm.reshape(1, num * rig, ch, ht, wd))
        lookup = getattr(corr_op, "lookup", corr_op)
        idx = self._lowmem_index(t0, t1, rig)
        t0, t1 = idx["t0"], idx["t1"]
        ii_all, jj_all = idx["ii"], idx["jj"]
        cl = torch.channels_last
        for _ in range(steps):
            coords1, mask = self.video.reproject(ii_all, jj_all)
            fast = (coords1.is_cuda and self.channels_last and coords1.dtype == torch.float32 and coords1.is_contiguous()
                    and self.target.dtype == torch.float32 and self.target.is_contiguous()
                    and self.weight.dtype == torch.float32 and self.weight.is_contiguous()
                    and self.net.dtype == torch.float16 and self.net[0].is_contiguous(memory_format=cl)
                    and self.net.shape[2] == 128
                    and tuple(self.target.shape) == tuple(coords1.shape) == tuple(self.weight.shape))
            if fast:
                from . import _lib
                L, st = _lib.lib(), _lib.stream_ptr(self.device)
                ht, wd = self.ht, self.wd
            else:
                motion = torch.cat([coords1 - self.coords0, self.target - coords1], dim=-1)
                motion = motion.permute(0, 1, 4, 2, 3).clamp(-64.0, 64.0)
            for ck in idx["chunks"]:
                sel, iis, jjs = ck["sel"], ck["ii"], ck["jj"]
                if fast:
                    n = sel.numel()
                    c1 = torch.empty(1, n, ht, wd, 2, dtype=torch.float32, device=self.device)
                    m4 = torch.empty(n, ht, wd, 4, dtype=torch.float16, device=self.device)
                    net_c = torch.empty(n, ht, wd, 128, dtype=torch.float16, device=self.device)
                    _lib.check(L.gs_lowmem_gather(_lib.ptr(coords1), _lib.ptr(self.target), _lib.ptr(self.net),
                                                  _lib.ptr(sel), _lib.ptr(c1), _lib.ptr(m4), _lib.ptr(net_c), n, ht, wd, st),
                               "lowmem_gather")
                    net_in = net_c.permute(0, 3, 1, 2).unsqueeze(0)
                    motion_c = m4.permute(0, 3, 1, 2).unsqueeze(0)
                else:
                    c1 = coords1.index_select(1, sel)
                    net_in, motion_c = self._select_edges(self.net, sel), motion.index_select(1, sel)
                corr1 = lookup(c1, ck["corr_ii"], ck["corr_jj"])
                with torch.autocast("cuda", dtype=torch.float16):
                    net, delta, weight, damping, upmask = self.update_op(
                        net_in, ck["inp"](), corr1, motion_c, iis, jjs, **ck["seg_kw"])
                    if self.upsample:
                        self.video.upsample(ck["uniq"], upmask[0])
                if fast and net.dtype == torch.float16 and net[0].is_contiguous(memory_format=cl) \
                        and tuple(net.shape) == (1, sel.numel(), 128, ht, wd) \
                        and delta.dtype == torch.float32 and weight.dtype == torch.float32 \
                        and tuple(delta.shape) == tuple(weight.shape) == (1, sel.numel(), ht, wd, 2):
                    delta_c, weight_c = delta.contiguous(), weight.contiguous()
                    _lib.check(L.gs_lowmem_scatter(_lib.ptr(c1), _lib.ptr(delta_c), _lib.ptr(weight_c),
                                                   _lib.ptr(net), _lib.ptr(sel), _lib.ptr(self.target), _lib.ptr(self.weight),
                                                   _lib.ptr(self.net), sel.numel(), ht, wd, st), "lowmem_scatter")
                else:
                    self.net[:, sel] = net.to(self.net.dtype)
                    self.target[:, sel] = c1 + delta.float()
                    self.weight[:, sel] = weight.float()
                self.damping[ck["uniq"]] = damping.float()
            damping = 0.2 * self.damping[idx["damping_index"]].contiguous() + EPS
            target = self.target.view(-1, self.ht, self.wd, 2).permute(0, 3, 1, 2).contiguous()
            weight = self.weight.view(-1, self.ht, self.wd, 2).permute(0, 3, 1, 2).contiguous()
            lm, ep = (1e-4, 1e-1) if ba_type == "loop" else (1e-5, 1e-2)
            kw = {"tables": idx.setdefault("ba_tables", {})} if getattr(self.video, "ba_accepts_tables", False) else {}
            self.video.ba(target, weight, damping, ii_all, jj_all, t0=t0, t1=t1,
                          iters=iters, lm=lm, ep=ep, motion_only=motion_only, ba_type=ba_type, **kw)
            self.video.dirty[:t] = True
```

include/goslam_hip.h:

```cpp
#ifndef GOSLAM_HIP_H
#define GOSLAM_HIP_H

#include <stddef.h>
#include <stdint.h>

#ifdef __cplusplus
extern "C" {
#endif

typedef void* gs_stream_t;

typedef enum {
  GS_OK = 0,
  GS_ERR_INVALID_ARG = -1,
  GS_ERR_WORKSPACE = -2,
  GS_ERR_LAUNCH = -3,
  GS_ERR_UNSUPPORTED = -4
} gs_status;

typedef enum { GS_F16 = 0, GS_F32 = 1, GS_F64 = 2 } gs_dtype;

const char* gs_version(void);
const char* gs_last_error(void);

int gs_timing_begin(gs_stream_t stream);
int gs_timing_end(void);
int gs_timing_read(const char* name, double* total_ms, int* count);
int gs_timing_names(char* buf, int buf_bytes);


int gs_corr_index_forward(const void* volume, const float* coords, void* corr,
                          int n, int h1, int w1, int h2, int w2, int radius, int dtype,
                          gs_stream_t stream);

int gs_corr_index_backward(const float* coords, const void* corr_grad, void* volume_grad,
                           int n, int h1, int w1, int h2, int w2, int radius, int dtype,
                           gs_stream_t stream);

#define GS_CORR_ROWMAJOR 0
#define GS_CORR_TILE8 1
int gs_corr_lookup_pyramid(const void* vol0, const void* vol1, const void* vol2, const void* vol3,
                           const float* coords, void* corr,
                           int n, int h1, int w1, int h2, int w2, int radius, int dtype,
                           int channels_last, int layout, gs_stream_t stream);
int gs_corr_lookup_enc(const void* vol0, const void* vol1, const void* vol2, const void* vol3, const float* coords,
                       const void* wpad, const float* bias, void* y, int y_stride, int n, int h1, int w1, int h2,
                       int w2, int layout, gs_stream_t stream);
int gs_corr_lookup_enc_slots(const void* vol0, const void* vol1, const void* vol2, const void* vol3, const int64_t* slot,
                             const float* coords, const void* wpad, const float* bias, void* y, int y_stride, int n,
                             int h1, int w1, int h2, int w2, int layout, gs_stream_t stream);
int gs_corr_lookup_pyramid_slots(const void* vol0, const void* vol1, const void* vol2, const void* vol3,
                                 const int64_t* slot, const float* coords, void* corr, int n, int h1, int w1, int h2,
                                 int w2, int radius, int dtype, int channels_last, int layout, gs_stream_t stream);

size_t gs_corr_volume_workspace_bytes(int n, int dim, int h, int w);
size_t gs_corr_level_elems(int h, int w, int level, int layout);
int gs_corr_volume_pyramid(const void* fmap1, const void* fmap2, void* vol0, void* vol1, void* vol2,
                           void* vol3, int n, int dim, int h, int w, int layout,
                           void* workspace, size_t workspace_bytes, gs_stream_t stream);
int gs_corr_volume_pyramid_slots(const void* fmap1, const void* fmap2, void* vol0, void* vol1, void* vol2,
                                 void* vol3, const int64_t* out_slot, int n, int dim, int h, int w, int layout,
                                 void* workspace, size_t workspace_bytes, gs_stream_t stream);

int gs_altcorr_forward(const void* fmap1, const void* fmap2, const float* coords, void* corr,
                       int b, int s, int h1, int w1, int h2, int w2, int c, int radius, int dtype,
                       gs_stream_t stream);

int gs_altcorr_backward(const float* fmap1, const float* fmap2, const float* coords, const float* corr_grad,
                        float* fmap1_grad, float* fmap2_grad, int b, int s, int h1, int w1, int h2, int w2,
                        int c, int radius, gs_stream_t stream);

int gs_altcorr_pyramid(const void* pyr0, const void* pyr1, const void* pyr2, const void* pyr3, const float* coords,
                       const int64_t* ii, const int64_t* jj, void* out, int e, int h, int w, int c, int radius,
                       gs_stream_t stream);


int gs_reproject(const float* poses, const float* disps, const float* intrinsics,
                 const int64_t* ii, const int64_t* jj, float* coords, float* valid,
                 int n, int h, int w, gs_stream_t stream);

int gs_projmap(const float* poses, const float* disps, const float* intrinsics,
               const int64_t* ii, const int64_t* jj, float* coords, float* valid,
               int n, int h, int w, gs_stream_t stream);

int gs_frame_distance(const float* poses, const float* disps, const float* intrinsics,
                      const int64_t* ii, const int64_t* jj, float* dist,
                      int n, int h, int w, float beta, gs_stream_t stream);

int gs_iproj(const float* poses, const float* disps, const float* intrinsics, float* points,
             int n, int h, int w, gs_stream_t stream);

int gs_depth_filter(const float* poses, const float* disps, const float* intrinsics,
                    const int64_t* ix, const float* thresh, float* counter,
                    int n, int num, int h, int w, gs_stream_t stream);

size_t gs_pointcloud_workspace_bytes(int k, int h, int w);
int gs_pointcloud_count(const float* poses, const float* disps, const float* intrinsics, const int64_t* index,
                        const float* disp_floor, float thresh, float visible_num, int k, int num, int h, int w,
                        void* workspace, size_t workspace_bytes, gs_stream_t stream);
int gs_pointcloud_mask(const float* mask, const int64_t* index, int k, int num, int h, int w, void* workspace,
                       size_t workspace_bytes, gs_stream_t stream);
int gs_pointcloud_scan(int k, int h, int w, void* workspace, size_t workspace_bytes, long long* offsets,
                       gs_stream_t stream);
int gs_pointcloud_emit(const float* poses_inv, const float* disps, const float* intrinsics, const float* images,
                       const int64_t* index, int k, int num, int h, int w, const void* workspace,
                       size_t workspace_bytes, long long n_points, float* points, float* colors, gs_stream_t stream);

#define GS_FRAME_PREP_MAX_VIEWS 32
typedef struct {
  const uint8_t* src;
  const float* map_x;
  const float* map_y;
  uint8_t* tmp;
  float* dst;
  int h, w, c, mh, mw;
} gs_color_view;
typedef struct {
  const uint16_t* src;
  float* dst;
  int h, w;
} gs_depth_view;
int gs_frame_prep_color(const gs_color_view* views_host, int n, int H_out, int W_out, int H_edge, int W_edge,
                        gs_stream_t stream);
int gs_frame_prep_depth(const gs_depth_view* views_host, int n, float scale, int H_out, int W_out, int H_edge,
                        int W_edge, gs_stream_t stream);


int gs_gru_gate_zr(const void* zr_pre, const float* bias_zr, const float* glo_zr, const void* inp_pre, void* hx,
                   void* z_out, int n, int hw, int ldx, gs_stream_t stream);
int gs_gru_gate_q(const void* q_pre, const float* bias_q, const float* glo_q, const void* inp_pre, const void* z,
                  const void* net, void* net_out, int n, int hw, gs_stream_t stream);
int gs_bias_act(const void* x, const float* bias, void* y, int rows, int channels, int x_stride, int y_stride,
                int act, gs_stream_t stream);
int gs_motion_features(const float* coords1, const float* target, void* out, int n, int h, int w,
                       gs_stream_t stream);
int gs_lowmem_gather(const float* coords1, const float* target, const void* net, const int64_t* sel,
                     float* coords_out, void* motion_out, void* net_out, int n_sel, int h, int w, gs_stream_t stream);
int gs_lowmem_scatter(const float* coords, const float* delta, const float* weight, const void* net_new,
                      const int64_t* sel, float* target, float* weight_all, void* net, int n_sel, int h, int w,
                      gs_stream_t stream);

int gs_ba_inputs(const float* coords1, const float* delta, const float* weight, float* target,
                 float* ba_target, float* ba_weight, int n, int h, int w, gs_stream_t stream);
int gs_conv1x1(const void* x, int x_stride, int k_in, const void* wpack, const float* bias, int act, void* y,
               int y_stride, int n_out, long long rows, gs_stream_t stream);
int gs_conv7x7_c4(const void* x, const void* wpack, const float* bias, void* y, int ys, int n, int h, int w, int relu,
                  int rt, gs_stream_t stream);
size_t gs_conv3x3_wpack_elems(int c_in, int n_out);
int gs_conv3x3_pp(const void* x, int x_stride, int c_in, const void* wpack, int tw, void* y, int y_stride, int n_out,
                  int n, int h, int w, int xcd_order, gs_stream_t stream);
int gs_conv3x3_bias_relu(const void* x, int x_stride, int c_in, const void* wpack, const float* bias, void* y,
                         int y_stride, int n_out, int n, int h, int w, gs_stream_t stream);
int gs_conv3x3_gru_zr2(const void* net, const void* x_rest, int x_rest_stride, int c_rest, const void* wpack,
                       const float* bias_zr, const float* glo_zr, const void* inp_pre, void* z_out, void* rnet_out,
                       int n, int h, int w, gs_stream_t stream);
int gs_conv3x3_gru_zr(const void* hx, int hx_stride, int c_in, const void* wpack, const float* bias_zr,
                      const float* glo_zr, const void* inp_pre, void* z_out, void* rnet_out, int n, int h, int w,
                      gs_stream_t stream);
int gs_conv3x3_gru_q(const void* rnet, const void* x_rest, int x_rest_stride, int c_rest, const void* wpack,
                     const float* bias_q, const float* glo_q, const void* inp_pre, const void* z, const void* net,
                     void* net_out, int n, int h, int w, gs_stream_t stream);
int gs_conv3x3_head(const void* x, int x_stride, const float* in_bias, int in_relu, const void* wpack,
                    const float* bias, int n_out, int epilogue, float out_scale, float* out, int n, int h, int w,
                    gs_stream_t stream);
int gs_segment_mean(const void* x, int x_stride, const float* in_bias, int in_relu, const int* seg_offsets,
                    const int* seg_edges, void* out, int n_seg, int hw, int channels, gs_stream_t stream);
size_t gs_norm_act_workspace_bytes(int n, int hw, int channels);
size_t gs_norm_act_workspace_bytes_chunks(int n, int chunks, int channels);
size_t gs_enc_conv_wpack_elems(int ksize, int c_in, int c_out);
int gs_enc_conv_stat_chunks(int h_out, int w_out, int c_out);
int gs_enc_conv(const void* x, int x_stride, int c_in, const void* wpack, const void* bias, void* y, int y_stride,
                int c_out, int ksize, int stride, int n, int h, int w, const void* stat_bias, void* stats_ws,
                gs_stream_t stream);
int gs_norm_act(const void* x, const void* bias, const void* skip, void* y, int n, int hw, int channels,
                int instance_norm, int relu_in, int relu_out, float eps, void* workspace, size_t workspace_bytes,
                int stat_chunks, gs_stream_t stream);
size_t gs_gru_glo_workspace_bytes(int n);
int gs_gru_glo(const void* w_pre, const float* w_bias, const void* net, const void* wz, const void* wr,
               const void* wq, const float* bz, const float* br, const float* bq, float* gzr, float* gq,
               int n, int hw, void* workspace, size_t workspace_bytes, gs_stream_t stream);

size_t gs_gru_glo_fused_workspace_bytes(int n, int hw);
int gs_gru_glo_fused(const void* net, int net_stride, const void* w_pack, const float* w_bias, const void* wz,
                     const void* wr, const void* wq, const float* bz, const float* br, const float* bq, float* gzr,
                     float* gq, int n, int hw, void* workspace, size_t workspace_bytes, gs_stream_t stream);

int gs_damping_rows(const float* eta, const int* inv, const int64_t* index, float* damping_buf, float* out,
                    int n_rows, int hw, float scale, float eps, gs_stream_t stream);

int gs_cvx_upsample(const float* disps, const void* mask, const int64_t* ix, float* out,
                    int m, int h, int w, int mask_channels_last, gs_stream_t stream);
int gs_upmask_upsample(const void* x, int x_stride, const void* weight, const float* bias, const float* disps,
                       const int64_t* ix, float* out, int m, int h, int w, gs_stream_t stream);


size_t gs_ba_workspace_bytes(int n_edges, int n_poses, int n_depth, int nbuf, int hw);

int gs_ba(float* poses, float* disps, const float* intrinsics, const float* disps_sens,
          const float* targets, const float* weights, const float* eta,
          const int64_t* ii, const int64_t* jj,
          int t0, int t1, int iterations, float lm, float ep, int motion_only,
          int n_edges, int n_depth, int nbuf, int h, int w,
          float* dx, float* dz, int32_t* status_out,
          void* workspace, size_t workspace_bytes, gs_stream_t stream);

#define GS_BA_REUSE_TABLES 1
int gs_ba_ex(float* poses, float* disps, const float* intrinsics, const float* disps_sens,
             const float* targets, const float* weights, const float* eta,
             const int64_t* ii, const int64_t* jj,
             int t0, int t1, int iterations, float lm, float ep, int motion_only,
             int n_edges, int n_depth, int nbuf, int h, int w,
             float* dx, float* dz, int32_t* status_out,
             void* workspace, size_t workspace_bytes, int flags, gs_stream_t stream);

int gs_chol_solve(double* H, double* b, int n, float lm, float ep, int path, float* dx, int32_t* status,
                  gs_stream_t stream);

int gs_edge_prep(const float* raw, float* d_work, const long long* ex_i, const long long* ex_j, int n_existing,
                 long long* es, int* count, int cap, int i0, int j0, int t, int rad, int nms, float cut, int stereo,
                 int jmin, gs_stream_t stream);
int gs_edge_greedy(const float* raw, const float* sorted_vals, const long long* order, long long* es, int* count,
                   int cap, int i0, int j0, int t, int nms, float thresh, int max_factors, int loop, gs_stream_t stream);

size_t gs_traj_eval_workspace_bytes(int n);
int gs_traj_world(const float* w2c, const float* compensate, int n, double* tq, double* mat, gs_stream_t stream);
int gs_ape_moments(const double* est, const double* ref, const unsigned char* mask, int n, double* moments,
                   void* workspace, size_t workspace_bytes, gs_stream_t stream);
int gs_ape_stats(const double* est, const double* ref, const unsigned char* mask, const double* sim, int n,
                 double* err, double* stats, void* workspace, size_t workspace_bytes, gs_stream_t stream);

#ifdef __cplusplus
}
#endif
#endif
```

Baseline: 79.62 keyframes/s.

## Fuse small BA, reprojection, damping and GRU input kernels to cut launches

Several small launches are folded into neighbouring kernels. Motion features are computed inside reprojection, and damping rows plus the age increment are folded into the BA input prep. The H clear, status write and disparity clamp move into the BA update kernel, and the GRU conv epilogues read per-source input rows through a pre_row index instead of a gathered copy. The goal is less launch and host overhead and fewer intermediate tensors in a launch-bound small-window workload, at the cost of more complex kernels and signature changes with optional trailing arguments.

Measured after the change: 78.68 keyframes/s. 0.988x the previous value.

```diff
diff --git a/go_slam_amd/_lib.py b/go_slam_amd/_lib.py
--- a/go_slam_amd/_lib.py
+++ b/go_slam_amd/_lib.py
@@ -36,6 +36,7 @@
     "gs_altcorr_forward": (c_int, [_P] * 4 + [c_int] * 9 + [_P]),
     "gs_altcorr_pyramid": (c_int, [_P] * 8 + [c_int] * 5 + [_P]),
     "gs_reproject": (c_int, [_P] * 7 + [c_int] * 3 + [_P]),
+    "gs_reproject_motion": (c_int, [_P] * 9 + [c_int] * 3 + [_P]),
     "gs_projmap": (c_int, [_P] * 7 + [c_int] * 3 + [_P]),
     "gs_frame_distance": (c_int, [_P] * 6 + [c_int] * 3 + [c_float, _P]),
     "gs_iproj": (c_int, [_P] * 4 + [c_int] * 3 + [_P]),
@@ -55,14 +56,15 @@
     "gs_lowmem_gather": (c_int, [_P] * 7 + [c_int, c_int, c_int, _P]),
     "gs_lowmem_scatter": (c_int, [_P] * 8 + [c_int, c_int, c_int, _P]),
     "gs_damping_rows": (c_int, [_P] * 5 + [c_int, c_int, c_float, c_float, _P]),
+    "gs_ba_inputs_damping": (c_int, [_P] * 6 + [c_int] * 3 + [_P] * 5 + [c_int, c_float, c_float, _P, _P]),
     "gs_conv1x1": (c_int, [_P, c_int, c_int, _P, _P, c_int, _P, c_int, c_int, ctypes.c_longlong, _P]),
     "gs_conv7x7_c4": (c_int, [_P, _P, _P, _P, c_int, c_int, c_int, c_int, c_int, c_int, _P]),
     "gs_conv3x3_wpack_elems": (c_size_t, [c_int, c_int]),
     "gs_conv3x3_pp": (c_int, [_P, c_int, c_int, _P, c_int, _P, c_int, c_int, c_int, c_int, c_int, c_int, _P]),
     "gs_conv3x3_bias_relu": (c_int, [_P, c_int, c_int, _P, _P, _P, c_int, c_int, c_int, c_int, c_int, _P]),
     "gs_conv3x3_gru_zr": (c_int, [_P, c_int, c_int, _P, _P, _P, _P, _P, _P, c_int, c_int, c_int, _P]),
-    "gs_conv3x3_gru_zr2": (c_int, [_P, _P, c_int, c_int, _P, _P, _P, _P, _P, _P, c_int, c_int, c_int, _P]),
-    "gs_conv3x3_gru_q": (c_int, [_P, _P, c_int, c_int, _P, _P, _P, _P, _P, _P, _P, c_int, c_int, c_int, _P]),
+    "gs_conv3x3_gru_zr2": (c_int, [_P, _P, c_int, c_int, _P, _P, _P, _P, _P, _P, c_int, c_int, c_int, _P, _P]),
+    "gs_conv3x3_gru_q": (c_int, [_P, _P, c_int, c_int, _P, _P, _P, _P, _P, _P, _P, c_int, c_int, c_int, _P, _P]),
     "gs_conv3x3_head": (c_int, [_P, c_int, _P, c_int, _P, _P, c_int, c_int, c_float, _P, c_int, c_int, c_int, _P]),
     "gs_segment_mean": (c_int, [_P, c_int, _P, c_int, _P, _P, _P, c_int, c_int, c_int, _P]),
     "gs_norm_act_workspace_bytes": (c_size_t, [c_int, c_int, c_int]),
@@ -77,7 +79,7 @@
     "gs_edge_greedy": (c_int, [_P] * 5 + [c_int] * 5 + [c_float, c_int, c_int, _P]),
     "gs_ba_workspace_bytes": (c_size_t, [c_int] * 5),
     "gs_ba": (c_int, [_P] * 9 + [c_int] * 3 + [c_float, c_float] + [c_int] * 6 + [_P, _P, _P, _P, c_size_t, _P]),
-    "gs_ba_ex": (c_int, [_P] * 9 + [c_int] * 3 + [c_float, c_float] + [c_int] * 6 + [_P, _P, _P, _P, c_size_t, c_int, _P]),
+    "gs_ba_ex": (c_int, [_P] * 9 + [c_int] * 3 + [c_float, c_float] + [c_int] * 6 + [_P, _P, _P, _P, c_size_t, c_int, c_float, _P]),
     "gs_chol_solve": (c_int, [_P, _P, c_int, c_float, c_float, c_int, _P, _P, _P]),
     "gs_traj_eval_workspace_bytes": (c_size_t, [c_int]),
     "gs_traj_world": (c_int, [_P, _P, c_int, _P, _P, _P]),
@@ -152,6 +154,18 @@
 }
 
 
+OPTIONAL_TRAILING = {"gs_conv3x3_gru_zr2": 1, "gs_conv3x3_gru_q": 1}
+
+
+def _pad_trailing(fn, n_args, n_optional):
+    def call(*args):
+        if n_args - n_optional <= len(args) < n_args:
+            args = args + (None,) * (n_args - len(args))
+        return fn(*args)
+    call.__name__ = fn.__name__
+    return call
+
+
 class ColorView(ctypes.Structure):
     _fields_ = [("src", c_void_p), ("map_x", c_void_p), ("map_y", c_void_p), ("tmp", c_void_p), ("dst", c_void_p),
                 ("h", c_int), ("w", c_int), ("c", c_int), ("mh", c_int), ("mw", c_int)]
@@ -197,6 +211,8 @@
             fn = getattr(handle, name)
             fn.restype = res
             fn.argtypes = args
+            if name in OPTIONAL_TRAILING:
+                setattr(handle, name, _pad_trailing(fn, len(args), OPTIONAL_TRAILING[name]))
         _lib = handle
     return _lib
 
diff --git a/go_slam_amd/csrc/ba.hip b/go_slam_amd/csrc/ba.hip
--- a/go_slam_amd/csrc/ba.hip
+++ b/go_slam_amd/csrc/ba.hip
@@ -488,13 +488,29 @@
   }
 }
 
+struct BaTail {
+  size_t clear_n;
+  int32_t* status_out;
+  float clamp_min;
+};
+
+__device__ __forceinline__ void ba_write_status(int32_t* status_out, const BaWs& w, int tid) {
+  if (tid < 4) status_out[tid] = (tid == 2) ? w.hdr[3] : (tid == 3 ? w.hdr[4] : w.hdr[tid]);
+}
+
 __global__ __launch_bounds__(256) void ba_update_kernel(
     float* __restrict__ poses, float* __restrict__ disps, const float* __restrict__ dx,
-    float* __restrict__ dz, int M, int t0, int t1, int hw, BaWs w) {
+    float* __restrict__ dz, int M, int t0, int t1, int hw, BaTail tail, BaWs w) {
   const int tid = threadIdx.x;
   const int P = t1 - t0;
+  if (tail.clear_n) {
+    const size_t stride = (size_t)gridDim.x * gridDim.y * 256;
+    for (size_t g = ((size_t)blockIdx.y * gridDim.x + blockIdx.x) * 256 + tid; g < tail.clear_n; g += stride) w.H[g] = 0.0;
+  }
+  const bool clamp = tail.clamp_min > 0.0f;
   if ((int)blockIdx.y == M) {
     if (blockIdx.x != 0) return;
+    if (tail.status_out) ba_write_status(tail.status_out, w, tid);
     for (int kk = t0 + tid; kk < t1; kk += 256) {
       float* pp = poses + (size_t)kk * 7;
       float t[3] = {pp[0], pp[1], pp[2]};
@@ -508,9 +524,17 @@
     }
     return;
   }
-  const int m = blockIdx.y;
   const int p = blockIdx.x * 256 + tid;
   if (p >= hw) return;
+  if ((int)blockIdx.y > M) {
+    const int f = (int)blockIdx.y - M - 1;
+    if (M > 0 && w.kinv[f] >= 0) return;
+    float* d = disps + (size_t)f * hw + p;
+    const float v = *d;
+    if (v < tail.clamp_min) *d = tail.clamp_min;
+    return;
+  }
+  const int m = blockIdx.y;
   if (m >= w.hdr[0]) {
     dz[(size_t)m * hw + p] = 0.0f;
     return;
@@ -531,12 +555,12 @@
   const float z = w.Q[o] * (w.W[o] - dw);
   dz[o] = z;
   const size_t dk = (size_t)w.kx[m] * hw + p;
-  disps[dk] = disps[dk] + z;
-}
-
-__global__ void ba_status_kernel(int32_t* status_out, BaWs w) {
-  if (threadIdx.x < 4) status_out[threadIdx.x] = (threadIdx.x == 2) ? w.hdr[3] : (threadIdx.x == 3 ? w.hdr[4] : w.hdr[threadIdx.x]);
-}
+  float d = disps[dk] + z;
+  if (clamp && d < tail.clamp_min) d = tail.clamp_min;
+  disps[dk] = d;
+}
+
+__global__ void ba_status_kernel(int32_t* status_out, BaWs w) { ba_write_status(status_out, w, threadIdx.x); }
 
 }
 
@@ -549,11 +573,13 @@
                         const float* targets, const float* weights, const float* eta, const int64_t* ii,
                         const int64_t* jj, int t0, int t1, int iterations, float lm, float ep, int motion_only,
                         int n_edges, int n_depth, int nbuf, int h, int w, float* dx, float* dz,
-                        int32_t* status_out, void* workspace, size_t workspace_bytes, int flags, gs_stream_t stream) {
+                        int32_t* status_out, void* workspace, size_t workspace_bytes, int flags, float clamp_min,
+                        gs_stream_t stream) {
   GS_REQUIRE(poses && disps && intrinsics && disps_sens && targets && weights && ii && jj && dx && workspace,
              "ba: null pointer");
   GS_REQUIRE(motion_only || (eta && dz), "ba: eta/dz required unless motion_only");
   GS_REQUIRE(h > 0 && w > 0 && n_edges >= 0 && iterations >= 0, "ba: bad shape");
+  GS_REQUIRE(clamp_min >= 0.0f, "ba: clamp_min must be >= 0 (0 = no clamp)");
   GS_REQUIRE(t0 >= 0 && t1 > t0 && t1 <= nbuf, "ba: window [%d,%d) outside buffer of %d frames", t0, t1, nbuf);
   GS_REQUIRE(nbuf <= kMaxBuf, "ba: buffer of %d frames exceeds the supported %d", nbuf, kMaxBuf);
   GS_REQUIRE(n_depth > 0 && n_depth <= nbuf && n_depth <= 65534, "ba: n_depth=%d out of range", n_depth);
@@ -575,7 +601,7 @@
   }
   const int chunks = gs_cdiv(hw, 256);
   for (int it = 0; it < iterations; ++it) {
-    if (hipMemsetAsync(ws.H, 0, ((size_t)n6 * n6 + n6) * sizeof(double), st) != hipSuccess) {
+    if (it == 0 && hipMemsetAsync(ws.H, 0, ((size_t)n6 * n6 + n6) * sizeof(double), st) != hipSuccess) {
       gs_set_error("ba: memset failed");
       return GS_ERR_LAUNCH;
     }
@@ -594,13 +620,17 @@
     }
     int rc = gs_chol_solve_launch(ws.H, ws.b, n6, lm, ep, dx, &ws.hdr[2], &ws.hdr[3], st);
     if (rc != GS_OK) return rc;
-    if (motion_only)
-      ba_update_kernel<<<dim3(1, 1), 256, 0, st>>>(poses, disps, dx, dz, 0, t0, t1, hw, ws);
-    else
-      ba_update_kernel<<<dim3(chunks, M + 1), 256, 0, st>>>(poses, disps, dx, dz, M, t0, t1, hw, ws);
+    const bool last = it + 1 == iterations;
+    BaTail tail;
+    tail.clear_n = last ? 0 : (size_t)n6 * n6 + n6;
+    tail.status_out = last ? status_out : nullptr;
+    tail.clamp_min = last ? clamp_min : 0.0f;
+    const int rows = (motion_only ? 0 : M) + 1 + (tail.clamp_min > 0.0f ? nbuf : 0);
+    const int gx = (motion_only && rows == 1 && !tail.clear_n) ? 1 : chunks;
+    ba_update_kernel<<<dim3(gx, rows), 256, 0, st>>>(poses, disps, dx, dz, motion_only ? 0 : M, t0, t1, hw, tail, ws);
     GS_CHECK_LAUNCH("ba_update");
   }
-  if (status_out) {
+  if (status_out && iterations == 0) {
     ba_status_kernel<<<1, 64, 0, st>>>(status_out, ws);
     GS_CHECK_LAUNCH("ba_status");
   }
@@ -613,5 +643,6 @@
                      int n_edges, int n_depth, int nbuf, int h, int w, float* dx, float* dz,
                      int32_t* status_out, void* workspace, size_t workspace_bytes, gs_stream_t stream) {
   return gs_ba_ex(poses, disps, intrinsics, disps_sens, targets, weights, eta, ii, jj, t0, t1, iterations, lm, ep,
-                  motion_only, n_edges, n_depth, nbuf, h, w, dx, dz, status_out, workspace, workspace_bytes, 0, stream);
-}
+                  motion_only, n_edges, n_depth, nbuf, h, w, dx, dz, status_out, workspace, workspace_bytes, 0, 0.0f,
+                  stream);
+}
diff --git a/go_slam_amd/csrc/conv3x3_pp.hip b/go_slam_amd/csrc/conv3x3_pp.hip
--- a/go_slam_amd/csrc/conv3x3_pp.hip
+++ b/go_slam_amd/csrc/conv3x3_pp.hip
@@ -35,6 +35,7 @@
   const float* bias;
   const float* glo;
   const _Float16* inp_pre;
+  const int* pre_row;
   const _Float16* aux0;
   const _Float16* aux1;
   _Float16* out0;
@@ -258,6 +259,7 @@
 #pragma unroll
   for (int i = 0; i < 4; ++i) {
     size_t pix4[NIT];
+    int img4[NIT];
     bool ok4[NIT];
     half8 pi4[NIT], u4[NIT], v4[NIT];
     const int piece = lane & (PIECES - 1);
@@ -274,11 +276,14 @@
         const half8 z8 = {0, 0, 0, 0, 0, 0, 0, 0};
         pi4[it] = z8; u4[it] = z8; v4[it] = z8;
         if (ok4[it]) {
+          const unsigned ihw = (unsigned)(H * W), upix = (unsigned)pix4[it];
+          img4[it] = (int)(upix / ihw);
+          const size_t ppix = ep.pre_row ? (size_t)ep.pre_row[img4[it]] * ihw + (upix - (unsigned)img4[it] * ihw) : pix4[it];
           if constexpr (EPI == 1) {
-            if (ep.inp_pre) pi4[it] = *reinterpret_cast<const half8*>(ep.inp_pre + pix4[it] * 384 + nb * 128 + c8);
+            if (ep.inp_pre) pi4[it] = *reinterpret_cast<const half8*>(ep.inp_pre + ppix * 384 + nb * 128 + c8);
             if (nb == 1) u4[it] = *reinterpret_cast<const half8*>(x + pix4[it] * xs + c8);
           } else {
-            if (ep.inp_pre) pi4[it] = *reinterpret_cast<const half8*>(ep.inp_pre + pix4[it] * 384 + 256 + c8);
+            if (ep.inp_pre) pi4[it] = *reinterpret_cast<const half8*>(ep.inp_pre + ppix * 384 + 256 + c8);
             u4[it] = *reinterpret_cast<const half8*>(ep.aux0 + pix4[it] * 128 + c8);
             v4[it] = *reinterpret_cast<const half8*>(ep.aux1 + pix4[it] * 128 + c8);
           }
@@ -312,7 +317,7 @@
           for (int k = 0; k < 8; ++k) o[k] = (_Float16)fmaxf((float)v[k] + bb[k], 0.0f);
           *reinterpret_cast<half8*>(yb + pix * ys + piece * 8) = o;
         } else if constexpr (EPI == 1) {
-          const int img = (int)(pix / ((size_t)H * W));
+          const int img = img4[it];
           const half8 pi = pi4[it];
           const float* bb = ep.bias + nb * 128 + c8;
           const float* gg = ep.glo + (size_t)img * 256 + nb * 128 + c8;
@@ -329,7 +334,7 @@
             *reinterpret_cast<half8*>(ep.out1 + pix * 128 + c8) = o;
           }
         } else {
-          const int img = (int)(pix / ((size_t)H * W));
+          const int img = img4[it];
           const half8 pi = pi4[it], zz = u4[it], nn = v4[it];
           const float* bb = ep.bias + c8;
           const float* gg = ep.glo + (size_t)img * 128 + c8;
@@ -424,7 +429,7 @@
 
 extern "C" int gs_conv3x3_gru_zr2(const void* net, const void* x_rest, int x_rest_stride, int c_rest, const void* wpack,
                                   const float* bias_zr, const float* glo_zr, const void* inp_pre, void* z_out,
-                                  void* rnet_out, int n, int h, int w, gs_stream_t stream) {
+                                  void* rnet_out, int n, int h, int w, gs_stream_t stream, const int* pre_row) {
   GS_REQUIRE(net && x_rest && wpack && bias_zr && glo_zr && z_out && rnet_out, "conv3x3_gru_zr2: null pointer");
   GS_REQUIRE(c_rest > 0 && c_rest % 32 == 0, "conv3x3_gru_zr2: c_rest must be a multiple of 32");
   GS_REQUIRE(x_rest_stride >= c_rest && x_rest_stride % 8 == 0, "conv3x3_gru_zr2: bad x_rest_stride");
@@ -436,6 +441,7 @@
   ep.inp_pre = (const _Float16*)inp_pre;
   ep.out0 = (_Float16*)z_out;
   ep.out1 = (_Float16*)rnet_out;
+  ep.pre_row = pre_row;
   ep.xb = (const _Float16*)x_rest;
   ep.xsb = x_rest_stride;
   ep.split = 128;
@@ -445,7 +451,8 @@
 
 extern "C" int gs_conv3x3_gru_q(const void* rnet, const void* x_rest, int x_rest_stride, int c_rest, const void* wpack,
                                 const float* bias_q, const float* glo_q, const void* inp_pre, const void* z,
-                                const void* net, void* net_out, int n, int h, int w, gs_stream_t stream) {
+                                const void* net, void* net_out, int n, int h, int w, gs_stream_t stream,
+                                const int* pre_row) {
   GS_REQUIRE(rnet && x_rest && wpack && bias_q && glo_q && z && net && net_out, "conv3x3_gru_q: null pointer");
   GS_REQUIRE(c_rest > 0 && c_rest % 32 == 0, "conv3x3_gru_q: c_rest must be a multiple of 32");
   GS_REQUIRE(x_rest_stride >= c_rest && x_rest_stride % 8 == 0, "conv3x3_gru_q: bad x_rest_stride");
@@ -458,6 +465,7 @@
   ep.aux0 = (const _Float16*)z;
   ep.aux1 = (const _Float16*)net;
   ep.out0 = (_Float16*)net_out;
+  ep.pre_row = pre_row;
   ep.xb = (const _Float16*)x_rest;
   ep.xsb = x_rest_stride;
   ep.split = 128;
diff --git a/go_slam_amd/csrc/geom.hip b/go_slam_amd/csrc/geom.hip
--- a/go_slam_amd/csrc/geom.hip
+++ b/go_slam_amd/csrc/geom.hip
@@ -5,10 +5,11 @@
 constexpr float kMinDepthKernel = 0.25f;
 constexpr float kMinDepthPy = 0.2f;
 
+template <bool MOTION>
 __global__ __launch_bounds__(256) void reproject_kernel(
     const float* __restrict__ poses, const float* __restrict__ disps, const float* __restrict__ intr,
     const int64_t* __restrict__ ii, const int64_t* __restrict__ jj, float* __restrict__ coords,
-    float* __restrict__ valid, int hw, int wd) {
+    float* __restrict__ valid, int hw, int wd, const float2* __restrict__ target, _Float16* __restrict__ motion) {
   const int p = blockIdx.x * 256 + threadIdx.x;
   const int e = blockIdx.y;
   if (p >= hw) return;
@@ -37,8 +38,19 @@
   gs_act_se3(tij, qij, X0, X1);
   const float Z = (X1[2] < 0.5f * kMinDepthPy) ? 1.0f : X1[2];
   const size_t o = (size_t)e * hw + p;
-  reinterpret_cast<float2*>(coords)[o] = make_float2(fxj * (X1[0] / Z) + cxj, fyj * (X1[1] / Z) + cyj);
+  const float2 c = make_float2(fxj * (X1[0] / Z) + cxj, fyj * (X1[1] / Z) + cyj);
+  reinterpret_cast<float2*>(coords)[o] = c;
   valid[o] = ((X1[2] > kMinDepthPy) && (X0[2] > kMinDepthPy)) ? 1.0f : 0.0f;
+  if constexpr (MOTION) {
+    const float2 tg = target[o];
+    typedef _Float16 half4m __attribute__((ext_vector_type(4)));
+    half4m m;
+    m[0] = (_Float16)fminf(fmaxf(c.x - u, -64.0f), 64.0f);
+    m[1] = (_Float16)fminf(fmaxf(c.y - v, -64.0f), 64.0f);
+    m[2] = (_Float16)fminf(fmaxf(tg.x - c.x, -64.0f), 64.0f);
+    m[3] = (_Float16)fminf(fmaxf(tg.y - c.y, -64.0f), 64.0f);
+    reinterpret_cast<half4m*>(motion)[o] = m;
+  }
 }
 
 __global__ __launch_bounds__(256) void projmap_kernel(
@@ -152,8 +164,22 @@
   GS_REQUIRE(poses && disps && intrinsics && ii && jj && coords && valid, "reproject: null pointer");
   GS_GEOM_COMMON("reproject");
   GS_REQUIRE(n <= 65535, "reproject: n=%d exceeds grid.y limit", n);
-  reproject_kernel<<<dim3(gs_cdiv(hw, 256), n), 256, 0, st>>>(poses, disps, intrinsics, ii, jj, coords, valid, hw, w);
+  reproject_kernel<false><<<dim3(gs_cdiv(hw, 256), n), 256, 0, st>>>(poses, disps, intrinsics, ii, jj, coords, valid, hw,
+                                                                     w, nullptr, nullptr);
   GS_CHECK_LAUNCH("reproject");
+  return GS_OK;
+}
+
+extern "C" int gs_reproject_motion(const float* poses, const float* disps, const float* intrinsics, const int64_t* ii,
+                                   const int64_t* jj, const float* target, float* coords, float* valid, void* motion,
+                                   int n, int h, int w, gs_stream_t stream) {
+  GS_REQUIRE(poses && disps && intrinsics && ii && jj && target && coords && valid && motion,
+             "reproject_motion: null pointer");
+  GS_GEOM_COMMON("reproject_motion");
+  GS_REQUIRE(n <= 65535, "reproject_motion: n=%d exceeds grid.y limit", n);
+  reproject_kernel<true><<<dim3(gs_cdiv(hw, 256), n), 256, 0, st>>>(poses, disps, intrinsics, ii, jj, coords, valid, hw, w,
+                                                                    (const float2*)target, (_Float16*)motion);
+  GS_CHECK_LAUNCH("reproject_motion");
   return GS_OK;
 }
 
diff --git a/go_slam_amd/csrc/gru_gates.hip b/go_slam_amd/csrc/gru_gates.hip
--- a/go_slam_amd/csrc/gru_gates.hip
+++ b/go_slam_amd/csrc/gru_gates.hip
@@ -430,12 +430,9 @@
   reinterpret_cast<half4m*>(out)[t] = o;
 }
 
-__global__ __launch_bounds__(256) void damping_rows_kernel(const float* __restrict__ eta, const int* __restrict__ inv,
-                                                           const int64_t* __restrict__ index,
-                                                           float* __restrict__ damping_buf, float* __restrict__ out,
-                                                           int hw, float scale, float eps, size_t total) {
-  const size_t t = (size_t)blockIdx.x * 256 + threadIdx.x;
-  if (t >= total) return;
+__device__ __forceinline__ void damping_row_element(const float* __restrict__ eta, const int* __restrict__ inv,
+                                                    const int64_t* __restrict__ index, float* __restrict__ damping_buf,
+                                                    float* __restrict__ out, int hw, float scale, float eps, size_t t) {
   const int k = (int)(t / hw), p = (int)(t - (size_t)k * hw);
   const int m = inv[k];
   float* slot = damping_buf + (size_t)index[k] * hw + p;
@@ -445,12 +442,19 @@
   out[t] = scale * v + eps;
 }
 
-__global__ __launch_bounds__(256) void ba_inputs_kernel(const float2* __restrict__ coords1, const float2* __restrict__ delta,
-                                                        const float2* __restrict__ weight, float2* __restrict__ target,
-                                                        float* __restrict__ ba_target, float* __restrict__ ba_weight,
-                                                        int hw, size_t total) {
-  const size_t t = (size_t)blockIdx.x * 256 + threadIdx.x;
-  if (t >= total) return;
+__global__ __launch_bounds__(256) void damping_rows_kernel(const float* __restrict__ eta, const int* __restrict__ inv,
+                                                           const int64_t* __restrict__ index,
+                                                           float* __restrict__ damping_buf, float* __restrict__ out,
+                                                           int hw, float scale, float eps, size_t total) {
+  const size_t t = (size_t)blockIdx.x * 256 + threadIdx.x;
+  if (t >= total) return;
+  damping_row_element(eta, inv, index, damping_buf, out, hw, scale, eps, t);
+}
+
+__device__ __forceinline__ void ba_inputs_element(const float2* __restrict__ coords1, const float2* __restrict__ delta,
+                                                  const float2* __restrict__ weight, float2* __restrict__ target,
+                                                  float* __restrict__ ba_target, float* __restrict__ ba_weight, int hw,
+                                                  size_t t) {
   const size_t e = t / hw;
   const int p = (int)(t - e * hw);
   const float2 c = coords1[t], d = delta[t], wt = weight[t];
@@ -460,6 +464,31 @@
   bt[0] = tg.x; bt[hw] = tg.y;
   float* bw = ba_weight + e * 2 * hw + p;
   bw[0] = wt.x; bw[hw] = wt.y;
+}
+
+__global__ __launch_bounds__(256) void ba_inputs_kernel(const float2* __restrict__ coords1, const float2* __restrict__ delta,
+                                                        const float2* __restrict__ weight, float2* __restrict__ target,
+                                                        float* __restrict__ ba_target, float* __restrict__ ba_weight,
+                                                        int hw, size_t total) {
+  const size_t t = (size_t)blockIdx.x * 256 + threadIdx.x;
+  if (t >= total) return;
+  ba_inputs_element(coords1, delta, weight, target, ba_target, ba_weight, hw, t);
+}
+
+__global__ __launch_bounds__(256) void ba_inputs_damping_kernel(
+    const float2* __restrict__ coords1, const float2* __restrict__ delta, const float2* __restrict__ weight,
+    float2* __restrict__ target, float* __restrict__ ba_target, float* __restrict__ ba_weight, size_t in_total,
+    unsigned in_blocks, const float* __restrict__ eta, const int* __restrict__ inv, const int64_t* __restrict__ index,
+    float* __restrict__ damping_buf, float* __restrict__ out, float scale, float eps, size_t damp_total,
+    int64_t* __restrict__ age, int n_age, int hw) {
+  if (blockIdx.x < in_blocks) {
+    const size_t t = (size_t)blockIdx.x * 256 + threadIdx.x;
+    if (t < (size_t)n_age) age[t] += 1;
+    if (t < in_total) ba_inputs_element(coords1, delta, weight, target, ba_target, ba_weight, hw, t);
+  } else {
+    const size_t t = (size_t)(blockIdx.x - in_blocks) * 256 + threadIdx.x;
+    if (t < damp_total) damping_row_element(eta, inv, index, damping_buf, out, hw, scale, eps, t);
+  }
 }
 }
 
@@ -499,3 +528,21 @@
   GS_CHECK_LAUNCH("damping_rows");
   return GS_OK;
 }
+
+extern "C" int gs_ba_inputs_damping(const float* coords1, const float* delta, const float* weight, float* target,
+                                    float* ba_target, float* ba_weight, int n, int h, int w, const float* eta,
+                                    const int* inv, const int64_t* index, float* damping_buf, float* out, int n_rows,
+                                    float scale, float eps, int64_t* age, gs_stream_t stream) {
+  GS_REQUIRE(coords1 && delta && weight && target && ba_target && ba_weight, "ba_inputs_damping: null pointer");
+  GS_REQUIRE(inv && index && damping_buf && out && age, "ba_inputs_damping: null pointer");
+  GS_REQUIRE(n > 0 && h > 0 && w > 0 && n_rows >= 0, "ba_inputs_damping: bad shape");
+  const int hw = h * w;
+  const size_t in_total = (size_t)n * hw, damp_total = (size_t)n_rows * hw;
+  const size_t in_blocks = (in_total + 255) / 256, blocks = in_blocks + (damp_total + 255) / 256;
+  GS_REQUIRE(blocks < (1ull << 31), "ba_inputs_damping: too many workgroups");
+  ba_inputs_damping_kernel<<<(unsigned)blocks, 256, 0, (hipStream_t)stream>>>(
+      (const float2*)coords1, (const float2*)delta, (const float2*)weight, (float2*)target, ba_target, ba_weight,
+      in_total, (unsigned)in_blocks, eta, inv, index, damping_buf, out, scale, eps, damp_total, age, n, hw);
+  GS_CHECK_LAUNCH("ba_inputs_damping");
+  return GS_OK;
+}
diff --git a/go_slam_amd/depth_video.py b/go_slam_amd/depth_video.py
--- a/go_slam_amd/depth_video.py
+++ b/go_slam_amd/depth_video.py
@@ -232,6 +232,10 @@
         ii, jj = DepthVideo.format_indices(ii, jj, self.device)
         return droid_backends.reproject(self.poses, self.disps, self.intrinsics, ii, jj)
 
+    def reproject_motion(self, ii, jj, target):
+        ii, jj = DepthVideo.format_indices(ii, jj, self.device)
+        return droid_backends.reproject_motion(self.poses, self.disps, self.intrinsics, ii, jj, target)
+
     def distance(self, ii=None, jj=None, beta=0.3, bidirectional=True):
         return_matrix = False
         N = self._count()
@@ -257,8 +261,11 @@
         with lock:
             if t1 is None:
                 t1 = max(int(ii.max()), int(jj.max())) + 1
+            native_clamp = int(iters) > 0 and self.disps.is_cuda
             out = droid_backends.ba(self.poses, self.disps, self.intrinsics[0].contiguous(), self.disps_sens,
-                                    target, weight, eta, ii, jj, t0, t1, iters, lm, ep, motion_only, tables=tables)
-            self.disps.clamp_(min=0.001)
+                                    target, weight, eta, ii, jj, t0, t1, iters, lm, ep, motion_only, tables=tables,
+                                    clamp_min=0.001 if native_clamp else 0.0)
+            if not native_clamp:
+                self.disps.clamp_(min=0.001)
             self._finish_locked_section()
         return out
diff --git a/go_slam_amd/droid_backends.py b/go_slam_amd/droid_backends.py
--- a/go_slam_amd/droid_backends.py
+++ b/go_slam_amd/droid_backends.py
@@ -33,7 +33,7 @@
 
 
 def ba(poses, disps, intrinsics, disps_sens, targets, weights, eta, ii, jj,
-       t0, t1, iterations, lm, ep, motion_only, tables=None):
+       t0, t1, iterations, lm, ep, motion_only, tables=None, clamp_min=0.0):
     _chk("targets", targets, torch.float32)
     _chk("weights", weights, torch.float32)
     _chk("poses", poses, torch.float32)
@@ -42,6 +42,8 @@
     _chk("disps_sens", disps_sens, torch.float32)
     _chk("ii", ii, torch.int64)
     _chk("jj", jj, torch.int64)
+    if clamp_min and int(iterations) <= 0:
+        raise RuntimeError("droid_backends.ba: clamp_min needs at least one iteration (no kernel runs without)")
     if not eta.is_contiguous():
         eta = eta.contiguous()
     dev = poses.device
@@ -76,7 +78,7 @@
                         _lib.ptr(targets), _lib.ptr(weights), _lib.ptr(eta), _lib.ptr(ii), _lib.ptr(jj),
                         int(t0), int(t1), int(iterations), float(lm), float(ep), int(bool(motion_only)),
                         E, M, nbuf, ht, wd, _lib.ptr(dx), _lib.ptr(dz), _lib.ptr(status),
-                        _lib.ptr(ws), ws.numel(), flags, _lib.stream_ptr(dev))
+                        _lib.ptr(ws), ws.numel(), flags, float(clamp_min), _lib.stream_ptr(dev))
     _lib.check(rc, "droid_backends.ba")
     if new_key is not None:
         tables["key"] = new_key
@@ -243,6 +245,28 @@
     return coords, valid
 
 
+def reproject_motion(poses, disps, intrinsics, ii, jj, target):
+    _chk("poses", poses, torch.float32)
+    _chk("disps", disps, torch.float32)
+    _chk("intrinsics", intrinsics, torch.float32)
+    _chk("ii", ii, torch.int64)
+    _chk("jj", jj, torch.int64)
+    _chk("target", target, torch.float32)
+    n = ii.shape[0]
+    _, ht, wd = disps.shape
+    if target.numel() != n * ht * wd * 2:
+        raise RuntimeError(f"reproject_motion: target has {target.numel()} elements, expected {n * ht * wd * 2}")
+    coords = torch.empty(1, n, ht, wd, 2, dtype=torch.float32, device=poses.device)
+    valid = torch.empty(1, n, ht, wd, 1, dtype=torch.float32, device=poses.device)
+    motion = torch.empty(n, ht, wd, 4, dtype=torch.float16, device=poses.device)
+    with torch.cuda.device(poses.device):
+        rc = _lib.lib().gs_reproject_motion(_lib.ptr(poses), _lib.ptr(disps), _lib.ptr(intrinsics), _lib.ptr(ii),
+                                            _lib.ptr(jj), _lib.ptr(target), _lib.ptr(coords), _lib.ptr(valid),
+                                            _lib.ptr(motion), n, ht, wd, _lib.stream_ptr(poses.device))
+    _lib.check(rc, "reproject_motion")
+    return coords, valid, motion
+
+
 def altcorr_forward(fmap1, fmap2, coords, radius):
     _chk("fmap1", fmap1)
     _chk("fmap2", fmap2, fmap1.dtype)
diff --git a/go_slam_amd/droid_net.py b/go_slam_amd/droid_net.py
--- a/go_slam_amd/droid_net.py
+++ b/go_slam_amd/droid_net.py
@@ -359,7 +359,7 @@
                                     _lib.ptr(gzr), _lib.ptr(gq), b, hw, _lib.ptr(ws), ws.numel(), st), "gru_glo")
         return gzr, gq
 
-    def forward_hx(self, net, hx, inp_pre=None, glo=None):
+    def forward_hx(self, net, hx, inp_pre=None, glo=None, pre_row=None):
         from . import _lib
         b, c, h, w = net.shape
         hw = h * w
@@ -378,13 +378,15 @@
                 out = torch.empty_like(net)
                 _lib.check(L.gs_conv3x3_gru_zr2(_lib.ptr(net), hx.data_ptr() + 2 * 128, cin, cin - 128,
                                                 _lib.ptr(conv3x3_weight_image(wzr, 32)), _lib.ptr(bzr), _lib.ptr(gzr),
-                                                _lib.ptr(inp_pre), _lib.ptr(z), _lib.ptr(rnet), b, h, w, st),
-                           "conv3x3_gru_zr2")
+                                                _lib.ptr(inp_pre), _lib.ptr(z), _lib.ptr(rnet), b, h, w, st,
+                                                _lib.ptr(pre_row)), "conv3x3_gru_zr2")
                 _lib.check(L.gs_conv3x3_gru_q(_lib.ptr(rnet), hx.data_ptr() + 2 * 128, cin, cin - 128,
                                               _lib.ptr(conv3x3_weight_image(wq, 32)), _lib.ptr(bq), _lib.ptr(gq),
                                               _lib.ptr(inp_pre), _lib.ptr(z), _lib.ptr(net), _lib.ptr(out), b, h, w,
-                                              st), "conv3x3_gru_q")
+                                              st, _lib.ptr(pre_row)), "conv3x3_gru_q")
                 return out
+            if pre_row is not None:
+                inp_pre = inp_pre.permute(0, 2, 3, 1).index_select(0, pre_row.long()).permute(0, 3, 1, 2)
             copy_channels(net, hx, 0)
             zr_pre = conv_nobias(hx, wzr, padding=1)
             z = torch.empty_like(net)
@@ -488,7 +490,7 @@
             cap = min(cap, dev_cap)
         return cap
 
-    def _edge_state(self, inp, n, ht, wd):
+    def _edge_state(self, inp, n, ht, wd, seg=None):
         import collections
         import weakref
         hx = getattr(self, "_hx", None)
@@ -501,8 +503,12 @@
             cache = self._inp_pre_cache = collections.OrderedDict()
         wkey = self.gru._weights_key()
         owner = inp._base if inp._base is not None else inp
-        key = (inp.data_ptr(), tuple(inp.shape), tuple(inp.stride()), inp.dtype)
+        key = (inp.data_ptr(), tuple(inp.shape), tuple(inp.stride()), inp.dtype, seg is not None)
         ent = cache.get(key)
+        if ent is not None and seg is not None and ent[5] is not seg["ix"]:
+            ent = ent[:5] + (seg["ix"],) if ent[5].shape == seg["ix"].shape and torch.equal(ent[5], seg["ix"]) else None
+            if ent is not None:
+                cache[key] = ent
         if ent is not None and ent[0]() is owner and ent[1] == inp._version and ent[2] == wkey:
             if self.cache_check and ent[4] != self._checksum(inp):
                 raise RuntimeError("UpdateModule: the context features `inp` were modified behind the version counter "
@@ -513,6 +519,15 @@
         inp4 = inp.view(n, -1, ht, wd)
         if inp4.dtype != torch.float16 or not inp4.is_contiguous(memory_format=torch.channels_last):
             inp4 = inp4.half().contiguous(memory_format=torch.channels_last)
+        if seg is not None:
+            rep = seg["order"].index_select(0, seg["offsets"][:-1].long()).long()
+            rows = inp4.permute(0, 2, 3, 1)
+            inp_rep = rows.index_select(0, rep)
+            pre_row = seg["ix"].to(torch.int32).contiguous()
+            if self.cache_check and not torch.equal(rows, inp_rep.index_select(0, seg["ix"].long())):
+                raise RuntimeError("UpdateModule: inp_by_source=True, but edges of one source keyframe carry different "
+                                   "context features; pass the per-edge `inp` without the flag")
+            inp4 = inp_rep.permute(0, 3, 1, 2)
         try:
             inp_pre = self.gru.inp_gates(inp4)
         except torch.OutOfMemoryError:
@@ -528,8 +543,10 @@
                 e = c.get(key)
                 if e is not None and e[0] is _ref:
                     del c[key]
+        if seg is not None:
+            inp_pre = (inp_pre, pre_row)
         cache[key] = (weakref.ref(owner, _gone), inp._version, wkey, inp_pre,
-                      self._checksum(inp) if self.cache_check else None)
+                      self._checksum(inp) if self.cache_check else None, None if seg is None else seg["ix"])
         nbytes = lambda e: sum(x.numel() * x.element_size()
                                for x in (e[3] if isinstance(e[3], (tuple, list)) else (e[3],)) if torch.is_tensor(x))
         total = sum(nbytes(e) for e in cache.values())
@@ -547,8 +564,9 @@
             return w, [m.bias.detach().float().contiguous() for m in mods]
         return self._packs.get("heads", [m.weight for m in mods] + [m.bias for m in mods], build)
 
-    def _corr_independent_part(self, net4, inp, f4, n, ht, wd):
-        hx, inp_pre = self._edge_state(inp, n, ht, wd)
+    def _corr_independent_part(self, net4, inp, f4, n, ht, wd, seg=None):
+        hx, inp_pre = self._edge_state(inp, n, ht, wd, seg)
+        inp_pre, pre_row = inp_pre if seg is not None else (inp_pre, None)
         if CONV7X7_OWN and conv7x7_c4_supported(self.flow_encoder[0], f4):
             f4 = conv7x7_c4_bias_act(self._packs, self.flow_encoder[0], f4, "relu")
         else:
@@ -556,9 +574,9 @@
         conv_bias_act(self._packs, self.flow_encoder[2], f4, "relu", out=hx, out_channel=256)
         with torch.autocast("cuda", enabled=False):
             glo = self.gru.global_context(net4)
-        return hx, inp_pre, glo
-
-    def _forward_fast(self, net, inp, corr, flow, ii, jj, seg=None):
+        return hx, inp_pre, pre_row, glo
+
+    def _forward_fast(self, net, inp, corr, flow, ii, jj, seg=None, inp_by_source=False):
         batch, num, ch, ht, wd = net.shape
         cl = torch.channels_last
         packs = self._packs
@@ -575,13 +593,14 @@
         if flow is None:
             flow = torch.zeros(batch, num, 4, ht, wd, device=net.device)
         f4 = flow.view(n, -1, ht, wd).half().contiguous(memory_format=cl)
-        hx, inp_pre, glo = self._corr_independent_part(net4, inp, f4, n, ht, wd)
+        hx, inp_pre, pre_row, glo = self._corr_independent_part(
+            net4, inp, f4, n, ht, wd, seg if inp_by_source and seg is not None and seg["ix"].numel() == n else None)
         if lazy is not None:
             c4 = lazy.encoded(*self._corr_enc0_padded())
         else:
             c4 = conv1x1_bias_act(packs, self.corr_encoder[0], c4, "relu")
         conv_bias_act(packs, self.corr_encoder[2], c4, "relu", out=hx, out_channel=128)
-        net4 = self.gru.forward_hx(net4, hx, inp_pre, glo=glo)
+        net4 = self.gru.forward_hx(net4, hx, inp_pre, glo=glo, pre_row=pre_row)
         net = net4.view(*out_dim)
         hw_, hb = self._head_weights()
         heads = conv_nobias(net4, hw_ if ii is not None else hw_[:256], padding=1)
@@ -615,10 +634,10 @@
         return (self.fuse_epilogues and net.is_cuda and not torch.is_grad_enabled() and net.dtype == torch.float16
                 and net.shape[2] == 128 and n4.is_contiguous(memory_format=cl) and torch.is_autocast_enabled())
 
-    def forward(self, net, inp, corr, flow=None, ii=None, jj=None, seg=None):
+    def forward(self, net, inp, corr, flow=None, ii=None, jj=None, seg=None, inp_by_source=False):
         batch, num, ch, ht, wd = net.shape
         if self._fast_ok(net, inp, corr):
-            return self._forward_fast(net, inp, corr, flow, ii, jj, seg)
+            return self._forward_fast(net, inp, corr, flow, ii, jj, seg, inp_by_source)
         if hasattr(corr, "materialize"):
             corr = corr.materialize()
         if flow is None:
diff --git a/go_slam_amd/factor_graph.py b/go_slam_amd/factor_graph.py
--- a/go_slam_amd/factor_graph.py
+++ b/go_slam_amd/factor_graph.py
@@ -369,16 +369,22 @@
     def update(self, t0=None, t1=None, iters=2, use_inactive=False, EPS=1e-7, motion_only=False):
         idx = self._edge_index(t0, t1, use_inactive)
         t0, t1, seg = idx["t0"], idx["t1"], idx["seg"]
-        coords1, mask = self.video.reproject(self.ii, self.jj)
-        fused = self._glue_fusable(coords1)
         ht, wd = self.ht, self.wd
         E = self.ii.numel()
+        m4 = None
+        if E and self.device.type == "cuda" and self.channels_last and self.target.dtype == torch.float32 \
+                and self.target.is_contiguous() and hasattr(self.video, "reproject_motion"):
+            coords1, mask, m4 = self.video.reproject_motion(self.ii, self.jj, self.target)
+        else:
+            coords1, mask = self.video.reproject(self.ii, self.jj)
+        fused = self._glue_fusable(coords1)
         if fused:
             from . import _lib
             L, st = _lib.lib(), _lib.stream_ptr(self.device)
-            m4 = torch.empty(E, ht, wd, 4, dtype=torch.float16, device=self.device)
-            _lib.check(L.gs_motion_features(_lib.ptr(coords1), _lib.ptr(self.target), _lib.ptr(m4), E, ht, wd, st),
-                       "motion_features")
+            if m4 is None:
+                m4 = torch.empty(E, ht, wd, 4, dtype=torch.float16, device=self.device)
+                _lib.check(L.gs_motion_features(_lib.ptr(coords1), _lib.ptr(self.target), _lib.ptr(m4), E, ht, wd, st),
+                           "motion_features")
             motion = m4.permute(0, 3, 1, 2).unsqueeze(0)
         else:
             motion = torch.cat([coords1 - self.coords0, self.target - coords1], dim=-1)
@@ -387,19 +393,29 @@
         corr = self.corr.lazy(coords1) if hasattr(self.corr, "lazy") else self.corr(coords1)
         with torch.autocast("cuda", dtype=torch.float16):
             self.net, delta, weight, damping, upmask = self.update_op(
-                self.net, self.inp, corr, motion, self.ii, self.jj, seg=seg)
+                self.net, self.inp, corr, motion, self.ii, self.jj, seg=seg, **self._by_source_kw())
 
         fuse_damping = fused and damping.dtype == torch.float32 and damping.is_contiguous() and \
             self.damping.is_contiguous() and damping.shape[1] == idx["uniq_host"].numel()
         if not fuse_damping:
             self.damping[seg["uniq"]] = damping.float()
         eta_rows = damping
+        aged = False
         if fused and delta.dtype == torch.float32 and weight.dtype == torch.float32:
             bt, bw, n_in = self._ba_buffers(idx, use_inactive)
             target_new = torch.empty_like(coords1)
-            _lib.check(L.gs_ba_inputs(_lib.ptr(coords1), _lib.ptr(delta.contiguous()), _lib.ptr(weight.contiguous()),
-                                      _lib.ptr(target_new), bt[n_in:].data_ptr(), bw[n_in:].data_ptr(), E, ht, wd, st),
-                       "ba_inputs")
+            delta_c, weight_c = delta.contiguous(), weight.contiguous()
+            if fuse_damping and E and self.age.is_contiguous() and self.age.dtype == torch.int64:
+                damping = torch.empty(idx["damping_index"].numel(), ht, wd, device=self.device)
+                _lib.check(L.gs_ba_inputs_damping(
+                    _lib.ptr(coords1), _lib.ptr(delta_c), _lib.ptr(weight_c), _lib.ptr(target_new), bt[n_in:].data_ptr(),
+                    bw[n_in:].data_ptr(), E, ht, wd, _lib.ptr(eta_rows), _lib.ptr(idx["damping_inv"]),
+                    _lib.ptr(idx["damping_index"]), _lib.ptr(self.damping), _lib.ptr(damping), damping.shape[0], 0.2,
+                    float(EPS), _lib.ptr(self.age), st), "ba_inputs_damping")
+                aged = True
+            else:
+                _lib.check(L.gs_ba_inputs(_lib.ptr(coords1), _lib.ptr(delta_c), _lib.ptr(weight_c), _lib.ptr(target_new),
+                                          bt[n_in:].data_ptr(), bw[n_in:].data_ptr(), E, ht, wd, st), "ba_inputs")
             self.target, self.weight = target_new, weight
             target, weight = bt, bw
         else:
@@ -414,7 +430,9 @@
             target = target.view(-1, ht, wd, 2).permute(0, 3, 1, 2).contiguous()
             weight = weight.view(-1, ht, wd, 2).permute(0, 3, 1, 2).contiguous()
 
-        if fuse_damping:
+        if aged:
+            pass
+        elif fuse_damping:
             damping = torch.empty(idx["damping_index"].numel(), ht, wd, device=self.device)
             _lib.check(L.gs_damping_rows(_lib.ptr(eta_rows), _lib.ptr(idx["damping_inv"]), _lib.ptr(idx["damping_index"]),
                                          _lib.ptr(self.damping), _lib.ptr(damping), damping.shape[0], ht * wd, 0.2,
@@ -431,7 +449,19 @@
                           lm=1e-4, ep=0.1, motion_only=motion_only, tables=tables)
         if self.upsample:
             self.video.upsample(seg["uniq"], upmask[0])
-        self.age += 1
+        if not aged:
+            self.age += 1
+
+    def _by_source_kw(self):
+        kw = getattr(self, "_by_source", None)
+        if kw is None:
+            import inspect
+            try:
+                params = inspect.signature(getattr(self.update_op, "forward", self.update_op)).parameters
+            except (TypeError, ValueError):
+                params = {}
+            kw = self._by_source = {"inp_by_source": True} if "inp_by_source" in params else {}
+        return kw
 
     def _select_edges(self, x5, sel):
         x4 = x5[0]
@@ -469,7 +499,8 @@
         for n, seg_h in enumerate(segs):
             ck = {k: up[f"{n}.{k}"] for k in ("sel", "ii", "jj", "corr_ii", "corr_jj", "uniq")}
             seg = {k: (up[f"{n}.seg.{k}"] if isinstance(v, np.ndarray) else v) for k, v in seg_h.items()}
-            ck["seg_kw"] = {"seg": seg} if getattr(self.update_op, "_forward_fast", None) is not None else {}
+            ck["seg_kw"] = {"seg": seg, **self._by_source_kw()} \
+                if getattr(self.update_op, "_forward_fast", None) is not None else {}
             def _inp(ix=ck["ii"], box=ck):
                 v = box.get("inp_cached")
                 if v is None:
diff --git a/include/goslam_hip.h b/include/goslam_hip.h
--- a/include/goslam_hip.h
+++ b/include/goslam_hip.h
@@ -78,6 +78,9 @@
 int gs_reproject(const float* poses, const float* disps, const float* intrinsics,
                  const int64_t* ii, const int64_t* jj, float* coords, float* valid,
                  int n, int h, int w, gs_stream_t stream);
+int gs_reproject_motion(const float* poses, const float* disps, const float* intrinsics,
+                        const int64_t* ii, const int64_t* jj, const float* target, float* coords, float* valid,
+                        void* motion, int n, int h, int w, gs_stream_t stream);
 
 int gs_projmap(const float* poses, const float* disps, const float* intrinsics,
                const int64_t* ii, const int64_t* jj, float* coords, float* valid,
@@ -153,13 +156,13 @@
                          int y_stride, int n_out, int n, int h, int w, gs_stream_t stream);
 int gs_conv3x3_gru_zr2(const void* net, const void* x_rest, int x_rest_stride, int c_rest, const void* wpack,
                        const float* bias_zr, const float* glo_zr, const void* inp_pre, void* z_out, void* rnet_out,
-                       int n, int h, int w, gs_stream_t stream);
+                       int n, int h, int w, gs_stream_t stream, const int* pre_row);
 int gs_conv3x3_gru_zr(const void* hx, int hx_stride, int c_in, const void* wpack, const float* bias_zr,
                       const float* glo_zr, const void* inp_pre, void* z_out, void* rnet_out, int n, int h, int w,
                       gs_stream_t stream);
 int gs_conv3x3_gru_q(const void* rnet, const void* x_rest, int x_rest_stride, int c_rest, const void* wpack,
                      const float* bias_q, const float* glo_q, const void* inp_pre, const void* z, const void* net,
-                     void* net_out, int n, int h, int w, gs_stream_t stream);
+                     void* net_out, int n, int h, int w, gs_stream_t stream, const int* pre_row);
 int gs_conv3x3_head(const void* x, int x_stride, const float* in_bias, int in_relu, const void* wpack,
                     const float* bias, int n_out, int epilogue, float out_scale, float* out, int n, int h, int w,
                     gs_stream_t stream);
@@ -187,6 +190,10 @@
 
 int gs_damping_rows(const float* eta, const int* inv, const int64_t* index, float* damping_buf, float* out,
                     int n_rows, int hw, float scale, float eps, gs_stream_t stream);
+int gs_ba_inputs_damping(const float* coords1, const float* delta, const float* weight, float* target,
+                         float* ba_target, float* ba_weight, int n, int h, int w, const float* eta, const int* inv,
+                         const int64_t* index, float* damping_buf, float* out, int n_rows, float scale, float eps,
+                         int64_t* age, gs_stream_t stream);
 
 int gs_cvx_upsample(const float* disps, const void* mask, const int64_t* ix, float* out,
                     int m, int h, int w, int mask_channels_last, gs_stream_t stream);
@@ -211,7 +218,7 @@
              int t0, int t1, int iterations, float lm, float ep, int motion_only,
              int n_edges, int n_depth, int nbuf, int h, int w,
              float* dx, float* dz, int32_t* status_out,
-             void* workspace, size_t workspace_bytes, int flags, gs_stream_t stream);
+             void* workspace, size_t workspace_bytes, int flags, float clamp_min, gs_stream_t stream);
 
 int gs_chol_solve(double* H, double* b, int n, float lm, float ep, int path, float* dx, int32_t* status,
                   gs_stream_t stream);
```
